# yhg926/MetaKSSD

Hardware: AMD Instinct MI355X
Metric: Gbases/s sketched (150 bp synthetic reads, L3K11 -A) (higher is better)
Workload: dtype u64 k-mers over u8 bases (integer)

## Files before the change

### include/metakssd_hip.h

```cpp
#ifndef METAKSSD_HIP_H
#define METAKSSD_HIP_H
#include <stddef.h>
#include <stdint.h>

#ifdef __cplusplus
extern "C" {
#endif

#define MK_ABI_VERSION 1

enum {
  MK_OK = 0,
  MK_ERR_ARG = -1,
  MK_ERR_NO_DEVICE = -2,
  MK_ERR_HIP = -3,
  MK_ERR_CROWDED = -4,
  MK_ERR_STATE = -5,
  MK_ERR_IO = -6,
  MK_ERR_FORMAT = -7,
  MK_ERR_NOMEM = -8
};

enum {
  MK_MODE_KOC = 0,
  MK_MODE_SET = 1,
  MK_MODE_UNIQ_SET = 2,
  MK_MODE_OCC_SET = 3
};

typedef struct mk_shuf {
  int32_t id, k, subk, drlevel;
  int32_t *table;
  uint64_t len;
} mk_shuf;

int mk_shuf_read(const char *path, mk_shuf *out);
int mk_shuf_generate(int32_t k, int32_t subk, int32_t drlevel, uint64_t seed, mk_shuf *out);
int mk_shuf_write(const mk_shuf *s, const char *path);
void mk_shuf_free(mk_shuf *s);

typedef struct mk_params {
  int32_t shuf_id, k, subk, drlevel;
  int32_t half_outctx_len;
  int32_t TL;
  int32_t crvsaddmove;
  int32_t component_num;
  int32_t comp_code_bits;
  int32_t dim_start, dim_end;
  uint32_t hashsize;
  uint32_t hashlimit;
  uint64_t tupmask, domask, undomask;
  const int32_t *shuf_table;
  uint64_t shuf_len;
  int32_t component_sz;
  int32_t reserved;
} mk_params;

int mk_params_init(const mk_shuf *shuf, mk_params *out);
int mk_params_init_csz(const mk_shuf *shuf, int32_t component_sz, mk_params *out);

typedef struct mk_engine mk_engine;

typedef struct mk_component {
  uint32_t *ids;
  uint16_t *counts;
  uint64_t n;
} mk_component;

typedef struct mk_result {
  int32_t component_num;
  uint64_t total;
  mk_component *components;
} mk_result;

typedef struct mk_profile {
  double scan_ms;
  uint64_t scan_launches;
  double resolve_ms;
  double clear_ms;
  double finish_ms;
  uint64_t bases_scanned;
  uint64_t rows_scanned;
  double finish_side_ms;
} mk_profile;

int mk_device_count(int *n);
int mk_engine_create(const mk_params *p, int device, mk_engine **out);
enum { MK_ENGINE_LAZY_TABLES = 1u };
int mk_engine_create_ex(const mk_params *p, int device, unsigned flags, mk_engine **out);
int mk_engine_destroy(mk_engine *e);
enum { MK_OPT_SPARSE = 1, MK_OPT_CAND_CAP = 2, MK_OPT_RESULT_CAP = 3, MK_OPT_DIRECT_HOST = 4, MK_OPT_FRONT_BITS = 5, MK_OPT_KEYLIST_CAP = 6,
       MK_OPT_BATCH_TAB_BITS = 7, MK_OPT_SPLIT_CUS = 10 };
int mk_engine_set_option(mk_engine *e, int option, int64_t value);
int mk_engine_set_stream(mk_engine *e, void *hip_stream);
int mk_engine_use_own_stream(mk_engine *e);
int mk_engine_share_scan_queue(mk_engine *e, mk_engine *with);
const char *mk_last_error(const mk_engine *e);

enum { MK_BEGIN_NOTHING_FOLLOWS = 0x100 };
int mk_sketch_begin(mk_engine *e, int mode);
int mk_sketch_begin_occ(mk_engine *e, int min_occurrence);
#define MK_ROW_PITCH(need) ((((need) + 15u) & ~15u) + (((((need) + 15u) & ~15u) & 127u) == 0u && (((need) + 15u) & ~15u) < 4096u ? 16u : 0u))
int mk_sketch_push_reads(mk_engine *e, const uint8_t *rows, uint32_t stride, uint64_t nreads, uint64_t first_read_ordinal);
#define MK_ROWS_PACKED 0x80000000u
#define MK_PACKED_PITCH 64u
#define MK_PACKED_MAX_BASES 152u
int mk_params_packed_ok(const mk_params *p);
int mk_pack_rows_host(const uint8_t *rows, uint32_t stride, uint64_t nrows, uint8_t *packed );
#define MK_ROWS_WIDE 0x40000000u
#define MK_WIDE_MAX_BASES 240u
uint64_t mk_fasta_pack_bound(size_t n, int32_t TL, uint32_t format);
int mk_fasta_pack_rows(const uint8_t *text, size_t n, int32_t TL, uint32_t format, uint8_t *rows, uint64_t max_rows, uint64_t *nrows);
int mk_sketch_push_reads_device(mk_engine *e, const uint8_t *rows_dev, uint32_t stride, uint64_t nreads,
                                uint64_t first_read_ordinal);
int mk_sketch_push_reads_async(mk_engine *e, const uint8_t *rows, uint32_t stride, uint64_t nreads, uint64_t first_read_ordinal,
                               uint64_t *ticket);
int mk_sketch_push_wait(mk_engine *e, uint64_t ticket);
int mk_sketch_push_stream(mk_engine *e, const uint8_t *text, uint64_t n, int final);
int mk_sketch_finish(mk_engine *e, mk_result *out);
int mk_sketch_finish_begin(mk_engine *e);
int mk_sketch_finish_end(mk_engine *e, mk_result *out);
int mk_result_release(mk_engine *e, mk_result *r);
int mk_engine_sync(mk_engine *e);

#define MK_BATCH_MAX_FILES 1024u
#define MK_BATCH_FILE_MAX ((uint64_t)64 << 20)
#define MK_BATCH_TEXT_MAX ((uint64_t)1 << 30)
typedef struct mk_batch_file {
  const uint8_t *text;
  uint64_t n;
} mk_batch_file;
typedef struct mk_batch_result {
  int32_t status;
  int32_t alone;
  mk_result r;
} mk_batch_result;
int mk_sketch_batch_begin(mk_engine *e, int mode, const mk_batch_file *files, uint32_t nfiles);
int mk_sketch_batch_begin_rows(mk_engine *e, int mode, uint32_t format, const mk_batch_file *files, uint32_t nfiles);
int mk_sketch_batch_end(mk_engine *e, mk_batch_result *out );

int mk_host_alloc(void **p, size_t bytes);
int mk_host_free(void *p);
int mk_host_register(void *p, size_t bytes);
int mk_host_unregister(void *p);
int mk_host_register_on(int device, void *p, size_t bytes);
int mk_host_arena_alloc(void **p, size_t bytes);
int mk_host_arena_free(void *p, size_t bytes);

int mk_partial_count(mk_engine *e, uint64_t *n);
int mk_partial_export(mk_engine *e, uint64_t *keys_dev, uint32_t *counts_dev, uint64_t *ords_dev, uint64_t capacity,
                      uint64_t *n_out);
int mk_partial_count_begin(mk_engine *e);
int mk_partial_export_async(mk_engine *e, uint64_t *keys_dev, uint32_t *counts_dev, uint64_t *ords_dev, uint64_t capacity,
                            uint64_t *n_out);
int mk_partial_import(mk_engine *e, const uint64_t *keys_dev, const uint32_t *counts_dev, const uint64_t *ords_dev,
                      uint64_t n);

int mk_partial_export_split_async(mk_engine *e, uint32_t nparts, uint64_t *keys_dev, uint32_t *counts_dev, uint64_t *ords_dev,
                                  uint64_t capacity, uint64_t *part_counts, uint64_t *n_out);
int mk_partial_export_split(mk_engine *e, uint32_t nparts, uint64_t *keys_dev, uint32_t *counts_dev, uint64_t *ords_dev,
                            uint64_t capacity, uint64_t *part_counts, uint64_t *n_out);
int mk_partial_restart(mk_engine *e);
int mk_partial_list_reserve(mk_engine *e, uint64_t n, uint64_t **keys_dev, uint32_t **counts_dev, uint64_t **ords_dev);
int mk_partial_list_commit(mk_engine *e, uint64_t n);
int mk_partial_list_adopt(mk_engine *e, const uint64_t *keys_dev, const uint32_t *counts_dev, const uint64_t *ords_dev, uint64_t n,
                          uint64_t offset);

int mk_profile_enable(mk_engine *e, int on);
int mk_profile_reset(mk_engine *e);
int mk_profile_get(mk_engine *e, mk_profile *out);

int mk_synth_rows_host(uint64_t seed, uint64_t first_read, uint64_t nreads, uint32_t len, uint32_t stride, uint8_t *rows);
int mk_synth_rows_device(int device, void *hip_stream, uint64_t seed, uint64_t first_read, uint64_t nreads, uint32_t len,
                         uint32_t stride, uint8_t *rows_dev);
int mk_synth_fastq_write(const char *path, uint64_t seed, uint64_t first_read, uint64_t nreads, uint32_t len);
int mk_synth_fastq_write_mt(const char *path, uint64_t seed, uint64_t first_read, uint64_t nreads, uint32_t len, int nthreads);

int mk_fastq_frame(const uint8_t *buf, size_t n, int final, uint8_t *rows, uint32_t stride, uint64_t max_rows,
                   uint64_t *nrows, size_t *consumed);
int mk_fastq_frame_q(const uint8_t *buf, size_t n, int final, int32_t qmin, int32_t TL, uint64_t records_before,
                     uint8_t *rows, uint32_t stride, uint64_t max_rows, uint64_t *nrows, uint64_t *nrecords,
                     size_t *consumed);
int mk_fastq_frame_mt(const uint8_t *buf, size_t n, int final, int occ, int32_t qmin, int32_t TL, uint64_t records_before,
                      uint8_t *rows, uint32_t stride, uint64_t max_rows, int nthreads, uint64_t *nrows, uint64_t *nrecords,
                      size_t *consumed);
typedef struct mk_fastq_opts {
  int32_t occ;
  int32_t qmin, TL;
  int32_t nthreads;
  int32_t inflight;
  uint64_t chunk_bytes;
  int32_t drop_pages;
  int32_t ahead;
  int32_t packed;
  int32_t fd;
  int32_t early_chunks;
  int32_t reserved2;
  uint64_t pool_bytes;
} mk_fastq_opts;
typedef struct mk_fastq_stats {
  uint64_t rows, records, chunks, chunks_discarded, serial_rows;
  uint32_t threads;
  double t_setup_s, t_wait_frame_s, t_push_s, t_total_s;
  double t_push_call_s, t_wait_call_s, t_push_call_max_s, t_first_push_call_s;
} mk_fastq_stats;
typedef struct mk_rows_sink {
  void *ctx;
  int (*push)(void *ctx, const uint8_t *rows, uint32_t stride, uint64_t nrows, uint64_t first_row_ordinal, uint64_t *token);
  int (*wait)(void *ctx, uint64_t token);
  uint8_t *(*alloc)(void *ctx, size_t bytes);
  void (*release)(void *ctx, uint8_t *p, size_t bytes);
  void (*ready)(void *ctx, const uint8_t *rows, size_t bytes);
} mk_rows_sink;
int mk_fastq_stream(const uint8_t *text, size_t n, const mk_fastq_opts *o, const mk_rows_sink *sink, uint64_t first_ordinal,
                    mk_fastq_stats *st);
int mk_sketch_push_fastq(mk_engine *e, const uint8_t *text, size_t n, const mk_fastq_opts *o, uint64_t first_ordinal,
                         mk_fastq_stats *st);

typedef struct mk_fasta_state {
  uint32_t TL;
  uint32_t in_header;
  uint32_t fill;
  uint32_t fresh;
  uint8_t pending[4096];
} mk_fasta_state;
int mk_fasta_window_init(mk_fasta_state *st, int32_t TL);
int mk_fasta_window(mk_fasta_state *st, const uint8_t *buf, size_t n, int final, uint8_t *rows, uint32_t stride,
                    uint64_t max_rows, uint64_t *nrows, size_t *consumed);

typedef struct mk_sketchdir mk_sketchdir;
int mk_sketchdir_open(const char *outdir, const mk_params *p, int koc, int nfiles, mk_sketchdir **out);
int mk_sketchdir_add(mk_sketchdir *d, const char *input_path, const mk_result *r);
int mk_sketchdir_close(mk_sketchdir *d);

enum { MK_SET_UNION = 0, MK_SET_UNIQ_UNION = 1 };
typedef struct mk_setop mk_setop;
int mk_setop_create(int device, mk_setop **out);
int mk_setop_destroy(mk_setop *s);
const char *mk_setop_last_error(const mk_setop *s);
int mk_setop_begin(mk_setop *s, int mode);
int mk_setop_add(mk_setop *s, const uint32_t *ids, uint64_t n);
int mk_setop_add_device(mk_setop *s, const uint32_t *ids_dev, uint64_t n);
int mk_setop_finish(mk_setop *s, const uint32_t **ids_out, uint64_t *n_out);
int mk_setop_result_device(mk_setop *s, const uint32_t **ids_dev, uint64_t *n);
int mk_setop_filter(mk_setop *s, int keep_members, const uint32_t *ids, uint64_t n, const uint64_t *bounds, uint32_t nb,
                    const uint32_t **ids_out, uint64_t *n_out, uint64_t *bounds_out);
// ... 174 lines not shown
```

### metakssd_amd/capi.py

```python
import ctypes as C
import os

import numpy as np

_HERE = os.path.dirname(os.path.abspath(__file__))
LIB_PATH = os.environ.get("MK_LIBRARY") or os.path.join(_HERE, "lib", "libmetakssd_hip.so")

MK_OK = 0
MK_ERR_ARG, MK_ERR_NO_DEVICE, MK_ERR_HIP, MK_ERR_CROWDED = -1, -2, -3, -4
MK_ERR_STATE, MK_ERR_IO, MK_ERR_FORMAT, MK_ERR_NOMEM = -5, -6, -7, -8
MK_MODE_KOC, MK_MODE_SET, MK_MODE_UNIQ_SET, MK_MODE_OCC_SET = 0, 1, 2, 3
MK_ROWS_PACKED, MK_PACKED_PITCH, MK_PACKED_MAX_BASES = 0x80000000, 64, 152
MK_ROWS_WIDE, MK_WIDE_MAX_BASES = 0x40000000, 240
MK_OPT_SPARSE, MK_OPT_CAND_CAP, MK_OPT_RESULT_CAP, MK_OPT_DIRECT_HOST, MK_OPT_FRONT_BITS, MK_OPT_KEYLIST_CAP, MK_OPT_BATCH_TAB_BITS = 1, 2, 3, 4, 5, 6, 7
MK_BEGIN_NOTHING_FOLLOWS = 0x100
MK_OPT_SPLIT_CUS = 10


class MkError(RuntimeError):
    def __init__(self, code, msg=""):
        super().__init__("metakssd_hip error %d: %s" % (code, msg))
        self.code = code


class CrowdedError(MkError):
    """more than hashlimit distinct keys: the reference aborts with 'the context space is too crowd' (iseq2comem.c:708-709)"""


class ShufC(C.Structure):
    _fields_ = [("id", C.c_int32), ("k", C.c_int32), ("subk", C.c_int32), ("drlevel", C.c_int32),
                ("table", C.POINTER(C.c_int32)), ("len", C.c_uint64)]


class ParamsC(C.Structure):
    _fields_ = [("shuf_id", C.c_int32), ("k", C.c_int32), ("subk", C.c_int32), ("drlevel", C.c_int32),
                ("half_outctx_len", C.c_int32), ("TL", C.c_int32), ("crvsaddmove", C.c_int32),
                ("component_num", C.c_int32), ("comp_code_bits", C.c_int32),
                ("dim_start", C.c_int32), ("dim_end", C.c_int32),
                ("hashsize", C.c_uint32), ("hashlimit", C.c_uint32),
                ("tupmask", C.c_uint64), ("domask", C.c_uint64), ("undomask", C.c_uint64),
                ("shuf_table", C.POINTER(C.c_int32)), ("shuf_len", C.c_uint64), ("component_sz", C.c_int32), ("reserved", C.c_int32)]


class ComponentC(C.Structure):
    _fields_ = [("ids", C.POINTER(C.c_uint32)), ("counts", C.POINTER(C.c_uint16)), ("n", C.c_uint64)]


class ResultC(C.Structure):
    _fields_ = [("component_num", C.c_int32), ("total", C.c_uint64), ("components", C.POINTER(ComponentC))]


class ProfileC(C.Structure):
    _fields_ = [("scan_ms", C.c_double), ("scan_launches", C.c_uint64), ("resolve_ms", C.c_double), ("clear_ms", C.c_double),
                ("finish_ms", C.c_double), ("bases_scanned", C.c_uint64), ("rows_scanned", C.c_uint64), ("finish_side_ms", C.c_double)]


class FastaStateC(C.Structure):
    _fields_ = [("TL", C.c_uint32), ("in_header", C.c_uint32), ("fill", C.c_uint32), ("fresh", C.c_uint32),
                ("pending", C.c_uint8 * 4096)]


class FastqOptsC(C.Structure):
    _fields_ = [("occ", C.c_int32), ("qmin", C.c_int32), ("TL", C.c_int32), ("nthreads", C.c_int32), ("inflight", C.c_int32),
                ("chunk_bytes", C.c_uint64), ("drop_pages", C.c_int32), ("ahead", C.c_int32), ("packed", C.c_int32), ("fd", C.c_int32),
                ("early_chunks", C.c_int32), ("reserved2", C.c_int32), ("pool_bytes", C.c_uint64)]


class FastqStatsC(C.Structure):
    _fields_ = [("rows", C.c_uint64), ("records", C.c_uint64), ("chunks", C.c_uint64), ("chunks_discarded", C.c_uint64),
                ("serial_rows", C.c_uint64), ("threads", C.c_uint32), ("t_setup_s", C.c_double), ("t_wait_frame_s", C.c_double),
                ("t_push_s", C.c_double), ("t_total_s", C.c_double), ("t_push_call_s", C.c_double), ("t_wait_call_s", C.c_double),
                ("t_push_call_max_s", C.c_double), ("t_first_push_call_s", C.c_double)]


_PUSH_FN = C.CFUNCTYPE(C.c_int, C.c_void_p, C.c_void_p, C.c_uint32, C.c_uint64, C.c_uint64, C.POINTER(C.c_uint64))
_WAIT_FN = C.CFUNCTYPE(C.c_int, C.c_void_p, C.c_uint64)
_ALLOC_FN = C.CFUNCTYPE(C.c_void_p, C.c_void_p, C.c_size_t)
_RELEASE_FN = C.CFUNCTYPE(None, C.c_void_p, C.c_void_p, C.c_size_t)
_READY_FN = C.CFUNCTYPE(None, C.c_void_p, C.c_void_p, C.c_size_t)


class RowsSinkC(C.Structure):
    _fields_ = [("ctx", C.c_void_p), ("push", _PUSH_FN), ("wait", _WAIT_FN), ("alloc", _ALLOC_FN), ("release", _RELEASE_FN),
                ("ready", C.c_void_p)]


class BatchFileC(C.Structure):
    _fields_ = [("text", C.c_void_p), ("n", C.c_uint64)]


class DistOptsC(C.Structure):
    _fields_ = [("metric", C.c_int32), ("outfields", C.c_int32), ("correction", C.c_int32), ("num_neigb", C.c_int32),
                ("dthreshold", C.c_double)]


class BgzfBlockC(C.Structure):
    _fields_ = [("in_off", C.c_uint64), ("out_off", C.c_uint64), ("in_len", C.c_uint32), ("pay_off", C.c_uint32), ("pay_len", C.c_uint32),
                ("crc32", C.c_uint32), ("isize", C.c_uint32), ("reserved", C.c_uint32)]


class GzipInfoC(C.Structure):
    _fields_ = [("pay_off", C.c_uint64), ("pay_len", C.c_uint64), ("crc32", C.c_uint32), ("isize", C.c_uint32), ("is_single", C.c_int32),
                ("reserved", C.c_int32)]


class GzMemberC(C.Structure):
    _fields_ = [("pay_off", C.c_uint64), ("out_off", C.c_uint64), ("pay_len", C.c_uint32), ("isize", C.c_uint32), ("crc32", C.c_uint32),
                ("reserved", C.c_uint32)]


class GzMemberResultC(C.Structure):
    _fields_ = [("status", C.c_uint32), ("consumed", C.c_uint32), ("pos", C.c_uint32), ("crc32", C.c_uint32)]


class GzFileC(C.Structure):
    _fields_ = [("comp", C.c_void_p), ("n", C.c_uint64), ("info", GzipInfoC)]


class BgzfOptsC(C.Structure):
    _fields_ = [("chunk_bytes", C.c_uint64), ("reserved", C.c_uint64)]


class BgzfStatsC(C.Structure):
    _fields_ = [("blocks", C.c_uint64), ("chunks", C.c_uint64), ("comp_bytes", C.c_uint64), ("text_bytes", C.c_uint64), ("rows", C.c_uint64),
                ("inflate_ms", C.c_double), ("frame_ms", C.c_double), ("t_scan_s", C.c_double), ("t_read_s", C.c_double), ("t_total_s", C.c_double),
                ("bad_block", C.c_int64), ("bad_status", C.c_int32), ("reserved", C.c_int32)]


def _load():
    if not os.path.exists(LIB_PATH):
        raise ImportError("%s not built: run `python -c 'import __graft_entry__ as g; g.build()'` "
                          "(make -C metakssd_amd/csrc)" % LIB_PATH)
    lib = C.CDLL(LIB_PATH)
    vp, u8p, u64, u32, i32 = C.c_void_p, C.POINTER(C.c_uint8), C.c_uint64, C.c_uint32, C.c_int32
    sig = {
        "mk_shuf_read": [C.c_char_p, C.POINTER(ShufC)],
        "mk_shuf_generate": [i32, i32, i32, u64, C.POINTER(ShufC)],
        "mk_shuf_write": [C.POINTER(ShufC), C.c_char_p],
        "mk_params_init": [C.POINTER(ShufC), C.POINTER(ParamsC)],
        "mk_params_init_csz": [C.POINTER(ShufC), i32, C.POINTER(ParamsC)],
        "mk_device_count": [C.POINTER(C.c_int)],
        "mk_engine_create": [C.POINTER(ParamsC), C.c_int, C.POINTER(vp)],
        "mk_engine_destroy": [vp],
        "mk_engine_set_option": [vp, C.c_int, C.c_int64],
        "mk_engine_set_stream": [vp, vp],
        "mk_engine_use_own_stream": [vp],
        "mk_engine_share_scan_queue": [vp, vp],
        "mk_sketch_begin": [vp, C.c_int],
        "mk_sketch_begin_occ": [vp, C.c_int],
        "mk_sketch_push_reads": [vp, vp, u32, u64, u64],
        "mk_sketch_push_reads_device": [vp, vp, u32, u64, u64],
        "mk_sketch_push_reads_async": [vp, vp, u32, u64, u64, C.POINTER(u64)],
        "mk_sketch_push_wait": [vp, u64],
        "mk_sketch_push_stream": [vp, vp, u64, C.c_int],
        "mk_partial_count_begin": [vp],
        "mk_partial_export_async": [vp, vp, vp, vp, u64, C.POINTER(u64)],
        "mk_pack_rows_host": [vp, u32, u64, vp],
        "mk_params_packed_ok": [C.POINTER(ParamsC)],
        "mk_sketch_batch_begin": [vp, C.c_int, vp, u32],
        "mk_sketch_batch_begin_rows": [vp, C.c_int, u32, vp, u32],
        "mk_fasta_pack_rows": [vp, C.c_size_t, C.c_int32, u32, vp, u64, C.POINTER(u64)],
        "mk_sketch_batch_end": [vp, vp],
        "mk_sketch_batch_begin_gz": [vp, C.c_int, C.POINTER(GzFileC), u32],
        "mk_sketch_batch_gz_status": [vp, vp, u32],
        "mk_gzip_scan": [C.c_int, vp, C.c_size_t, C.POINTER(GzipInfoC)],
        "mk_inflate_members": [vp, vp, C.c_size_t, C.POINTER(GzMemberC), u32, vp, C.c_size_t, C.POINTER(GzMemberResultC)],
        "mk_sketch_finish": [vp, C.POINTER(ResultC)],
        "mk_sketch_finish_begin": [vp],
        "mk_sketch_finish_end": [vp, C.POINTER(ResultC)],
        "mk_result_release": [vp, C.POINTER(ResultC)],
        "mk_engine_sync": [vp],
        "mk_host_alloc": [C.POINTER(vp), C.c_size_t],
        "mk_host_free": [vp],
        "mk_host_arena_alloc": [C.POINTER(vp), C.c_size_t],
        "mk_host_arena_free": [vp, C.c_size_t],
        "mk_host_register": [vp, C.c_size_t],
        "mk_host_unregister": [vp],
        "mk_partial_count": [vp, C.POINTER(u64)],
        "mk_partial_export": [vp, vp, vp, vp, u64, C.POINTER(u64)],
        "mk_partial_import": [vp, vp, vp, vp, u64],
        "mk_partial_export_split": [vp, u32, vp, vp, vp, u64, C.POINTER(u64), C.POINTER(u64)],
        "mk_partial_export_split_async": [vp, u32, vp, vp, vp, u64, C.POINTER(u64), C.POINTER(u64)],
        "mk_partial_restart": [vp],
        "mk_partial_list_reserve": [vp, u64, C.POINTER(vp), C.POINTER(vp), C.POINTER(vp)],
        "mk_partial_list_commit": [vp, u64],
        "mk_partial_list_adopt": [vp, vp, vp, vp, u64, u64],
        "mk_profile_enable": [vp, C.c_int],
        "mk_profile_reset": [vp],
        "mk_profile_get": [vp, C.POINTER(ProfileC)],
        "mk_synth_rows_host": [u64, u64, u64, u32, u32, vp],
        "mk_synth_rows_device": [C.c_int, vp, u64, u64, u64, u32, u32, vp],
        "mk_synth_fastq_write": [C.c_char_p, u64, u64, u64, u32],
        "mk_synth_fastq_write_mt": [C.c_char_p, u64, u64, u64, u32, C.c_int],
        "mk_fastq_stream": [vp, C.c_size_t, C.POINTER(FastqOptsC), C.POINTER(RowsSinkC), u64, C.POINTER(FastqStatsC)],
        "mk_sketch_push_fastq": [vp, vp, C.c_size_t, C.POINTER(FastqOptsC), u64, C.POINTER(FastqStatsC)],
        "mk_fastq_frame": [vp, C.c_size_t, C.c_int, vp, u32, u64, C.POINTER(u64), C.POINTER(C.c_size_t)],
        "mk_fastq_frame_q": [vp, C.c_size_t, C.c_int, i32, i32, u64, vp, u32, u64, C.POINTER(u64), C.POINTER(u64),
                             C.POINTER(C.c_size_t)],
        "mk_fastq_frame_mt": [vp, C.c_size_t, C.c_int, C.c_int, i32, i32, u64, vp, u32, u64, C.c_int, C.POINTER(u64), C.POINTER(u64),
                              C.POINTER(C.c_size_t)],
        "mk_fasta_window_init": [C.POINTER(FastaStateC), i32],
        "mk_fasta_window": [C.POINTER(FastaStateC), vp, C.c_size_t, C.c_int, vp, u32, u64, C.POINTER(u64),
                            C.POINTER(C.c_size_t)],
        "mk_setop_create": [C.c_int, C.POINTER(vp)],
        "mk_setop_destroy": [vp],
        "mk_setop_begin": [vp, C.c_int],
        "mk_setop_add": [vp, vp, u64],
        "mk_setop_add_device": [vp, vp, u64],
        "mk_setop_finish": [vp, C.POINTER(vp), C.POINTER(u64)],
        "mk_setop_result_device": [vp, C.POINTER(vp), C.POINTER(u64)],
        "mk_setop_join": [vp, vp, vp, u64, vp, u64, vp, u32, C.POINTER(vp), C.POINTER(u64), vp],
        "mk_setop_last_join_ms": [vp, C.POINTER(C.c_double)],
        "mk_mco_create": [C.c_int, C.POINTER(vp)],
        "mk_mco_destroy": [vp],
        "mk_mco_build": [vp, vp, vp, u32, C.POINTER(vp), C.POINTER(u64), C.POINTER(vp), C.POINTER(vp), C.POINTER(u64)],
        "mk_mco_index_rows": [vp, u64, u64, vp],
        "mk_mco_sort_pairs": [vp, vp, vp, u64],
        "mk_mco_set_option": [vp, C.c_int, C.c_int64],
        "mk_mco_count_begin": [vp, u32, u32],
        "mk_mco_count_add": [vp, vp, u64, vp, vp, vp, vp, vp],
        "mk_mco_count_finish": [vp, vp],
        "mk_mco_last_kernel_ms": [vp, C.POINTER(C.c_double), C.POINTER(C.c_double)],
        "mk_abv_create": [C.c_int, C.POINTER(vp)],
        "mk_abv_destroy": [vp],
        "mk_abv_index": [vp, vp, u64, vp, u32, u32, C.POINTER(vp), C.POINTER(vp), C.POINTER(vp), C.POINTER(C.c_int64)],
        "mk_abv_load": [vp, vp, u64, vp, u32, vp, u32],
        "mk_abv_search": [vp, C.c_int, u32, vp, vp, vp, C.POINTER(vp), C.POINTER(vp), C.POINTER(C.c_int64)],
        "mk_abv_last_kernel_ms": [vp, C.POINTER(C.c_double), C.POINTER(C.c_double)],
        "mk_composite_create": [C.c_int, C.POINTER(vp)],
        "mk_composite_destroy": [vp],
        "mk_composite_load_begin": [vp, u32, u32],
        "mk_composite_load_component": [vp, u32, vp, vp],
        "mk_composite_query_begin": [vp, u32],
        "mk_composite_query_component": [vp, u32, vp, vp, vp],
        "mk_composite_query_finish": [vp, C.POINTER(vp), vp],
        "mk_composite_set_option": [vp, C.c_int, C.c_int64],
        "mk_composite_last_kernel_ms": [vp, C.POINTER(C.c_double), C.POINTER(C.c_double)],
        "mk_composite_last_counts": [vp, C.POINTER(u64), C.POINTER(u64)],
        "mk_byread_create": [C.c_int, C.POINTER(vp)],
        "mk_byread_destroy": [vp],
        "mk_byread_begin": [vp, C.POINTER(ParamsC)],
        "mk_byread_push_text": [vp, vp, u64, C.c_int],
        "mk_byread_take": [vp, u32, C.POINTER(vp), C.POINTER(u64), C.POINTER(vp), C.POINTER(u64)],
        "mk_byread_finish": [vp, C.POINTER(u64), C.POINTER(u64), C.POINTER(C.c_double)],
        "mk_reverse_ids": [vp, vp, u64, u32, vp],
        "mk_byread_last_kernel_ms": [vp, C.POINTER(C.c_double), C.POINTER(C.c_double)],
        "mk_byread_write_stat": [C.c_char_p, C.POINTER(ParamsC), C.c_char_p],
        "mk_reverse_outname": [C.c_char_p, C.c_char_p, C.c_size_t],
        "mk_dist_print": [vp, C.POINTER(DistOptsC), i32, i32, u32, u32, vp, vp, vp, vp, vp],
        "mk_sketchdir_open": [C.c_char_p, C.POINTER(ParamsC), C.c_int, C.c_int, C.POINTER(vp)],
        "mk_sketchdir_add": [vp, C.c_char_p, C.POINTER(ResultC)],
        "mk_sketchdir_close": [vp],
        "mk_bgzf_scan": [C.c_int, vp, C.c_size_t, C.POINTER(C.POINTER(BgzfBlockC)), C.POINTER(u64), C.POINTER(u64), C.POINTER(C.c_int)],
        "mk_inflate_create": [C.c_int, C.POINTER(vp)],
        "mk_inflate_destroy": [vp],
        "mk_inflate_blocks": [vp, vp, C.c_size_t, C.POINTER(BgzfBlockC), u64, vp, C.c_size_t, vp],
        "mk_fastq_frame_device": [vp, vp, C.c_size_t, C.c_int, vp, C.c_size_t, C.POINTER(u32), C.POINTER(u64), C.POINTER(C.c_size_t), C.POINTER(u32)],
        "mk_fastq_frame_q_device": [vp, vp, C.c_size_t, C.c_int, i32, u64, vp, C.c_size_t, C.POINTER(u32), C.POINTER(u64), C.POINTER(u64),
                                    C.POINTER(C.c_size_t), C.POINTER(u32)],
        "mk_inflate_last_kernel_ms": [vp, C.POINTER(C.c_double), C.POINTER(C.c_double)],
        "mk_sketch_push_bgzf": [vp, C.c_int, C.c_size_t, C.POINTER(BgzfOptsC), u64, C.POINTER(BgzfStatsC)],
        "mk_sketch_push_bgzf_q": [vp, C.c_int, C.c_size_t, C.POINTER(BgzfOptsC), i32, u64, C.POINTER(BgzfStatsC)],
    }
    for name, args in sig.items():
        fn = getattr(lib, name)
        fn.argtypes = args
        fn.restype = C.c_int
    lib.mk_shuf_free.argtypes = [C.POINTER(ShufC)]
    lib.mk_shuf_free.restype = None
    lib.mk_setop_last_error.argtypes = [vp]
    lib.mk_setop_last_error.restype = C.c_char_p
    lib.mk_mco_last_error.argtypes = [vp]
    lib.mk_mco_last_error.restype = C.c_char_p
    lib.mk_abv_last_error.argtypes = [vp]
    lib.mk_abv_last_error.restype = C.c_char_p
    lib.mk_composite_last_error.argtypes = [vp]
    lib.mk_composite_last_error.restype = C.c_char_p
    lib.mk_byread_last_error.argtypes = [vp]
    lib.mk_byread_last_error.restype = C.c_char_p
    lib.mk_inflate_last_error.argtypes = [vp]
    lib.mk_inflate_last_error.restype = C.c_char_p
    lib.mk_inflate_status_text.argtypes = [C.c_int]
    lib.mk_inflate_status_text.restype = C.c_char_p
    lib.mk_bgzf_last_error.argtypes = []
    lib.mk_bgzf_last_error.restype = C.c_char_p
    lib.mk_bgzf_free.argtypes = [C.POINTER(BgzfBlockC)]
    lib.mk_bgzf_free.restype = None
    lib.mk_setop_stream.argtypes = [vp]
    lib.mk_setop_stream.restype = vp
    lib.mk_last_error.argtypes = [vp]
    lib.mk_last_error.restype = C.c_char_p
    lib.mk_fasta_pack_bound.argtypes = [C.c_size_t, C.c_int32, u32]
    lib.mk_fasta_pack_bound.restype = u64
    return lib


lib = _load()
# ... 51 lines not shown
def synth_rows_host(seed, first_read, nreads, length, stride):
    rows = np.empty(nreads * stride, dtype=np.uint8)
    _check(lib.mk_synth_rows_host(seed, first_read, nreads, length, stride, rows.ctypes.data))
    return rows


def pack_rows_host(rows, stride):
    rows = np.ascontiguousarray(rows, dtype=np.uint8)
    n = rows.size // stride
    raw = np.zeros(n * MK_PACKED_PITCH + 64, dtype=np.uint8)
    off = (-raw.ctypes.data) % 64
    out = raw[off:off + n * MK_PACKED_PITCH]
    _check(lib.mk_pack_rows_host(rows.ctypes.data if n else None, stride, n, out.ctypes.data if n else None))
    return out


def fasta_pack_rows(text, TL, fmt=None):
    fmt = MK_ROWS_PACKED if fmt is None else fmt
    b = np.frombuffer(bytes(text), dtype=np.uint8)
    bound = int(lib.mk_fasta_pack_bound(len(b), TL, fmt))
    raw = np.zeros(bound * MK_PACKED_PITCH + 64, dtype=np.uint8)
    off = (-raw.ctypes.data) % 64
    n = C.c_uint64(0)
    rc = lib.mk_fasta_pack_rows(b.ctypes.data if len(b) else None, len(b), TL, fmt, raw.ctypes.data + off, bound, C.byref(n))
    return raw[off:off + n.value * MK_PACKED_PITCH], rc


def fastq_frame(buf, stride, final=True, max_rows=None):
    b = np.frombuffer(buf, dtype=np.uint8)
    max_rows = max_rows if max_rows is not None else len(b) // 4 + 1
    rows = np.zeros(max(1, max_rows) * stride, dtype=np.uint8)
    n, used = C.c_uint64(0), C.c_size_t(0)
    rc = lib.mk_fastq_frame(b.ctypes.data if len(b) else None, len(b), 1 if final else 0, rows.ctypes.data, stride,
                            max_rows, C.byref(n), C.byref(used))
    return rows[: n.value * stride], n.value, used.value, rc


def fastq_frame_q(buf, stride, TL, qmin=0, final=True, records_before=0, max_rows=None):
    b = np.frombuffer(buf, dtype=np.uint8)
    max_rows = max_rows if max_rows is not None else len(b) // 4 + len(b) // max(1, stride - TL) + 2
    rows = np.zeros(max(1, max_rows) * stride, dtype=np.uint8)
    n, nrec, used = C.c_uint64(0), C.c_uint64(0), C.c_size_t(0)
    rc = lib.mk_fastq_frame_q(b.ctypes.data if len(b) else None, len(b), 1 if final else 0, qmin, TL, records_before,
                              rows.ctypes.data, stride, max_rows, C.byref(n), C.byref(nrec), C.byref(used))
    return rows[: n.value * stride], n.value, nrec.value, used.value, rc


def fastq_frame_mt(buf, stride, nthreads, occ=False, TL=22, qmin=0, final=True, records_before=0, max_rows=None):
    b = np.frombuffer(buf, dtype=np.uint8)
    max_rows = max_rows if max_rows is not None else len(b) // 4 + len(b) // max(1, stride - TL) + 2
    rows = np.zeros(max(1, max_rows) * stride, dtype=np.uint8)
    n, nrec, used = C.c_uint64(0), C.c_uint64(0), C.c_size_t(0)
    rc = lib.mk_fastq_frame_mt(b.ctypes.data if len(b) else None, len(b), 1 if final else 0, 1 if occ else 0, qmin, TL, records_before,
                               rows.ctypes.data, stride, max_rows, nthreads, C.byref(n), C.byref(nrec), C.byref(used))
    return rows[: n.value * stride], n.value, nrec.value, used.value, rc


def fastq_stream(buf, nthreads=4, chunk_bytes=0, occ=False, TL=22, qmin=0, first_ordinal=0, inflight=2, drop_pages=False, packed=False, pool_bytes=0,
                 ready_log=None, via_fd=False, early_chunks=0):
    b = np.frombuffer(buf, dtype=np.uint8)
    pushes, keep = [], {}
    libc = C.CDLL(None)
    libc.malloc.restype = C.c_void_p
    libc.malloc.argtypes = [C.c_size_t]
    libc.free.argtypes = [C.c_void_p]

    def push(ctx, rows, stride, nrows, ord0, token):
        a = np.ctypeslib.as_array(C.cast(rows, C.POINTER(C.c_uint8)), shape=(nrows * (stride & ~MK_ROWS_PACKED),)).copy()
        pushes.append((a, stride, nrows, ord0))
        token[0] = len(pushes)
        return 0

    def wait(ctx, token):
        return 0

    blocks = []

    def alloc(ctx, n):
        p = libc.malloc(n)
        blocks.append((p, n))
        return p

    def ready(ctx, rows, n):
        if ready_log is not None:
            ready_log.append((rows - blocks[-1][0], n))
    ready_fn = _READY_FN(ready)
    sink = RowsSinkC(None, _PUSH_FN(push), _WAIT_FN(wait), _ALLOC_FN(alloc), _RELEASE_FN(lambda ctx, p, n: libc.free(p)),
                     C.cast(ready_fn, C.c_void_p) if ready_log is not None else None)
    keep["sink"] = (sink, ready_fn)
    fd = -1
    if via_fd:
        import tempfile
        tf = tempfile.TemporaryFile()
        tf.write(bytes(buf))
        tf.flush()
        fd = tf.fileno()
        keep["file"] = tf
    o = FastqOptsC(1 if occ else 0, qmin, TL, nthreads, inflight, chunk_bytes, 1 if drop_pages else 0, 0, 1 if packed else 0, fd if via_fd else 0, early_chunks, 0, pool_bytes)
    if ready_log is not None:
        ready_log.append(blocks)
    st = FastqStatsC()
    rc = lib.mk_fastq_stream(None if via_fd or not len(b) else b.ctypes.data, len(b), C.byref(o), C.byref(sink), first_ordinal, C.byref(st))
    return pushes, st, rc


def fasta_windows(buf, TL, stride, chunk=None):
    b = np.frombuffer(buf, dtype=np.uint8)
    st = FastaStateC()
    _check(lib.mk_fasta_window_init(C.byref(st), TL))
    out = []
    max_rows = 4096
    rows = np.zeros(max_rows * stride, dtype=np.uint8)
    pos, step = 0, (chunk or max(1, len(b)))
    while True:
        end = min(len(b), pos + step)
        final = end >= len(b)
        off = pos
        while True:
            n, used = C.c_uint64(0), C.c_size_t(0)
            ptr = b[off:end].ctypes.data if end > off else None
            _check(lib.mk_fasta_window(C.byref(st), ptr, end - off, 1 if final else 0, rows.ctypes.data, stride, max_rows,
                                       C.byref(n), C.byref(used)))
            if n.value:
                out.append(rows[: n.value * stride].copy())
            off += used.value
            if off >= end and n.value < max_rows:
                break
        pos = end
        if final:
            break
    return np.concatenate(out) if out else np.zeros(0, dtype=np.uint8)


class Engine:

    def __init__(self, shuf, device=0, sparse=None, cand_cap=None, component_sz=8, front_bits=None):
        self.shuf = shuf
        self.params = shuf.params(component_sz)
        self.h = C.c_void_p()
        rc = lib.mk_engine_create(C.byref(self.params), device, C.byref(self.h))
        if rc != MK_OK:
            raise MkError(rc, lib.mk_last_error(None).decode(errors="replace"))
        self.device = device
        if sparse is not None:
            self.set_option(MK_OPT_SPARSE, int(sparse))
        if cand_cap is not None:
            self.set_option(MK_OPT_CAND_CAP, int(cand_cap))
        if front_bits is not None:
            self.set_option(MK_OPT_FRONT_BITS, int(front_bits))

    def set_option(self, option, value):
        _check(lib.mk_engine_set_option(self.h, option, value), self.h)

    def close(self):
        if self.h:
            lib.mk_engine_destroy(self.h)
            self.h = C.c_void_p()

    def __del__(self):
        try:
            self.close()
        except Exception:
            pass

    def set_stream(self, stream_handle):
        _check(lib.mk_engine_set_stream(self.h, C.c_void_p(stream_handle or None)), self.h)

    def use_own_stream(self):
        _check(lib.mk_engine_use_own_stream(self.h), self.h)

    def share_scan_queue(self, owner):
        _check(lib.mk_engine_share_scan_queue(self.h, owner.h), self.h)

    def begin(self, mode=MK_MODE_KOC):
        _check(lib.mk_sketch_begin(self.h, mode), self.h)

    def begin_occ(self, min_occurrence=1):
        _check(lib.mk_sketch_begin_occ(self.h, min_occurrence), self.h)

    def push_bgzf(self, path, chunk_bytes=0, first_ordinal=0, qmin=None):
        o, st = BgzfOptsC(chunk_bytes, 0), BgzfStatsC()
        fd = os.open(path, os.O_RDONLY)
        try:
            if qmin is None:
                rc = lib.mk_sketch_push_bgzf(self.h, fd, os.fstat(fd).st_size, C.byref(o), first_ordinal, C.byref(st))
            else:
                rc = lib.mk_sketch_push_bgzf_q(self.h, fd, os.fstat(fd).st_size, C.byref(o), qmin, first_ordinal, C.byref(st))
        finally:
            os.close(fd)
        if rc:
            err = MkError(rc, (lib.mk_bgzf_last_error() or b"").decode())
            err.stats = st
            raise err
        return st

    def push_bgzf_q(self, path, qmin=0, chunk_bytes=0, first_ordinal=0):
        return self.push_bgzf(path, chunk_bytes, first_ordinal, qmin=qmin)

    def push_reads(self, rows, stride, first_read_ordinal=0):
        rows = np.ascontiguousarray(rows, dtype=np.uint8)
        pitch = stride & ~MK_ROWS_PACKED
        assert rows.size % pitch == 0
        n = rows.size // pitch
        if n:
            _check(lib.mk_sketch_push_reads(self.h, rows.ctypes.data, stride, n, first_read_ordinal), self.h)
        return n

    def push_fastq(self, buf, nthreads=8, chunk_bytes=0, occ=False, TL=22, qmin=0, first_ordinal=0, inflight=2, packed=False):
        b = np.frombuffer(buf, dtype=np.uint8)
        o = FastqOptsC(1 if occ else 0, qmin, TL, nthreads, inflight, chunk_bytes, 0, 0, 1 if packed else 0)
        st = FastqStatsC()
        _check(lib.mk_sketch_push_fastq(self.h, b.ctypes.data if len(b) else None, len(b), C.byref(o), first_ordinal, C.byref(st)), self.h)
        return st

    def push_stream(self, text, final=True, piece=None):
        b = np.frombuffer(bytes(text), dtype=np.uint8)
        if not piece:
            _check(lib.mk_sketch_push_stream(self.h, b.ctypes.data if len(b) else None, len(b), 1 if final else 0), self.h)
            return
        at = 0
        while True:
            n = min(piece, len(b) - at)
            last = at + n >= len(b)
            part = np.ascontiguousarray(b[at:at + n])
            _check(lib.mk_sketch_push_stream(self.h, part.ctypes.data if n else None, n, 1 if (last and final) else 0), self.h)
            at += n
            if last:
                break

    def push_reads_async(self, rows, stride, first_read_ordinal=0):
        assert rows.dtype == np.uint8 and rows.flags["C_CONTIGUOUS"] and rows.size % stride == 0
        t = C.c_uint64(0)
        _check(lib.mk_sketch_push_reads_async(self.h, rows.ctypes.data, stride, rows.size // stride, first_read_ordinal, C.byref(t)), self.h)
        return t.value

    def push_wait(self, ticket):
        _check(lib.mk_sketch_push_wait(self.h, ticket), self.h)

    def push_reads_device(self, dev_ptr, stride, nreads, first_read_ordinal=0):
        _check(lib.mk_sketch_push_reads_device(self.h, C.c_void_p(dev_ptr), stride, nreads, first_read_ordinal), self.h)

    def finish(self):
        r = ResultC()
        _check(lib.mk_sketch_finish(self.h, C.byref(r)), self.h)
        out = []
        for c in range(r.component_num):
            comp = r.components[c]
            n = comp.n
            ids = np.ctypeslib.as_array(comp.ids, shape=(n,)).copy() if n else np.zeros(0, np.uint32)
            cnt = None
            if comp.counts:
                cnt = np.ctypeslib.as_array(comp.counts, shape=(n,)).copy() if n else np.zeros(0, np.uint16)
            out.append((ids, cnt))
        self.last_total = r.total
        lib.mk_result_release(self.h, C.byref(r))
        return out

    def batch_begin(self, texts, mode=MK_MODE_SET, one_buffer=False):
        arrs = []
        if one_buffer:
            offs, at = [], 0
            for t in texts:
                offs.append(at)
                at += (len(t) + 1023) // 1024 * 1024
            buf = np.zeros(max(at, 1024), dtype=np.uint8)
            for t, o in zip(texts, offs):
                buf[o:o + len(t)] = np.frombuffer(bytes(t), dtype=np.uint8)
            arrs = [buf[o:o + len(t)] for t, o in zip(texts, offs)]
            keep = [buf]
        else:
            arrs = [np.frombuffer(bytes(t), dtype=np.uint8).copy() for t in texts]
            keep = arrs
        files = (BatchFileC * len(texts))()
        for i, a in enumerate(arrs):
            files[i].text = (keep[0].ctypes.data + offs[i]) if one_buffer else (a.ctypes.data if a.size else None)
            files[i].n = a.size
        _check(lib.mk_sketch_batch_begin(self.h, mode, C.cast(files, C.c_void_p), len(texts)), self.h)
        self._batches = getattr(self, "_batches", [])
        self._batches.append((keep, len(texts)))

    def batch_begin_rows(self, row_arrays, mode=MK_MODE_SET, pinned=False, fmt=MK_ROWS_PACKED, gap=MK_PACKED_PITCH):
        n = len(row_arrays)
        files = (BatchFileC * n)()
        if pinned:
            total = sum(a.size + gap for a in row_arrays) + 4096
            p = C.c_void_p()
            _check(lib.mk_host_alloc(C.byref(p), total))
            buf = np.ctypeslib.as_array((C.c_uint8 * total).from_address(p.value))
            buf[:] = 0xA5
            at = 0
            for i, a in enumerate(row_arrays):
                buf[at:at + a.size] = a
                files[i].text = p.value + at
                files[i].n = a.size
                at += a.size + gap
            del buf
            keep = ("pinned", None, p.value)
        else:
            arrs = []
            for i, a in enumerate(row_arrays):
                raw = np.zeros(a.size + 64, dtype=np.uint8)
                off = (-raw.ctypes.data) % 64
                raw[off:off + a.size] = a
                arrs.append(raw)
                files[i].text = (raw.ctypes.data + off) if a.size else None
                files[i].n = a.size
# ... 768 lines not shown
```

### metakssd_amd/csrc/mk_engine.hip

```cpp
#include "metakssd_hip.h"
#include "mk_poison.hip.h"
#include "mk_kernels.hip.h"
#include "mk_stream.hip.h"
#include "mk_batch.hip.h"
#include "mk_gz.hip.h"
#include "mk_packed.hip.h"

#include <math.h>
#include <stdarg.h>
#include <stdio.h>
#include <stdlib.h>
#include <string.h>

#include <vector>

static thread_local char g_create_error[512] = "";

struct mk_evpair { hipEvent_t a, b; };
#define MK_TICKETS 16
#define MK_REGIONS 3
#define MK_REGION_BYTES ((size_t)256 << 20)

struct mk_engine {
  int device = 0;
  int num_cu = 0;
  mk_params P{};
  mk_keyparams kp{};
  char err[512] = "";
  hipStream_t own_stream = nullptr, stream = nullptr, copy_stream = nullptr;
  hipStream_t scan_stream = nullptr, split_stream = nullptr;
  hipEvent_t ev_scan_pre = nullptr, ev_scan_post = nullptr;
  int split_cus = 0, scan_cus = 0;
  bool tail = false, tail_active = false;
  bool scan_shared = false;
  mk_engine *scan_owner = nullptr;
  int scan_lent = 0;

  int32_t *d_shuf = nullptr;
  uint32_t *d_accept = nullptr;
  uint32_t *d_accept_bits = nullptr;
  uint32_t n_accept = 0;
  uint32_t bm_bits = 0;
  uint4 *d_cand = nullptr;
  uint32_t *d_cand_count = nullptr;
  uint32_t cand_slots = 0, cand_cap = 0;

  void *d_tab = nullptr;
  size_t tab_bytes = 0;
  bool sparse = false, tables_tracked = false;
  uint32_t *d_dirty_acc = nullptr, *d_dirty_slot = nullptr, *d_list_acc = nullptr, *d_list_slot = nullptr, *d_nlist = nullptr;
  uint32_t acc_words = 0, slot_words = 0, acc_blocks = 0;
  mk_table tab{};
  uint32_t *d_slot = nullptr;
  mk_dist dist{};
  uint32_t *d_chunk = nullptr;
  uint32_t nchunks = 0;
  unsigned long long *d_comp_totals = nullptr, *h_comp_totals = nullptr;
  unsigned long long *d_counters = nullptr;
  void *d_front = nullptr;
  mk_front *d_front_desc = nullptr;
  mk_front front{};
  uint64_t front_slots = 0;
  int front_bits_opt = -1;
  bool big_maybe_dirty = true;
  unsigned long long *h_counters = nullptr;
  bool tables_ready = false;
  bool init_queued = true;
  mk_accept_pair *d_pairs = nullptr;
  uint32_t *h_ids = nullptr;
  uint16_t *h_cnt = nullptr;
  uint64_t h_cap = 0;
  std::vector<mk_component> comps;

  uint8_t *d_stage[MK_REGIONS] = {};
  size_t stage_bytes = 0;
  hipEvent_t ev_copied[MK_REGIONS] = {}, ev_scanned[MK_REGIONS] = {};
  bool stage_two_streams[MK_REGIONS] = {};
  int stage_cur = 0;
  bool direct_host = false;
  bool region_open = false;
  size_t region_fill = 0;
  uint32_t region_stride = 0;
  uint64_t region_first_ord = 0, region_rows = 0;
  hipEvent_t ev_ticket[MK_TICKETS] = {};
  uint64_t tickets_issued = 0;
  std::vector<std::pair<const void *, size_t>> lds_granted;

  uint32_t *d_res_ids = nullptr;
  uint16_t *d_res_cnt = nullptr;
  uint64_t res_cap = 0;
  hipStream_t res_stream = nullptr;
  hipEvent_t ev_res = nullptr;
  bool res_koc = false;
  uint64_t res_D = 0;
  bool res_pending = false, res_side = false;
  uint64_t res_total = 0;
  unsigned long long *d_snap = nullptr, *h_snap = nullptr;
  std::vector<mk_evpair> ev_finish_side;
  void *d_kl = nullptr;
  uint64_t kl_cap = 0;
  uint32_t *d_kl_buckets = nullptr;
  uint64_t kl_bucket_cap = 0;
  bool slot_clean = false;
  uint8_t *d_text = nullptr, *d_stream = nullptr, *d_stream_tmp = nullptr;
  size_t text_cap = 0, stream_cap = 0;
  mk_fa_sum *d_fa_sum = nullptr;
  size_t fa_sum_cap = 0;
  mk_fa_state *d_fa_state = nullptr, *h_fa_state = nullptr;
  unsigned long long *d_split = nullptr;
  bool counter0_used = true;
  uint64_t fa_tail = 0;
  uint64_t fa_rows_done = 0;
  bool fa_used = false, fa_final = false;
  uint32_t fa_pitch = 0;

  struct mk_bctx *bctx[3] = {nullptr, nullptr, nullptr};
  uint64_t batch_begun = 0, batch_ended = 0;
  int batch_tb_opt = 0;
  std::vector<uint32_t> gz_status;
  const mk_batch_dev *cur_batch = nullptr;

  int mode = -1;
  uint32_t min_occ = 1;
  bool begun = false, compacted = false;
  bool count_queued = false;
  uint64_t D = 0;

  int tune_threads = 1024;
  bool tune_onepass = true;
  uint32_t tune_cb = MK_MAX_CB;

  bool profiling = false;
  std::vector<mk_evpair> ev_scan, ev_resolve, ev_clear, ev_finish, ev_pool;
  uint64_t prof_rows = 0, prof_bytes = 0;
};

static int mk_fail(mk_engine *e, int code, const char *fmt, ...) {
  char buf[512];
  va_list ap;
  va_start(ap, fmt);
  vsnprintf(buf, sizeof buf, fmt, ap);
  va_end(ap);
  if (e) snprintf(e->err, sizeof e->err, "%s", buf);
  else snprintf(g_create_error, sizeof g_create_error, "%s", buf);
  return code;
}

#define MK_HIP(e, call)                                                                                   \
  do {                                                                                                    \
    hipError_t _r = (call);                                                                               \
    if (_r != hipSuccess) return mk_fail((e), _r == hipErrorOutOfMemory ? MK_ERR_NOMEM : MK_ERR_HIP,      \
                                         "%s:%d %s -> %s", __FILE__, __LINE__, #call, hipGetErrorString(_r)); \
  } while (0)

extern "C" const char *mk_last_error(const mk_engine *e) { return e ? e->err : g_create_error; }

extern "C" int mk_device_count(int *n) {
  if (!n) return MK_ERR_ARG;
  int c = 0;
  hipError_t r = hipGetDeviceCount(&c);
  if (r != hipSuccess) { *n = 0; return mk_fail(nullptr, MK_ERR_NO_DEVICE, "hipGetDeviceCount: %s", hipGetErrorString(r)); }
  *n = c;
  return MK_OK;
}

extern "C" int mk_host_alloc(void **p, size_t bytes) {
  if (!p) return MK_ERR_ARG;
  hipError_t r = mk_pin_alloc(p, bytes, hipHostMallocDefault);
  return r == hipSuccess ? MK_OK : mk_fail(nullptr, MK_ERR_NOMEM, "mk_pin_alloc(%zu): %s", bytes, hipGetErrorString(r));
}
extern "C" int mk_host_free(void *p) { return hipHostFree(p) == hipSuccess ? MK_OK : MK_ERR_HIP; }
#include <pthread.h>
#include <sys/mman.h>
struct mk_touch_job { uint8_t *p; size_t n; pthread_t th; };
static void *mk_touch_run(void *arg) {
  mk_touch_job *j = (mk_touch_job *)arg;
  const int pz = mk_poison_byte();
  if (pz >= 0) memset(j->p, pz, j->n);
  else for (size_t off = 0; off < j->n; off += 4096) j->p[off] = 0;
  return nullptr;
}
extern "C" int mk_host_arena_alloc(void **out, size_t bytes) {
  if (!out || !bytes) return MK_ERR_ARG;
  const size_t huge = (size_t)2 << 20;
  const size_t len = (bytes + huge - 1) & ~(huge - 1);
  void *m = mmap(nullptr, len, PROT_READ | PROT_WRITE, MAP_PRIVATE | MAP_ANONYMOUS, -1, 0);
  if (m == MAP_FAILED) return mk_fail(nullptr, MK_ERR_NOMEM, "mmap(%zu) failed", len);
#ifdef MADV_HUGEPAGE
  (void)madvise(m, len, MADV_HUGEPAGE);
#endif
  enum { T = 8 };
  mk_touch_job job[T];
  int started = 0;
  for (int t = 0; t < T; t++) {
    const size_t lo = len / T * (size_t)t, hi = t + 1 == T ? len : len / T * (size_t)(t + 1);
    job[t].p = (uint8_t *)m + lo; job[t].n = hi - lo;
    if (t + 1 < T && pthread_create(&job[t].th, nullptr, mk_touch_run, &job[t]) == 0) started |= 1 << t;
    else mk_touch_run(&job[t]);
  }
  for (int t = 0; t < T; t++) if (started & (1 << t)) pthread_join(job[t].th, nullptr);
  hipError_t r = hipHostRegister(m, len, hipHostRegisterDefault);
  if (r != hipSuccess) {
    (void)hipGetLastError();
    munmap(m, len);
    return mk_fail(nullptr, r == hipErrorOutOfMemory ? MK_ERR_NOMEM : MK_ERR_HIP, "hipHostRegister(%zu): %s", len, hipGetErrorString(r));
  }
  *out = m;
  return MK_OK;
}
extern "C" int mk_host_arena_free(void *p, size_t bytes) {
  if (!p) return MK_ERR_ARG;
  const size_t huge = (size_t)2 << 20;
  const size_t len = (bytes + huge - 1) & ~(huge - 1);
  const bool ok = hipHostUnregister(p) == hipSuccess;
  if (!ok) (void)hipGetLastError();
  munmap(p, len);
  return ok ? MK_OK : MK_ERR_HIP;
}

extern "C" int mk_host_register(void *p, size_t bytes) {
  if (!p || !bytes) return MK_ERR_ARG;
  hipError_t r = hipHostRegister(p, bytes, hipHostRegisterDefault);
  if (r != hipSuccess) { (void)hipGetLastError(); return mk_fail(nullptr, MK_ERR_HIP, "hipHostRegister(%zu): %s", bytes, hipGetErrorString(r)); }
  return MK_OK;
}
extern "C" int mk_host_register_on(int device, void *p, size_t bytes) {
  if (hipSetDevice(device) != hipSuccess) { (void)hipGetLastError(); return mk_fail(nullptr, MK_ERR_NO_DEVICE, "hipSetDevice(%d) failed", device); }
  return mk_host_register(p, bytes);
}
extern "C" int mk_host_unregister(void *p) {
  if (hipHostUnregister(p) == hipSuccess) return MK_OK;
  (void)hipGetLastError();
  return MK_ERR_HIP;
}

static mk_evpair mk_ev_get(mk_engine *e) {
  mk_evpair p{nullptr, nullptr};
  if (!e->ev_pool.empty()) { p = e->ev_pool.back(); e->ev_pool.pop_back(); return p; }
  hipEventCreate(&p.a);
  hipEventCreate(&p.b);
  return p;
}

struct mk_accept_job {
  const int32_t *t;
  uint64_t lo, hi;
  int32_t ds, de;
  std::vector<mk_accept_pair> out;
  pthread_t th;
  bool started;
};
static void *mk_accept_run(void *arg) {
  mk_accept_job *j = (mk_accept_job *)arg;
  const int32_t *t = j->t;
  const uint32_t ds = (uint32_t)j->ds, span = (uint32_t)(j->de - j->ds);
  for (uint64_t d = j->lo; d < j->hi; d++) {
    const int32_t v = t[d];
    if ((uint32_t)v - ds < span) j->out.push_back(mk_accept_pair{(uint32_t)d, v});
  }
  return nullptr;
}

static void mk_bctx_free(struct mk_bctx *c);

extern "C" int mk_engine_destroy(mk_engine *e) {
  if (!e) return MK_ERR_ARG;
  if (e->scan_lent > 0) return mk_fail(e, MK_ERR_STATE, "mk_engine_destroy: %d engine(s) still borrow this engine's scan queue (mk_engine_share_scan_queue): destroy them first", e->scan_lent);
  if (e->scan_owner) { e->scan_owner->scan_lent--; e->scan_owner = nullptr; }
  hipSetDevice(e->device);
  (void)hipStreamSynchronize(e->stream);
  for (hipStream_t st : {e->own_stream, e->copy_stream, e->scan_stream, e->split_stream, e->res_stream})
    if (st && st != e->stream) (void)hipStreamSynchronize(st);
  hipFree(e->d_pairs);
  hipFree(e->d_cand); hipFree(e->d_cand_count);
  hipFree(e->d_shuf); hipFree(e->d_accept); hipFree(e->d_accept_bits); hipFree(e->d_tab); hipFree(e->d_front); hipFree(e->d_front_desc); hipFree(e->d_slot);
  hipFree(e->d_dirty_acc); hipFree(e->d_dirty_slot); hipFree(e->d_list_acc); hipFree(e->d_list_slot); hipFree(e->d_nlist);
  hipFree(e->dist.key); hipFree(e->dist.ord); hipFree(e->dist.cnt);
  hipFree(e->d_chunk); hipFree(e->d_comp_totals); hipFree(e->d_counters); hipFree(e->d_split);
  hipFree(e->d_kl); hipFree(e->d_kl_buckets);
  for (mk_bctx *c : e->bctx) mk_bctx_free(c);
  hipFree(e->d_res_ids); hipFree(e->d_res_cnt); hipFree(e->d_snap);
  if (e->h_snap) hipHostFree(e->h_snap);
  if (e->res_stream) hipStreamDestroy(e->res_stream);
  if (e->scan_stream && !e->scan_shared) hipStreamDestroy(e->scan_stream);
  if (e->split_stream) hipStreamDestroy(e->split_stream);
  if (e->ev_scan_pre) hipEventDestroy(e->ev_scan_pre);
  if (e->ev_scan_post) hipEventDestroy(e->ev_scan_post);
  if (e->ev_res) hipEventDestroy(e->ev_res);
  hipFree(e->d_text); hipFree(e->d_stream); hipFree(e->d_stream_tmp); hipFree(e->d_fa_sum); hipFree(e->d_fa_state);
  if (e->h_fa_state) hipHostFree(e->h_fa_state);
  for (int i = 0; i < MK_TICKETS; i++) if (e->ev_ticket[i]) hipEventDestroy(e->ev_ticket[i]);
  if (e->h_counters) hipHostFree(e->h_counters);
  if (e->h_ids) hipHostFree(e->h_ids);
  if (e->h_cnt) hipHostFree(e->h_cnt);
  for (int i = 0; i < MK_REGIONS; i++) {
    hipFree(e->d_stage[i]);
    if (e->ev_copied[i]) hipEventDestroy(e->ev_copied[i]);
    if (e->ev_scanned[i]) hipEventDestroy(e->ev_scanned[i]);
  }
  for (auto *v : {&e->ev_scan, &e->ev_resolve, &e->ev_clear, &e->ev_finish, &e->ev_finish_side, &e->ev_pool})
    for (auto &p : *v) { hipEventDestroy(p.a); hipEventDestroy(p.b); }
  if (e->own_stream) hipStreamDestroy(e->own_stream);
  delete e;
  return MK_OK;
}

static int mk_config_sparse(mk_engine *e, bool on) {
  hipFree(e->d_dirty_acc); hipFree(e->d_dirty_slot); hipFree(e->d_list_acc); hipFree(e->d_list_slot); hipFree(e->d_nlist);
  e->d_dirty_acc = e->d_dirty_slot = e->d_list_acc = e->d_list_slot = e->d_nlist = nullptr;
  e->tab.dirty = nullptr;
  e->tab.dirty_shift = 0;
  e->sparse = on;
  e->tables_tracked = false;
  if (!on) return MK_OK;
  const uint64_t S = e->P.hashsize;
  e->acc_blocks = (uint32_t)((S + MK_SPARSE_BLOCK - 1) / MK_SPARSE_BLOCK);
  e->acc_words = (e->acc_blocks + 31u) / 32u;
  const uint32_t nch = (uint32_t)((S + MK_DUMP_CHUNK - 1) / MK_DUMP_CHUNK);
  e->slot_words = (nch + 31u) / 32u;
  MK_HIP(e, mk_dev_alloc(&e->d_dirty_acc, (size_t)e->acc_words * 4));
  MK_HIP(e, mk_dev_alloc(&e->d_dirty_slot, (size_t)e->slot_words * 4));
  MK_HIP(e, mk_dev_alloc(&e->d_list_acc, (size_t)e->acc_words * 32 * 4));
  MK_HIP(e, mk_dev_alloc(&e->d_list_slot, (size_t)e->slot_words * 32 * 4));
  MK_HIP(e, mk_dev_alloc(&e->d_nlist, 4 * sizeof(uint32_t)));
  e->tab.dirty = e->d_dirty_acc;
  e->tab.dirty_shift = MK_SPARSE_SHIFT;
  return MK_OK;
}

static int mk_config_cand(mk_engine *e, uint32_t cap) {
  hipFree(e->d_cand); hipFree(e->d_cand_count);
  e->d_cand = nullptr; e->d_cand_count = nullptr;
  e->cand_cap = cap;
  MK_HIP(e, mk_dev_alloc(&e->d_cand, (size_t)e->cand_slots * (e->cand_cap + 1) * sizeof(uint4)));
  MK_HIP(e, mk_dev_alloc(&e->d_cand_count, (size_t)e->cand_slots * sizeof(uint32_t)));
  hipLaunchKernelGGL(mk_fill16_kernel, dim3(4), dim3(256), 0, e->stream, (uint4 *)e->d_cand_count, (unsigned long long)e->cand_slots / 4ull, 0u);
  MK_HIP(e, hipGetLastError());
  return MK_OK;
}

#include <time.h>
static double mk_tick_now() { timespec t; clock_gettime(CLOCK_MONOTONIC, &t); return t.tv_sec + 1e-9 * t.tv_nsec; }
#ifdef MK_TUNING
#define MK_TICK(label) do { if (getenv("MK_DEBUG")) { double n_ = mk_tick_now(); fprintf(stderr, "[engine create] %-22s %.4f s\n", label, n_ - tick_); tick_ = n_; } } while (0)
#else
#define MK_TICK(label) do { } while (0)
#endif

static int mk_config_front(mk_engine *e, int bits) {
  hipFree(e->d_front);
  e->d_front = nullptr; e->front_slots = 0;
  e->tab.fr = nullptr;
  e->front = mk_front{};
  e->big_maybe_dirty = true;
  const uint64_t S = e->P.hashsize;
  if (bits < 0) {
    bits = 0;
    if (!e->sparse && S >= (1ull << 20)) while ((2ull << bits) <= S / 6) bits++;
    if (e->sparse) {
      uint32_t sb = 0;
      while ((1ull << sb) < S) sb++;
      bits = sb > 21u ? 18 : (sb > 6u ? (int)sb - 3 : 3);
    }
  }
  if (bits == 0) return MK_OK;
  e->front_slots = 1ull << bits;
  MK_HIP(e, mk_dev_alloc(&e->d_front, e->front_slots * 16));
  if (!e->d_front_desc) MK_HIP(e, mk_dev_alloc((void **)&e->d_front_desc, sizeof(mk_front)));
  e->front.kc1 = (unsigned long long *)e->d_front;
  e->front.ordinv1 = e->front.kc1 + e->front_slots;
  e->front.state = (uint32_t *)(e->d_counters + 4);
  { uint32_t sb = 0; while ((1ull << sb) < S) sb++; e->front.shift = sb > (uint32_t)bits ? sb - (uint32_t)bits : 0u; }
  e->front.mask = (uint32_t)(e->front_slots - 1);
  e->front.limit = (uint32_t)(e->front_slots / 4);
  hipLaunchKernelGGL(mk_front_store_kernel, dim3(1), dim3(1), 0, e->stream, e->d_front_desc, e->front);
  MK_HIP(e, hipGetLastError());
  e->tab.fr = e->d_front_desc;
  return MK_OK;
}

static int mk_dist_reserve(mk_engine *e, uint64_t cap) {
  if (cap <= e->dist.cap && e->dist.key) return MK_OK;
  hipFree(e->dist.key); hipFree(e->dist.ord); hipFree(e->dist.cnt);
  e->dist.key = nullptr; e->dist.ord = nullptr; e->dist.cnt = nullptr; e->dist.cap = 0;
  MK_HIP(e, mk_dev_alloc(&e->dist.key, cap * 8));
  MK_HIP(e, mk_dev_alloc(&e->dist.ord, cap * 8));
  MK_HIP(e, mk_dev_alloc(&e->dist.cnt, cap * 4));
  e->dist.cap = cap;
  return MK_OK;
}

static int mk_tables_alloc(mk_engine *e);
static int mk_engine_init(mk_engine *e, const mk_params *p, bool lazy_tables) {
#ifdef MK_TUNING
  double tick_ = mk_tick_now();
#endif
  const uint64_t L = p->shuf_len;
  enum { NT = 4 };
  mk_accept_job job[NT];
  const int nt = L >= (1ull << 20) ? NT : 1;
  for (int t = 0; t < nt; t++) {
    job[t].t = p->shuf_table; job[t].lo = L / nt * (uint64_t)t; job[t].hi = t + 1 == nt ? L : L / nt * (uint64_t)(t + 1);
    job[t].ds = p->dim_start; job[t].de = p->dim_end;
    job[t].started = nt > 1 && pthread_create(&job[t].th, nullptr, mk_accept_run, &job[t]) == 0;
  }
  struct warm_job { int device; pthread_t th; bool started; } warm{e->device, {}, false};
  warm.started = pthread_create(&warm.th, nullptr, [](void *arg) -> void * {
    warm_job *w = (warm_job *)arg;
    hipFuncAttributes attr;
    if (hipSetDevice(w->device) != hipSuccess || hipFuncGetAttributes(&attr, (const void *)mk_fill16_kernel) != hipSuccess) (void)hipGetLastError();
    return nullptr;
  }, &warm) == 0;
  auto join_accept = [&]() {
    for (int t = 0; t < nt; t++) {
      if (job[t].started) { pthread_join(job[t].th, nullptr); job[t].started = false; }
      else if (job[t].t) mk_accept_run(&job[t]);
      job[t].t = nullptr;
    }
  };
  auto join_all = [&]() {
    join_accept();
    if (warm.started) { pthread_join(warm.th, nullptr); warm.started = false; }
  };
  struct joiner { decltype(join_all) &f; ~joiner() { f(); } } join_guard{join_all};

  MK_HIP(e, hipSetDevice(e->device));
  MK_HIP(e, hipDeviceGetAttribute(&e->num_cu, hipDeviceAttributeMultiprocessorCount, e->device));
  MK_TICK("device");
#ifdef MK_TUNING
  if (const char *t = getenv("MK_TUNE_CUS")) {
    const int n = atoi(t), first = getenv("MK_TUNE_CU_FIRST") ? atoi(getenv("MK_TUNE_CU_FIRST")) : 0;
    if (n < 1 || first < 0 || first + n > e->num_cu) return mk_fail(e, MK_ERR_ARG, "MK_TUNE_CUS / MK_TUNE_CU_FIRST out of range");
    uint32_t mask[16] = {0};
    for (int i = first; i < first + n; i++) mask[i >> 5] |= 1u << (i & 31);
    MK_HIP(e, hipExtStreamCreateWithCUMask(&e->own_stream, (uint32_t)((e->num_cu + 31) / 32), mask));
    e->num_cu = n;
    fprintf(stderr, "[tuning] queue on CUs %d..%d of the mask\n", first, first + n - 1);
  } else
#endif
  MK_HIP(e, hipStreamCreateWithFlags(&e->own_stream, hipStreamNonBlocking));
  MK_TICK("stream 1");
  e->copy_stream = e->own_stream;
  e->stream = e->own_stream;
  for (int i = 0; i < MK_REGIONS; i++) {
    MK_HIP(e, hipEventCreateWithFlags(&e->ev_copied[i], hipEventDisableTiming));
    MK_HIP(e, hipEventCreateWithFlags(&e->ev_scanned[i], hipEventDisableTiming));
  }

  e->P = *p;
  mk_keyparams &kp = e->kp;
  kp.tupmask = p->tupmask; kp.domask = p->domask; kp.undomask = p->undomask;
  kp.lowmask = (1ull << (2 * p->half_outctx_len)) - 1ull;
  kp.TL = (uint32_t)p->TL; kp.crvsaddmove = (uint32_t)p->crvsaddmove;
  kp.out2 = 2u * (uint32_t)p->half_outctx_len;
  kp.key_lshift = 2u * (uint32_t)p->TL - 4u * (uint32_t)p->half_outctx_len;
  kp.dr4 = 4u * (uint32_t)p->drlevel;
  kp.dim_start = p->dim_start; kp.dim_end = p->dim_end;
  kp.S = p->hashsize;

  const uint32_t dbits = 4u * (uint32_t)p->subk;
  const size_t bit_bytes = ((size_t)((L + 31) / 32) * sizeof(uint32_t) + 15u) & ~(size_t)15u;
  MK_HIP(e, mk_dev_alloc(&e->d_shuf, L * sizeof(int32_t)));
  MK_HIP(e, mk_dev_alloc(&e->d_accept_bits, bit_bytes));
  MK_HIP(e, mk_dev_alloc(&e->d_counters, 8 * sizeof(unsigned long long)));
  MK_TICK("events + first allocs");
  join_accept();
  size_t npairs = 0;
  for (int t = 0; t < nt; t++) npairs += job[t].out.size();
  if (npairs > (1u << 30)) return mk_fail(e, MK_ERR_ARG, "mk_engine_create: %zu accepted inner substrings", npairs);
  e->n_accept = (uint32_t)(2u * npairs);
  const size_t fixed = (16 + MK_MAX_COMP) * sizeof(unsigned long long);
  MK_HIP(e, mk_pin_alloc((void **)&e->h_counters, fixed + (npairs + 1) * sizeof(mk_accept_pair), hipHostMallocDefault));
  e->h_comp_totals = e->h_counters + 16;
  mk_accept_pair *hp = (mk_accept_pair *)((uint8_t *)e->h_counters + fixed);
  {
    size_t at = 0;
    for (int t = 0; t < nt; t++) { if (!job[t].out.empty()) memcpy(hp + at, job[t].out.data(), job[t].out.size() * sizeof(mk_accept_pair)); at += job[t].out.size(); }
  }
  MK_TICK("accept pass joined + pinned block");
  MK_HIP(e, mk_dev_alloc(&e->d_accept, ((size_t)e->n_accept + 2) * sizeof(uint32_t)));
  if (warm.started) { pthread_join(warm.th, nullptr); warm.started = false; }
  MK_TICK("code object");
  hipLaunchKernelGGL(mk_fill16_kernel, dim3((unsigned)e->num_cu * 2u), dim3(256), 0, e->own_stream, (uint4 *)e->d_accept_bits,
                     (unsigned long long)(bit_bytes / 16u), 0u);
  hipLaunchKernelGGL(mk_fill16_kernel, dim3(1), dim3(64), 0, e->own_stream, (uint4 *)e->d_counters, 4ull, 0u);
  MK_HIP(e, hipGetLastError());
  MK_TICK("first launches");
  if (npairs) {
    uint64_t blocks = (npairs + 255) / 256;
    if (blocks > (uint64_t)e->num_cu * 8u) blocks = (uint64_t)e->num_cu * 8u;
    hipLaunchKernelGGL(mk_accept_scatter_kernel, dim3((unsigned)blocks), dim3(256), 0, e->own_stream, (const mk_accept_pair *)hp,
                       (uint32_t)npairs, dbits, e->d_shuf, e->d_accept_bits, e->d_accept);
    MK_HIP(e, hipGetLastError());
  }
  MK_TICK("accept upload + scatter");
  {
    int wb = 4 * p->subk - 10;
    e->bm_bits = (uint32_t)(wb < 0 ? 0 : wb > 14 ? 14 : wb);
  }

  e->nchunks = (uint32_t)((p->hashsize + MK_DUMP_CHUNK - 1) / MK_DUMP_CHUNK);
  if (p->component_num > (int)MK_MAX_COMP) return mk_fail(e, MK_ERR_ARG, "component_num %d > %u", p->component_num, MK_MAX_COMP);
  e->tab.err = (uint32_t *)(e->d_counters + 2);
  e->comps.resize((size_t)p->component_num);
  e->cand_slots = (uint32_t)e->num_cu * 16u;
  { int rc = mk_config_cand(e, 8192u); if (rc) return rc; }
  MK_TICK("candidate buffers");
  for (int i = 0; i < MK_TICKETS; i++) MK_HIP(e, hipEventCreateWithFlags(&e->ev_ticket[i], hipEventDisableTiming));
#ifdef MK_TUNING
  if (const char *t = getenv("MK_SCAN_THREADS")) { int v = atoi(t); if (v == 512 || v == 768 || v == 1024) e->tune_threads = v; }
  if (const char *t = getenv("MK_SCAN_ONEPASS")) e->tune_onepass = atoi(t) != 0;
  if (const char *t = getenv("MK_SCAN_CB")) { int v = atoi(t); if (v >= 16 && v <= MK_MAX_CB && v % 16 == 0) e->tune_cb = (uint32_t)v; }
#endif
  return lazy_tables ? MK_OK : mk_tables_alloc(e);
}

static int mk_tables_alloc(mk_engine *e) {
  if (e->tables_ready) return MK_OK;
#ifdef MK_TUNING
  double tick_ = mk_tick_now();
#endif
  const mk_params *p = &e->P;
  MK_HIP(e, hipSetDevice(e->device));
  const uint64_t S = p->hashsize;
  e->tab_bytes = S * (8 + 8);
  MK_HIP(e, mk_dev_alloc(&e->d_tab, e->tab_bytes));
  e->tab.kc = (unsigned long long *)e->d_tab;
  e->tab.ordinv = e->tab.kc + S;
  MK_HIP(e, mk_dev_alloc(&e->d_slot, S * sizeof(uint32_t)));
  MK_TICK("table + layout table");
  { int rc = mk_config_sparse(e, S >= (1ull << 26)); if (rc) return rc; }
  { int rc = mk_config_front(e, -1); if (rc) return rc; }
  MK_TICK("sparse + front");
  { int rc = mk_dist_reserve(e, e->sparse && S > (32ull << 20) ? (32ull << 20) : S); if (rc) return rc; }
  MK_HIP(e, mk_dev_alloc(&e->d_chunk, (size_t)e->nchunks * (size_t)p->component_num * sizeof(uint32_t)));
  MK_HIP(e, mk_dev_alloc(&e->d_comp_totals, MK_MAX_COMP * sizeof(unsigned long long)));
  MK_TICK("key list + dump tables");
  e->tables_ready = true;
  return MK_OK;
}

extern "C" int mk_engine_create(const mk_params *p, int device, mk_engine **out) { return mk_engine_create_ex(p, device, 0u, out); }

extern "C" int mk_engine_create_ex(const mk_params *p, int device, unsigned flags, mk_engine **out) {
  if (!p || !out || !p->shuf_table) return mk_fail(nullptr, MK_ERR_ARG, "mk_engine_create: null argument");
  if (p->k < 1 || p->k > 16 || p->hashsize < 251u || p->shuf_len != (1ull << (4 * p->subk)))
    return mk_fail(nullptr, MK_ERR_ARG, "mk_engine_create: inconsistent mk_params (use mk_params_init)");
  int n = 0;
  hipError_t r = hipGetDeviceCount(&n);
  if (r != hipSuccess || n <= 0)
    return mk_fail(nullptr, MK_ERR_NO_DEVICE, "no HIP device (%s); this library has no CPU path",
                   r == hipSuccess ? "device count 0" : hipGetErrorString(r));
  if (device < 0 || device >= n) return mk_fail(nullptr, MK_ERR_NO_DEVICE, "device %d out of range (0..%d)", device, n - 1);
  mk_engine *e = new mk_engine();
  e->device = device;
  int rc = mk_engine_init(e, p, (flags & MK_ENGINE_LAZY_TABLES) != 0);
  if (rc != MK_OK) {
    snprintf(g_create_error, sizeof g_create_error, "%s", e->err);
    mk_engine_destroy(e);
    return rc;
  }
  *out = e;
  return MK_OK;
}

static int mk_flush_region(mk_engine *e);
static int mk_tail_end(mk_engine *e);

static int mk_poison_scratch(mk_engine *e) {
  if (mk_poison_byte() < 0) return MK_OK;
  { static const bool off = getenv("MK_POISON_SCRATCH") && atoi(getenv("MK_POISON_SCRATCH")) == 0; if (off) return MK_OK; }
  hipStream_t s = e->stream;
  if (e->d_cand) MK_HIP(e, mk_dev_repoison(e->d_cand, (size_t)e->cand_slots * (e->cand_cap + 1) * sizeof(uint4), s));
  if (e->d_kl) MK_HIP(e, mk_dev_repoison(e->d_kl, (size_t)e->kl_cap * (8 + 8 + 4 + 4 + 2) + 64, s));
  if (e->d_kl_buckets) MK_HIP(e, mk_dev_repoison(e->d_kl_buckets, (size_t)e->kl_bucket_cap * 4, s));
  if (e->d_split) MK_HIP(e, mk_dev_repoison(e->d_split, 2 * MK_SPLIT_MAX * sizeof(unsigned long long), s));
  if (!e->res_pending) {
    if (e->dist.key) {
      MK_HIP(e, mk_dev_repoison(e->dist.key, (size_t)e->dist.cap * 8, s));
      MK_HIP(e, mk_dev_repoison(e->dist.ord, (size_t)e->dist.cap * 8, s));
      MK_HIP(e, mk_dev_repoison(e->dist.cnt, (size_t)e->dist.cap * 4, s));
    }
    if (e->d_chunk) MK_HIP(e, mk_dev_repoison(e->d_chunk, (size_t)e->nchunks * (size_t)e->P.component_num * sizeof(uint32_t), s));
    if (e->d_comp_totals) MK_HIP(e, mk_dev_repoison(e->d_comp_totals, MK_MAX_COMP * sizeof(unsigned long long), s));
    if (e->d_res_ids) {
      MK_HIP(e, mk_dev_repoison(e->d_res_ids, (size_t)e->res_cap * 4, s));
      MK_HIP(e, mk_dev_repoison(e->d_res_cnt, (size_t)e->res_cap * 2, s));
    }
  }
  if (e->d_text) MK_HIP(e, mk_dev_repoison(e->d_text, e->text_cap, s));
  if (e->d_stream) MK_HIP(e, mk_dev_repoison(e->d_stream, e->stream_cap, s));
  if (e->d_stream_tmp) MK_HIP(e, mk_dev_repoison(e->d_stream_tmp, 8192, s));
  if (e->d_fa_sum) MK_HIP(e, mk_dev_repoison(e->d_fa_sum, e->fa_sum_cap * sizeof(mk_fa_sum), s));
  if (e->d_stage[0] && e->copy_stream == e->stream)
    for (int i = 0; i < MK_REGIONS; i++) MK_HIP(e, mk_dev_repoison(e->d_stage[i], e->stage_bytes, s));
  return MK_OK;
}

static int mk_config_split(mk_engine *e, int r) {
  bool nomask = false;
#ifdef MK_TUNING
  nomask = getenv("MK_TUNE_SPLIT_NOMASK") != nullptr;
#endif
  if (r != 0 && !nomask && (r < 32 || r > e->num_cu / 2 || r % 32 != 0))
    return mk_fail(e, MK_ERR_ARG, "MK_OPT_SPLIT_CUS takes 0 (one queue) or a multiple of 32 up to half the device's %d compute units", e->num_cu);
  if (e->batch_begun != e->batch_ended) return mk_fail(e, MK_ERR_STATE, "MK_OPT_SPLIT_CUS while a batch is in flight");
  if (e->scan_lent > 0) return mk_fail(e, MK_ERR_STATE, "MK_OPT_SPLIT_CUS: %d engine(s) borrow this engine's scan queue (set them back to one queue first)", e->scan_lent);
  if (e->scan_owner) { e->scan_owner->scan_lent--; e->scan_owner = nullptr; }
  if (e->stream == e->split_stream && e->split_stream) e->stream = e->own_stream;
  e->tail = e->tail_active = false;
  if (e->scan_stream) { (void)hipStreamSynchronize(e->scan_stream); if (!e->scan_shared) (void)hipStreamDestroy(e->scan_stream); e->scan_stream = nullptr; }
  if (e->split_stream) { (void)hipStreamSynchronize(e->split_stream); (void)hipStreamDestroy(e->split_stream); e->split_stream = nullptr; }
  if (e->res_stream) { (void)hipStreamSynchronize(e->res_stream); (void)hipStreamDestroy(e->res_stream); e->res_stream = nullptr; }
  e->split_cus = 0; e->scan_cus = 0; e->scan_shared = false;
  if (e->init_queued) { MK_HIP(e, hipStreamSynchronize(e->own_stream)); e->init_queued = false; }
  if (r == 0) return MK_OK;
  const int n = e->num_cu;
  uint32_t scan_mask[16] = {0}, rest_mask[16] = {0};
  if (n > 512) return mk_fail(e, MK_ERR_ARG, "MK_OPT_SPLIT_CUS: %d compute units", n);
  for (int i = 0; i < n; i++) (i < n - r ? scan_mask : rest_mask)[i >> 5] |= 1u << (i & 31);
  if (nomask) {
    MK_HIP(e, hipStreamCreateWithFlags(&e->scan_stream, hipStreamNonBlocking));
    MK_HIP(e, hipStreamCreateWithFlags(&e->split_stream, hipStreamNonBlocking));
  } else {
    MK_HIP(e, hipExtStreamCreateWithCUMask(&e->scan_stream, (uint32_t)((n + 31) / 32), scan_mask));
    MK_HIP(e, hipExtStreamCreateWithCUMask(&e->split_stream, (uint32_t)((n + 31) / 32), rest_mask));
  }
  if (!e->ev_scan_pre) {
    MK_HIP(e, hipEventCreateWithFlags(&e->ev_scan_pre, hipEventDisableTiming));
    MK_HIP(e, hipEventCreateWithFlags(&e->ev_scan_post, hipEventDisableTiming));
  }
  e->split_cus = r; e->scan_cus = n - r;
  if (e->stream == e->own_stream) e->stream = e->split_stream;
  return MK_OK;
}

extern "C" int mk_engine_set_option(mk_engine *e, int option, int64_t value) {
  if (!e) return MK_ERR_ARG;
  if (e->begun) return mk_fail(e, MK_ERR_STATE, "mk_engine_set_option inside a sketch (between begin and finish)");
  if (e->res_pending) return mk_fail(e, MK_ERR_STATE, "mk_engine_set_option while a result is outstanding (mk_sketch_finish_end first)");
  MK_HIP(e, hipSetDevice(e->device));
  if (option == MK_OPT_SPARSE || option == MK_OPT_FRONT_BITS || option == MK_OPT_KEYLIST_CAP) { int rc = mk_tables_alloc(e); if (rc) return rc; }
  MK_HIP(e, hipStreamSynchronize(e->stream));
  if (e->res_stream) MK_HIP(e, hipStreamSynchronize(e->res_stream));
  switch (option) {
    case MK_OPT_SPARSE: {
      if (value < -1 || value > 1) return mk_fail(e, MK_ERR_ARG, "MK_OPT_SPARSE takes -1 (by table size), 0 or 1");
      int rc = mk_config_sparse(e, value < 0 ? e->P.hashsize >= (1u << 26) : value != 0);
      if (rc == MK_OK && !e->sparse) rc = mk_dist_reserve(e, e->kp.S);
      return rc ? rc : mk_config_front(e, e->front_bits_opt);
    }
    case MK_OPT_FRONT_BITS:
      if (value < -1 || (value > 0 && value < 3) || value > 28) return mk_fail(e, MK_ERR_ARG, "MK_OPT_FRONT_BITS takes -1 (by table size), 0 (none) or 3..28");
      e->front_bits_opt = (int)value;
      return mk_config_front(e, e->front_bits_opt);
    case MK_OPT_CAND_CAP:
      if (value < 0 || value > (1 << 20)) return mk_fail(e, MK_ERR_ARG, "MK_OPT_CAND_CAP takes 0 .. 2^20 records per scan wave");
      if (e->batch_begun != e->batch_ended) return mk_fail(e, MK_ERR_STATE, "MK_OPT_CAND_CAP while a batch is in flight");
      return mk_config_cand(e, (uint32_t)value);
    case MK_OPT_DIRECT_HOST:
      e->direct_host = value != 0;
      return MK_OK;
    case MK_OPT_SPLIT_CUS: return mk_config_split(e, (int)value);
    case MK_OPT_BATCH_TAB_BITS:
      if (value != 0 && (value < 9 || value > 22)) return mk_fail(e, MK_ERR_ARG, "MK_OPT_BATCH_TAB_BITS takes 0 (by file size) or 9..22");
      if (e->batch_begun != e->batch_ended) return mk_fail(e, MK_ERR_STATE, "MK_OPT_BATCH_TAB_BITS while a batch is in flight");
      e->batch_tb_opt = (int)value;
      return MK_OK;
    case MK_OPT_KEYLIST_CAP: {
      if (!e->sparse) return mk_fail(e, MK_ERR_ARG, "MK_OPT_KEYLIST_CAP needs sparse bookkeeping (the dense passes do not grow the key list)");
      if (value < 16 || (uint64_t)value > e->kp.S) return mk_fail(e, MK_ERR_ARG, "MK_OPT_KEYLIST_CAP takes 16 .. hashsize entries");
      hipFree(e->dist.key); hipFree(e->dist.ord); hipFree(e->dist.cnt);
      e->dist.key = nullptr; e->dist.ord = nullptr; e->dist.cnt = nullptr; e->dist.cap = 0;
      return mk_dist_reserve(e, (uint64_t)value);
    }
    case MK_OPT_RESULT_CAP: {
      if (value < 1 || value > (int64_t)e->P.hashsize) return mk_fail(e, MK_ERR_ARG, "MK_OPT_RESULT_CAP takes 1 .. hashsize entries");
      if (e->h_ids) hipHostFree(e->h_ids);
      if (e->h_cnt) hipHostFree(e->h_cnt);
      e->h_ids = nullptr; e->h_cnt = nullptr; e->h_cap = 0;
      MK_HIP(e, mk_pin_alloc((void **)&e->h_ids, (size_t)value * 4, hipHostMallocDefault));
      MK_HIP(e, mk_pin_alloc((void **)&e->h_cnt, (size_t)value * 2, hipHostMallocDefault));
      e->h_cap = (uint64_t)value;
      return MK_OK;
    }
    default: return mk_fail(e, MK_ERR_ARG, "unknown engine option %d", option);
  }
}

extern "C" int mk_engine_set_stream(mk_engine *e, void *hip_stream) {
  if (!e) return MK_ERR_ARG;
  if (e->region_open) {
    MK_HIP(e, hipSetDevice(e->device));
    int rc = mk_flush_region(e);
    if (rc) return rc;
  }
  if (e->init_queued) {
    MK_HIP(e, hipSetDevice(e->device));
    MK_HIP(e, hipStreamSynchronize(e->own_stream));
    e->init_queued = false;
  }
  { int rc = mk_tail_end(e); if (rc) return rc; }
  if (e->split_stream && (hipStream_t)hip_stream != e->split_stream) {
    MK_HIP(e, hipSetDevice(e->device));
    MK_HIP(e, hipEventRecord(e->ev_scan_pre, e->split_stream));
    MK_HIP(e, hipStreamWaitEvent((hipStream_t)hip_stream, e->ev_scan_pre, 0));
  }
  e->stream = (hipStream_t)hip_stream;
  return MK_OK;
}
extern "C" int mk_engine_share_scan_queue(mk_engine *e, mk_engine *with) {
  if (!e || !with || e == with) return MK_ERR_ARG;
  if (e->begun) return mk_fail(e, MK_ERR_STATE, "mk_engine_share_scan_queue inside a sketch");
  if (!e->scan_stream || !with->scan_stream || with->scan_shared || e->split_cus != with->split_cus || e->device != with->device)
    return mk_fail(e, MK_ERR_ARG, "mk_engine_share_scan_queue: both engines need the same MK_OPT_SPLIT_CUS setting on one device, and the owner a queue of its own");
  MK_HIP(e, hipSetDevice(e->device));
  MK_HIP(e, hipStreamSynchronize(e->scan_stream));
  if (e->scan_lent > 0) return mk_fail(e, MK_ERR_STATE, "mk_engine_share_scan_queue: this engine's own queue is lent to another engine");
  if (!e->scan_shared) MK_HIP(e, hipStreamDestroy(e->scan_stream));
  if (e->scan_owner) e->scan_owner->scan_lent--;
  e->scan_stream = with->scan_stream;
  e->scan_shared = true;
  e->scan_owner = with;
  with->scan_lent++;
  return MK_OK;
}
extern "C" int mk_engine_use_own_stream(mk_engine *e) {
  if (!e) return MK_ERR_ARG;
  if (e->region_open) {
    MK_HIP(e, hipSetDevice(e->device));
    int rc = mk_flush_region(e);
    if (rc) return rc;
  }
  { int rc = mk_tail_end(e); if (rc) return rc; }
  e->stream = e->split_stream ? e->split_stream : e->own_stream;
  return MK_OK;
}

extern "C" int mk_engine_sync(mk_engine *e) {
  if (!e) return MK_ERR_ARG;
  MK_HIP(e, hipSetDevice(e->device));
  { int rc = mk_flush_region(e); if (rc) return rc; }
  if (e->copy_stream != e->stream) MK_HIP(e, hipStreamSynchronize(e->copy_stream));
  MK_HIP(e, hipStreamSynchronize(e->stream));
  return MK_OK;
}

extern "C" int mk_engine_get_stream(mk_engine *e, void **hip_stream, int *device) {
  if (!e || !hip_stream) return MK_ERR_ARG;
  if (e->scan_stream) return mk_fail(e, MK_ERR_STATE, "mk_engine_get_stream: MK_OPT_SPLIT_CUS runs the scan on a queue of its own");
  MK_HIP(e, hipSetDevice(e->device));
  { int rc = mk_flush_region(e); if (rc) return rc; }
  if (e->copy_stream != e->stream) MK_HIP(e, hipStreamSynchronize(e->copy_stream));
  *hip_stream = (void *)e->stream;
  if (device) *device = e->device;
  return MK_OK;
}

extern "C" int mk_profile_enable(mk_engine *e, int on) { if (!e) return MK_ERR_ARG; e->profiling = on != 0; return MK_OK; }

extern "C" int mk_profile_reset(mk_engine *e) {
  if (!e) return MK_ERR_ARG;
  MK_HIP(e, hipSetDevice(e->device));
  MK_HIP(e, hipStreamSynchronize(e->stream));
  if (e->res_stream) MK_HIP(e, hipStreamSynchronize(e->res_stream));
  for (auto *v : {&e->ev_scan, &e->ev_resolve, &e->ev_clear, &e->ev_finish, &e->ev_finish_side}) {
    for (auto &p : *v) e->ev_pool.push_back(p);
    v->clear();
  }
  e->prof_rows = e->prof_bytes = 0;
  return MK_OK;
}

extern "C" int mk_profile_get(mk_engine *e, mk_profile *out) {
  if (!e || !out) return MK_ERR_ARG;
  MK_HIP(e, hipSetDevice(e->device));
  MK_HIP(e, hipStreamSynchronize(e->stream));
  if (e->res_stream) MK_HIP(e, hipStreamSynchronize(e->res_stream));
  memset(out, 0, sizeof *out);
  auto sum = [&](std::vector<mk_evpair> &v) {
    double s = 0;
    for (auto &p : v) { float ms = 0; if (hipEventElapsedTime(&ms, p.a, p.b) == hipSuccess) s += ms; }
    return s;
  };
  out->scan_ms = sum(e->ev_scan);
  out->scan_launches = e->ev_scan.size();
  out->resolve_ms = sum(e->ev_resolve);
  out->clear_ms = sum(e->ev_clear);
  out->finish_ms = sum(e->ev_finish);
  out->finish_side_ms = sum(e->ev_finish_side);
  out->rows_scanned = e->prof_rows;
  out->bases_scanned = e->prof_bytes;
  return MK_OK;
}

static int mk_tail_end(mk_engine *e) {
  e->tail = false;
  if (e->tail_active) {
    if (e->split_stream && e->stream == e->own_stream) {
      MK_HIP(e, hipEventRecord(e->ev_scan_pre, e->own_stream));
      MK_HIP(e, hipStreamWaitEvent(e->split_stream, e->ev_scan_pre, 0));
      e->stream = e->split_stream;
    }
    e->tail_active = false;
  }
  return MK_OK;
}

extern "C" int mk_sketch_begin_occ(mk_engine *e, int min_occurrence) {
  if (!e) return MK_ERR_ARG;
  if (min_occurrence < 1 || min_occurrence >= 15)
    return mk_fail(e, MK_ERR_ARG, "fastq2co(): Occurence num should be 1..14 (got %d)", min_occurrence);
  int rc = mk_sketch_begin(e, MK_MODE_OCC_SET);
  if (rc == MK_OK) e->min_occ = (uint32_t)min_occurrence;
  return rc;
}

extern "C" int mk_sketch_begin(mk_engine *e, int mode) {
  if (!e) return MK_ERR_ARG;
  const bool tail = (mode & MK_BEGIN_NOTHING_FOLLOWS) != 0;
  mode &= ~MK_BEGIN_NOTHING_FOLLOWS;
  if (mode < MK_MODE_KOC || mode > MK_MODE_OCC_SET) return MK_ERR_ARG;
  MK_HIP(e, hipSetDevice(e->device));
  { int rc = mk_tables_alloc(e); if (rc) return rc; }
  { int rc = mk_tail_end(e); if (rc) return rc; }
  e->tail = tail && e->scan_stream && e->stream == e->split_stream;
  { int rc = mk_poison_scratch(e); if (rc) return rc; }
  mk_evpair ev{};
  if (e->profiling) { ev = mk_ev_get(e); MK_HIP(e, hipEventRecord(ev.a, e->stream)); }
  bool clear_front = false;
  if (e->sparse && e->tables_tracked) {
    if (!e->tab.fr || e->big_maybe_dirty) {
      hipLaunchKernelGGL(mk_dirty_list_kernel, dim3(1), dim3(1024), 0, e->stream, e->d_dirty_acc, e->acc_words, e->d_list_acc, e->d_nlist, 1,
                         (const uint32_t *)nullptr);
      hipLaunchKernelGGL(mk_dirty_clear_kernel, dim3((unsigned)e->num_cu * 8u), dim3(256), 0, e->stream, e->tab.kc, e->tab.ordinv, e->kp.S,
                         (const uint32_t *)e->d_list_acc, (const uint32_t *)e->d_nlist, (uint32_t)MK_SPARSE_SHIFT, (uint32_t *)nullptr,
                         (const uint32_t *)nullptr, (const uint32_t *)nullptr, (uint32_t)MK_DUMP_SHIFT);
      MK_HIP(e, hipGetLastError());
    }
    if (e->tab.fr) { clear_front = true; e->big_maybe_dirty = false; }
    if (!e->slot_clean) {
      MK_HIP(e, hipMemsetAsync(e->d_slot, 0xFF, (size_t)e->kp.S * sizeof(uint32_t), e->stream));
      e->slot_clean = true;
    }
  } else {
    if (!e->tab.fr || e->big_maybe_dirty) MK_HIP(e, hipMemsetAsync(e->d_tab, 0, e->tab_bytes, e->stream));
    if (e->tab.fr) { clear_front = true; e->big_maybe_dirty = false; }
    if (e->sparse) {
      MK_HIP(e, hipMemsetAsync(e->d_slot, 0xFF, (size_t)e->kp.S * sizeof(uint32_t), e->stream));
      MK_HIP(e, hipMemsetAsync(e->d_dirty_acc, 0, (size_t)e->acc_words * 4, e->stream));
      MK_HIP(e, hipMemsetAsync(e->d_dirty_slot, 0, (size_t)e->slot_words * 4, e->stream));
      e->tables_tracked = true;
      e->slot_clean = true;
    }
  }
  {
    const unsigned long long n16 = clear_front ? (unsigned long long)e->front_slots : 0ull;
    unsigned long long blocks = (n16 + 1023u) / 1024u;
    if (blocks > (unsigned long long)e->num_cu * 8u) blocks = (unsigned long long)e->num_cu * 8u;
    if (blocks == 0) blocks = 1;
    const bool fa = e->fa_used && e->d_fa_state;
    hipLaunchKernelGGL(mk_begin_clear_kernel, dim3((unsigned)blocks), dim3(256), 0, e->stream, (uint4 *)e->d_front, n16, e->d_counters,
                       (uint32_t *)e->d_fa_state, fa ? (uint32_t)(sizeof(mk_fa_state) / 4u) : 0u);
    MK_HIP(e, hipGetLastError());
    e->counter0_used = false;
  }
  if (e->profiling) { MK_HIP(e, hipEventRecord(ev.b, e->stream)); e->ev_clear.push_back(ev); }
  e->region_open = false;
  e->mode = mode;
  e->min_occ = 1;
  e->begun = true;
  e->compacted = false;
  e->count_queued = false;
  e->D = 0;
  e->fa_used = false; e->fa_final = false; e->fa_tail = 0; e->fa_rows_done = 0; e->fa_pitch = 0;
  return MK_OK;
}

template <int K, int SK, bool V, int T, int NP, bool OP>
static hipError_t mk_launch_scan_t(mk_engine *e, const mk_scan_args &a, dim3 grid, size_t lds, hipStream_t s) {
  const void *fn = (const void *)mk_scan_kernel<K, SK, V, T, NP, OP>;
  size_t *granted = nullptr;
  for (auto &g : e->lds_granted) if (g.first == fn) granted = &g.second;
  if (!granted) { e->lds_granted.emplace_back(fn, 0); granted = &e->lds_granted.back().second; }
  if (lds > *granted) {
    hipError_t r = hipFuncSetAttribute(fn, hipFuncAttributeMaxDynamicSharedMemorySize, (int)lds);
    if (r != hipSuccess) return r;
    *granted = lds;
  }
  hipLaunchKernelGGL((mk_scan_kernel<K, SK, V, T, NP, OP>), grid, dim3(T), lds, s, a);
  return hipGetLastError();
}
template <int K, int SK, bool V>
static hipError_t mk_launch_scan_k(mk_engine *e, int threads, bool onepass, const mk_scan_args &a, dim3 grid, size_t lds, hipStream_t s) {
  constexpr int NPBIG = V ? MK_MAX_PIECES : MK_MAX_CB / 4;
  constexpr int NPSMALL = V ? 5 : 20;
  const bool small = a.ppr <= (uint32_t)NPSMALL;
  if constexpr (V) {
    if (onepass && small)
      return threads >= 1024 ? mk_launch_scan_t<K, SK, V, 1024, NPSMALL, true>(e, a, grid, lds, s)
             : threads >= 768 ? mk_launch_scan_t<K, SK, V, 768, NPSMALL, true>(e, a, grid, lds, s)
                              : mk_launch_scan_t<K, SK, V, 512, NPSMALL, true>(e, a, grid, lds, s);
  }
  switch (threads) {
    case 1024: return small ? mk_launch_scan_t<K, SK, V, 1024, NPSMALL, false>(e, a, grid, lds, s) : mk_launch_scan_t<K, SK, V, 1024, NPBIG, false>(e, a, grid, lds, s);
    case 768: return small ? mk_launch_scan_t<K, SK, V, 768, NPSMALL, false>(e, a, grid, lds, s) : mk_launch_scan_t<K, SK, V, 768, NPBIG, false>(e, a, grid, lds, s);
    default: return small ? mk_launch_scan_t<K, SK, V, 512, NPSMALL, false>(e, a, grid, lds, s) : mk_launch_scan_t<K, SK, V, 512, NPBIG, false>(e, a, grid, lds, s);
  }
}

static int mk_launch_scan_ex(mk_engine *e, const uint8_t *rows_dev, uint32_t stride, uint32_t pitch, uint32_t rowlen, uint64_t nreads,
                             const unsigned long long *nreads_dev, uint64_t first_ord) {
  if (nreads == 0) return MK_OK;
  if (nreads >= (1ull << 31)) return mk_fail(e, MK_ERR_ARG, "scan launch of %llu reads: the caller splits pushes below 2^31", (unsigned long long)nreads);
  const bool wide = (stride & MK_ROWS_WIDE) != 0;
  const bool packed = (stride & (MK_ROWS_PACKED | MK_ROWS_WIDE)) != 0;
  if (packed) { stride &= ~(MK_ROWS_PACKED | MK_ROWS_WIDE); pitch = stride; }
  mk_scan_args a{};
  a.rows = rows_dev; a.nreads = nreads; a.first_ord = first_ord; a.stride = stride;
  a.pitch = pitch; a.rowlen = rowlen; a.nreads_dev = nreads_dev;
  const bool vec = (stride % 16u == 0) && (pitch % 16u == 0) && (((uintptr_t)rows_dev & 15u) == 0);
  const bool tuned_sk = (e->P.subk == 6 && e->P.k >= 9 && e->P.k <= 11) || (e->P.subk == 5 && e->P.k == 11);
  const bool tuned_geom = tuned_sk && stride % 8u == 0;
  const uint32_t g = vec ? 16u : (tuned_geom ? 8u : 4u);
  const uint32_t max_cb = e->tune_cb;
  a.ncb = (stride + max_cb - 1) / max_cb;
  a.CB = ((stride + a.ncb - 1) / a.ncb + g - 1) / g * g;
  if (a.CB > max_cb) { a.ncb++; a.CB = ((stride + a.ncb - 1) / a.ncb + g - 1) / g * g; }
  a.ncb = (stride + a.CB - 1) / a.CB;
  a.ppr = a.CB / (vec ? 16u : 4u);
  a.ppr_inv = (1u << 20) / a.ppr + 1u;
  a.rowdw = (a.CB / 4u) | 1u;
  a.wave_lds_dwords = ((64u * a.rowdw + 1u) & ~1u) + 2u;
  a.bm_words = 1u << e->bm_bits;
  const int tuned_k = (tuned_sk && stride % 8u == 0 && a.CB % 8u == 0) ? e->P.k : 0;
  if (packed && !tuned_k) return mk_fail(e, MK_ERR_ARG, "packed rows need a geometry with a tuned scan kernel");
  a.mt_words = tuned_k && e->P.subk == 6 ? MK_ZMASK_WORDS : 0u;
  a.pair_subk = tuned_k ? (uint32_t)e->P.subk : 0u;
  if (tuned_k && e->P.subk == 5) a.bm_words = 16384u;
  a.dimmask = (uint32_t)((1ull << (4 * e->P.subk)) - 1ull);
  a.accept = e->d_accept; a.n_accept = e->n_accept;
  a.shuf = e->d_shuf;
  a.accept_bits = e->d_accept_bits;
  a.kp = e->kp;
  a.tab = e->tab;
  a.cand = e->d_cand; a.cand_count = e->d_cand_count; a.cand_cap = e->cand_cap;
  a.batch = e->cur_batch;
  if (a.batch) a.tab.fr = nullptr;
  const bool onepass = e->tune_onepass && vec && a.ncb == 2 && stride == 2u * a.CB && a.ppr <= 5u;
  int threads = e->tune_threads;
  size_t lds = 0;
  const size_t fwords = tuned_k && e->P.subk == 6 && !packed ? (size_t)MK_ZF_WORDS : (size_t)a.bm_words;
  for (;; threads -= 256) {
    lds = ((size_t)a.mt_words + fwords + (size_t)(threads / 64) * a.wave_lds_dwords) * 4u;
    if (vec) lds += 2u * (a.ppr <= 5u ? 5u : (uint32_t)MK_MAX_PIECES) * 64u * 4u;
    if (packed) { threads = 1024; lds = ((size_t)a.mt_words + (size_t)a.bm_words) * 4u; }
    if (lds <= 160u * 1024u || threads <= 512) break;
  }
  if (lds > 160u * 1024u) return mk_fail(e, MK_ERR_ARG, "scan: LDS budget exceeded (%zu bytes)", lds);
  const uint32_t waves = (uint32_t)threads / 64u;
  const uint64_t ntiles = (nreads + 63) / 64;
  uint64_t blocks = (ntiles + waves - 1) / waves;
  uint64_t wgs_per_cu = 1;
#ifdef MK_TUNING
  if (const char *t = getenv("MK_SCAN_WGS_PER_CU")) { const int v = atoi(t); if (v >= 1 && v * waves <= 16u) wgs_per_cu = (uint64_t)v; }
#endif
  const uint64_t scan_cus = e->scan_stream ? (uint64_t)e->scan_cus : (uint64_t)e->num_cu;
  if (blocks > scan_cus * wgs_per_cu) blocks = scan_cus * wgs_per_cu;
  dim3 grid((unsigned)blocks);
#ifdef MK_TUNING
  if (getenv("MK_DEBUG")) {
    static int once = 0;
    if (!once++) fprintf(stderr, "scan cfg: threads %d blocks %llu CB %u ncb %u rowdw %u lds %zu B onepass %d\n", threads,
                         (unsigned long long)blocks, a.CB, a.ncb, a.rowdw, lds, (int)onepass);
  }
#endif

  if (!a.batch) e->big_maybe_dirty = true;
  hipStream_t ss = e->stream;
  if (e->scan_stream) {
    MK_HIP(e, hipEventRecord(e->ev_scan_pre, e->stream));
    MK_HIP(e, hipStreamWaitEvent(e->scan_stream, e->ev_scan_pre, 0));
    ss = e->scan_stream;
  }
  mk_evpair ev{};
  if (e->profiling) { ev = mk_ev_get(e); MK_HIP(e, hipEventRecord(ev.a, ss)); }
  hipError_t r;
  if (packed) {
    auto launch_packed = [&](auto kern) -> hipError_t {
      const void *fn = (const void *)kern;
      size_t *granted = nullptr;
      for (auto &g : e->lds_granted) if (g.first == fn) granted = &g.second;
      if (!granted) { e->lds_granted.emplace_back(fn, 0); granted = &e->lds_granted.back().second; }
      if (lds > *granted) {
        const hipError_t rr = hipFuncSetAttribute(fn, hipFuncAttributeMaxDynamicSharedMemorySize, (int)lds);
        if (rr != hipSuccess) return rr;
        *granted = lds;
      }
      hipLaunchKernelGGL(kern, grid, dim3(1024), lds, ss, a);
      return hipGetLastError();
    };
    if (wide) switch (tuned_k * 10 + e->P.subk) {
      case 116: r = launch_packed(mk_scan_packed_kernel<11, 6, true>); break;
      case 106: r = launch_packed(mk_scan_packed_kernel<10, 6, true>); break;
      case 96: r = launch_packed(mk_scan_packed_kernel<9, 6, true>); break;
      default: r = launch_packed(mk_scan_packed_kernel<11, 5, true>); break;
    } else switch (tuned_k * 10 + e->P.subk) {
      case 116: r = launch_packed(mk_scan_packed_kernel<11, 6>); break;
      case 106: r = launch_packed(mk_scan_packed_kernel<10, 6>); break;
      case 96: r = launch_packed(mk_scan_packed_kernel<9, 6>); break;
      default: r = launch_packed(mk_scan_packed_kernel<11, 5>); break;
    }
  } else
  switch (tuned_k * 10 + (tuned_k ? e->P.subk : 0)) {
    case 116: r = vec ? mk_launch_scan_k<11, 6, true>(e, threads, onepass, a, grid, lds, ss) : mk_launch_scan_k<11, 6, false>(e, threads, false, a, grid, lds, ss); break;
    case 106: r = vec ? mk_launch_scan_k<10, 6, true>(e, threads, onepass, a, grid, lds, ss) : mk_launch_scan_k<10, 6, false>(e, threads, false, a, grid, lds, ss); break;
    case 96: r = vec ? mk_launch_scan_k<9, 6, true>(e, threads, onepass, a, grid, lds, ss) : mk_launch_scan_k<9, 6, false>(e, threads, false, a, grid, lds, ss); break;
    case 115: r = vec ? mk_launch_scan_k<11, 5, true>(e, threads, onepass, a, grid, lds, ss) : mk_launch_scan_k<11, 5, false>(e, threads, false, a, grid, lds, ss); break;
    default: r = vec ? mk_launch_scan_k<0, 0, true>(e, threads, onepass, a, grid, lds, ss) : mk_launch_scan_k<0, 0, false>(e, threads, false, a, grid, lds, ss); break;
  }
  if (r != hipSuccess) return mk_fail(e, MK_ERR_HIP, "scan launch: %s", hipGetErrorString(r));
  if (e->profiling) {
    MK_HIP(e, hipEventRecord(ev.b, ss));
    e->ev_scan.push_back(ev);
    e->prof_rows += nreads;
    e->prof_bytes += nreads * stride;
  }
  if (e->scan_stream) {
    MK_HIP(e, hipEventRecord(e->ev_scan_post, ss));
    if (e->tail && e->begun && !a.batch && e->stream == e->split_stream) {
      MK_HIP(e, hipEventRecord(e->ev_scan_pre, e->split_stream));
      MK_HIP(e, hipStreamWaitEvent(e->own_stream, e->ev_scan_pre, 0));
      e->stream = e->own_stream;
      e->tail_active = true;
    }
    MK_HIP(e, hipStreamWaitEvent(e->stream, e->ev_scan_post, 0));
  }
  {
    const uint32_t used_slots = (uint32_t)blocks * waves;
    mk_evpair ev2{};
    if (e->profiling) { ev2 = mk_ev_get(e); MK_HIP(e, hipEventRecord(ev2.a, e->stream)); }
    const uint32_t rwgs = (used_slots + MK_RESOLVE_THREADS / 64 - 1) / (MK_RESOLVE_THREADS / 64);
    const uint32_t rcus = e->scan_stream && e->stream == e->split_stream ? (uint32_t)e->split_cus : (uint32_t)e->num_cu;
    uint32_t rgrid = rwgs < rcus ? rwgs : rcus;
#ifdef MK_TUNING
    if (const char *t = getenv("MK_RESOLVE_GRID")) { const uint32_t g = (uint32_t)atoi(t); if (g && g <= used_slots) rgrid = g; }
#endif
    const size_t rlds = (size_t)a.bm_words * 4u + (size_t)(MK_RESOLVE_THREADS / 64) * 2u * MK_RQ_CAP * sizeof(uint4);
    {
      const void *fn = (const void *)mk_resolve_kernel;
      size_t *granted = nullptr;
      for (auto &g : e->lds_granted) if (g.first == fn) granted = &g.second;
      if (!granted) { e->lds_granted.emplace_back(fn, 0); granted = &e->lds_granted.back().second; }
      if (rlds > *granted) {
        MK_HIP(e, hipFuncSetAttribute(fn, hipFuncAttributeMaxDynamicSharedMemorySize, (int)rlds));
        *granted = rlds;
      }
    }
    hipLaunchKernelGGL(mk_resolve_kernel, dim3(rgrid), dim3(MK_RESOLVE_THREADS), rlds, e->stream, a, used_slots);
    MK_HIP(e, hipGetLastError());
#ifdef MK_TUNING
    if (getenv("MK_COUNT_RECORDS")) {
      static int shown = 0;
      if (shown++ < 3) {
        std::vector<uint32_t> h(used_slots);
        MK_HIP(e, hipStreamSynchronize(e->stream));
        MK_HIP(e, hipMemcpy(h.data(), e->d_cand_count, (size_t)used_slots * 4, hipMemcpyDeviceToHost));
        unsigned long long sum = 0;
        for (uint32_t v : h) sum += v;
        fprintf(stderr, "[scan records] %llu reads -> %llu candidate records (%.4f a read, %.3f %% of the 8-base windows of 150-base reads)\n",
                (unsigned long long)nreads, sum, (double)sum / (double)nreads, 100.0 * (double)sum / ((double)nreads * 19.0));
      }
    }
#endif
    if (e->profiling) { MK_HIP(e, hipEventRecord(ev2.b, e->stream)); e->ev_resolve.push_back(ev2); }
  }
  if (!a.batch) { e->compacted = false; e->count_queued = false; }
  return MK_OK;
}

static int mk_launch_scan(mk_engine *e, const uint8_t *rows_dev, uint32_t stride, uint64_t nreads, uint64_t first_ord) {
  return mk_launch_scan_ex(e, rows_dev, stride, stride, 0u, nreads, nullptr, first_ord);
}

static int mk_check_push(mk_engine *e, const void *rows, uint32_t stride) {
  if (!e) return MK_ERR_ARG;
  if (!e->begun) return mk_fail(e, MK_ERR_STATE, "push before mk_sketch_begin");
  if (stride & MK_ROWS_PACKED) {
    if (stride != (MK_PACKED_PITCH | MK_ROWS_PACKED)) return mk_fail(e, MK_ERR_ARG, "push: packed rows have a pitch of %u bytes", MK_PACKED_PITCH);
    if (!mk_params_packed_ok(&e->P)) return mk_fail(e, MK_ERR_ARG, "push: packed rows need a geometry with a tuned scan kernel (mk_params_packed_ok)");
    if (!rows) return mk_fail(e, MK_ERR_ARG, "push: rows == NULL");
    if ((uintptr_t)rows & 15u) return mk_fail(e, MK_ERR_ARG, "push: packed rows must be 16-byte aligned");
    return MK_OK;
  }
  if (!rows || stride < 4 || stride > 4096 || (stride & 3u)) return mk_fail(e, MK_ERR_ARG, "push: stride must be a multiple of 4 in 4..4096");
  return MK_OK;
}

extern "C" int mk_sketch_push_reads_device(mk_engine *e, const uint8_t *rows_dev, uint32_t stride, uint64_t nreads,
                                           uint64_t first_read_ordinal) {
  int rc = mk_check_push(e, rows_dev, stride);
  if (rc) return rc;
  MK_HIP(e, hipSetDevice(e->device));
  if ((first_read_ordinal + nreads) >> 51) return mk_fail(e, MK_ERR_ARG, "read ordinal too large");
  const uint64_t waves = (uint64_t)e->num_cu * (uint64_t)(e->tune_threads / 64);
  uint64_t per = (uint64_t)(e->cand_cap / 32u) * 64u * waves;
  if (per < 64u * waves) per = 64u * waves;
  if (per > (1ull << 30)) per = 1ull << 30;
  for (uint64_t done = 0; done < nreads; done += per) {
    const uint64_t n = nreads - done < per ? nreads - done : per;
    int rc2 = mk_launch_scan(e, rows_dev + done * (uint64_t)(stride & ~MK_ROWS_PACKED), stride, n, first_read_ordinal + done);
    if (rc2) return rc2;
  }
  return MK_OK;
}

static int mk_flush_region(mk_engine *e) {
  if (!e->region_open) return MK_OK;
  const int b = e->stage_cur;
  e->region_open = false;
  e->stage_cur = (b + 1) % MK_REGIONS;
  if (e->region_rows == 0) return MK_OK;
  const bool two_streams = e->stream != e->copy_stream;
  if (two_streams) {
    MK_HIP(e, hipEventRecord(e->ev_copied[b], e->copy_stream));
    MK_HIP(e, hipStreamWaitEvent(e->stream, e->ev_copied[b], 0));
  }
  int rc = mk_launch_scan(e, e->d_stage[b], e->region_stride, e->region_rows, e->region_first_ord);
  if (rc) return rc;
  if (two_streams) MK_HIP(e, hipEventRecord(e->ev_scanned[b], e->stream));
  e->stage_two_streams[b] = two_streams;
  return MK_OK;
}

extern "C" int mk_sketch_push_reads_async(mk_engine *e, const uint8_t *rows, uint32_t stride, uint64_t nreads,
                                          uint64_t first_read_ordinal, uint64_t *ticket) {
  int rc = mk_check_push(e, rows, stride);
  if (rc) return rc;
  if (!ticket) return MK_ERR_ARG;
  MK_HIP(e, hipSetDevice(e->device));
  if ((first_read_ordinal + nreads) >> 51) return mk_fail(e, MK_ERR_ARG, "read ordinal too large");
#ifdef MK_TUNING
  double tick_ = mk_tick_now();
  const bool first_push_ = !e->d_stage[0];
#endif
  if (e->direct_host) {
    hipPointerAttribute_t attr;
    if (hipPointerGetAttributes(&attr, rows) == hipSuccess && attr.type == hipMemoryTypeHost && attr.devicePointer) {
      rc = mk_flush_region(e);
      if (rc) return rc;
      rc = mk_launch_scan(e, (const uint8_t *)attr.devicePointer, stride, nreads, first_read_ordinal);
      if (rc) return rc;
      const uint64_t t = e->tickets_issued;
      hipEvent_t ev = e->ev_ticket[t % MK_TICKETS];
      if (t >= MK_TICKETS) MK_HIP(e, hipEventSynchronize(ev));
      MK_HIP(e, hipEventRecord(ev, e->stream));
      e->tickets_issued = t + 1;
      *ticket = t;
      return MK_OK;
    }
    (void)hipGetLastError();
  }
  if (!e->d_stage[0]) {
    e->stage_bytes = MK_REGION_BYTES;
    for (int i = 0; i < MK_REGIONS; i++) MK_HIP(e, mk_dev_alloc(&e->d_stage[i], e->stage_bytes));
  }
#ifdef MK_TUNING
  if (first_push_) MK_TICK("push1: staging alloc");
#endif
  const uint32_t pitch = stride & ~MK_ROWS_PACKED;
  for (uint64_t done = 0; done < nreads;) {
    const uint64_t ord = first_read_ordinal + done;
    if (e->region_open && (stride != e->region_stride || ord != e->region_first_ord + e->region_rows ||
                           e->region_fill + pitch > e->stage_bytes)) {
      rc = mk_flush_region(e);
      if (rc) return rc;
    }
    if (!e->region_open) {
      if (e->stage_two_streams[e->stage_cur]) MK_HIP(e, hipStreamWaitEvent(e->copy_stream, e->ev_scanned[e->stage_cur], 0));
      e->region_open = true;
      e->region_fill = 0; e->region_rows = 0;
      e->region_stride = stride; e->region_first_ord = ord;
    }
    const uint64_t room = (e->stage_bytes - e->region_fill) / pitch;
    const uint64_t n = nreads - done < room ? nreads - done : room;
    MK_HIP(e, hipMemcpyAsync(e->d_stage[e->stage_cur] + e->region_fill, rows + done * pitch, n * pitch, hipMemcpyHostToDevice,
                             e->copy_stream));
#ifdef MK_TUNING
    if (first_push_ && done == 0) MK_TICK("push1: first memcpyAsync");
#endif
    e->region_fill += n * pitch;
    e->region_rows += n;
    done += n;
    if (e->region_fill + pitch > e->stage_bytes) {
      rc = mk_flush_region(e);
      if (rc) return rc;
    }
  }
  const uint64_t t = e->tickets_issued;
  hipEvent_t ev = e->ev_ticket[t % MK_TICKETS];
  if (t >= MK_TICKETS) MK_HIP(e, hipEventSynchronize(ev));
  MK_HIP(e, hipEventRecord(ev, e->copy_stream));
#ifdef MK_TUNING
  if (first_push_) MK_TICK("push1: ticket record");
#endif
  e->tickets_issued = t + 1;
  *ticket = t;
  return MK_OK;
}

extern "C" int mk_sketch_push_wait(mk_engine *e, uint64_t ticket) {
  if (!e) return MK_ERR_ARG;
// ... 1200 lines not shown
```

### metakssd_amd/csrc/mk_kernels.hip.h

```cpp
#pragma once
#include <hip/hip_runtime.h>
#include <stdint.h>

#include "host/mk_host_internal.h"
#include "mk_key.hip.h"

#define MK_WAVE 64
#define MK_MAX_CB 128
#define MK_MAX_PIECES 8
#define MK_EMPTY32 0xFFFFFFFFu
#define MK_ZMASK_WORDS 256u
#define MK_CNT_BITS 24
#define MK_CNT_MASK 0xFFFFFFull
#define MK_CNT_SAT 0xF00000ull

struct mk_table {
  unsigned long long *kc;
  unsigned long long *ordinv;
  uint32_t *err;
  uint32_t *dirty;
  uint32_t dirty_shift;
  const struct mk_front *fr;
};
struct mk_front {
  unsigned long long *kc1, *ordinv1;
  uint32_t *state;
  uint32_t shift;
  uint32_t mask;
  uint32_t limit;
  uint32_t reserved;
};
#define MK_FRONT_PROBES 16u

struct mk_batch_dev;
__device__ __forceinline__ void mk_b_upsert(const mk_batch_dev &b, uint32_t row, uint64_t key, uint64_t ord);

struct mk_scan_args {
  const uint8_t *rows;
  uint64_t nreads, first_ord;
  uint32_t stride;
  uint32_t pitch;
  uint32_t rowlen;
  const unsigned long long *nreads_dev;
  uint32_t CB, ncb;
  uint32_t ppr;
  uint32_t ppr_inv;
  uint32_t rowdw;
  uint32_t wave_lds_dwords;
  uint32_t bm_words;
  uint32_t mt_words;
  uint32_t pair_subk;
  uint32_t dimmask;
  const uint32_t *accept;
  uint32_t n_accept;
  const int32_t *shuf;
  const uint32_t *accept_bits;
  mk_keyparams kp;
  mk_table tab;
  uint4 *cand;
  uint32_t *cand_count;
  uint32_t cand_cap;
  const mk_batch_dev *batch;
};

__device__ __forceinline__ void mk_probe_init(uint64_t key, uint32_t S, uint32_t &n, uint32_t &h2) {
  n = (uint32_t)(key % S);
  h2 = 1u + (uint32_t)(key % (uint64_t)(S - 1));
}
__device__ __forceinline__ uint32_t mk_probe_next(uint32_t n, uint32_t h2, uint32_t S) {
  uint64_t t = (uint64_t)n + h2;
  return (uint32_t)(t >= S ? t - S : t);
}

__device__ __forceinline__ void mk_upsert_big(const mk_table &tab, uint32_t S, uint64_t key, uint64_t ord, uint32_t add) {
  if (tab.fr) {
    uint32_t *st = tab.fr->state;
    if (__hip_atomic_load(&st[1], __ATOMIC_RELAXED, __HIP_MEMORY_SCOPE_AGENT) == 0u) atomicOr(&st[1], 1u);
  }
  uint32_t n, h2;
  mk_probe_init(key, S, n, h2);
  const unsigned long long fresh = ((unsigned long long)key << MK_CNT_BITS) | add;
  for (uint32_t i = 0; i < S; i++) {
    unsigned long long cur = __hip_atomic_load(&tab.kc[n], __ATOMIC_RELAXED, __HIP_MEMORY_SCOPE_AGENT);
    bool mine = false;
    if (cur == 0ull) {
      const unsigned long long prev = atomicCAS(&tab.kc[n], 0ull, fresh);
      if (prev == 0ull) mine = true;
      else cur = prev;
    }
    if (mine || (cur >> MK_CNT_BITS) == key) {
      if (!mine && (cur & MK_CNT_MASK) < MK_CNT_SAT) atomicAdd(&tab.kc[n], (unsigned long long)add);
      atomicMax(&tab.ordinv[n], ~(unsigned long long)ord);
      if (mine && tab.dirty) {
        const uint32_t b = n >> tab.dirty_shift;
        atomicOr(&tab.dirty[b >> 5], 1u << (b & 31u));
      }
      return;
    }
    n = mk_probe_next(n, h2, S);
  }
  atomicOr(&tab.err[0], 1u);
}
__device__ __forceinline__ bool mk_upsert(const mk_table &tab, uint32_t S, uint64_t key, uint64_t ord, uint32_t add, bool front_open) {
  if (front_open) {
    const mk_front f = *tab.fr;
    uint32_t n = (uint32_t)(key % S) >> f.shift;
    const uint32_t step = (uint32_t)(key * 0x9E3779B1u) | 1u;
    const unsigned long long fresh = ((unsigned long long)key << MK_CNT_BITS) | add;
    for (uint32_t i = 0; i < MK_FRONT_PROBES; i++) {
      unsigned long long cur = __hip_atomic_load(&f.kc1[n], __ATOMIC_RELAXED, __HIP_MEMORY_SCOPE_AGENT);
      bool mine = false;
      if (cur == 0ull) {
        const unsigned long long prev = atomicCAS(&f.kc1[n], 0ull, fresh);
        if (prev == 0ull) mine = true;
        else cur = prev;
      }
      if (mine || (cur >> MK_CNT_BITS) == key) {
        if (!mine && (cur & MK_CNT_MASK) < MK_CNT_SAT) atomicAdd(&f.kc1[n], (unsigned long long)add);
        atomicMax(&f.ordinv1[n], ~(unsigned long long)ord);
        return mine;
      }
      n = (n + step) & f.mask;
    }
  }
  mk_upsert_big(tab, S, key, ord, add);
  return false;
}
__device__ __forceinline__ void mk_front_launch_end(const mk_table &tab, uint32_t installed, uint32_t nworkgroups) {
  if (!tab.fr) return;
  uint32_t *st = tab.fr->state;
  if (installed) atomicAdd(&st[0], installed);
  __threadfence();
  if (atomicAdd(&st[3], 1u) == nworkgroups - 1u) {
    __threadfence();
    const uint32_t total = __hip_atomic_load(&st[0], __ATOMIC_RELAXED, __HIP_MEMORY_SCOPE_AGENT);
    __hip_atomic_store(&st[2], total > tab.fr->limit ? 1u : 0u, __ATOMIC_RELAXED, __HIP_MEMORY_SCOPE_AGENT);
    __hip_atomic_store(&st[3], 0u, __ATOMIC_RELAXED, __HIP_MEMORY_SCOPE_AGENT);
  }
}
__device__ __forceinline__ bool mk_front_open(const mk_table &tab) {
  return tab.fr && __hip_atomic_load(&tab.fr->state[2], __ATOMIC_RELAXED, __HIP_MEMORY_SCOPE_AGENT) == 0u;
}

__device__ __forceinline__ uint64_t mk_scan_to_ref_codes(uint64_t k) { return k ^ ((k >> 1) & 0x5555555555555555ull); }

__device__ __forceinline__ void mk_resolve_one(const mk_scan_args &a, uint64_t scan_fwd, uint64_t ord) {
  const uint64_t fwd = mk_scan_to_ref_codes(scan_fwd);
  const uint64_t rc = mk_revcomp(fwd, a.kp.TL);
  const uint64_t uni = fwd < rc ? fwd : rc;
  uint64_t key;
  if (mk_accept_key(a.kp, a.accept_bits, a.shuf, uni, key)) {
    if (a.batch) mk_b_upsert(*a.batch, (uint32_t)(ord >> 12), key, ord);
    else mk_upsert_big(a.tab, a.kp.S, key, ord, 1u);
  }
}

typedef __attribute__((address_space(3))) const uint32_t *mk_lds_cu32;
__device__ __forceinline__ uint32_t mk_filter_mask(uint32_t x);

__device__ __forceinline__ void mk_resolve_record(const mk_scan_args &a, const uint4 r, const uint32_t *filter) {
  if (r.w & 0x80000000u) {
    mk_resolve_one(a, ((uint64_t)r.y << 32) | r.x, ((uint64_t)(r.w & 0x7FFFFFFFu) << 32) | r.z);
    return;
  }
  const uint32_t SH = a.kp.out2 - 2u;
  const uint32_t hm = (uint32_t)((1ull << (2u * a.kp.TL - 32u)) - 1ull);
  const uint32_t pos0 = (r.y & 0x1FFu) << 3, jmin = (r.y >> 9) & 7u, e = (r.y >> 12) & 15u;
  const uint32_t lo = r.y & 0xFFFF0000u, h2 = r.z & 0xFFFFu, h3 = r.z >> 16;
  const uint64_t ord0 = ((a.first_ord + (uint64_t)r.w) << 12) | pos0;
  uint32_t before = r.x, hits = 0;
#pragma unroll
  for (uint32_t j = 0; j < 8; j++) {
    const uint32_t x = (before >> SH) & a.dimmask;
    if (j >= jmin && j < e && (!filter || (mk_filter_mask(x) & ~filter[(x >> 10) & (a.bm_words - 1u)]) == 0u)) hits |= 1u << j;
    before = __builtin_amdgcn_alignbit(r.x, lo, 30u - 2u * j);
  }
  while (hits) {
    const uint32_t j = (uint32_t)__builtin_ctz(hits);
    hits &= hits - 1u;
    const uint32_t dd = 2u * (j + 1u);
    const uint32_t fl = __builtin_amdgcn_alignbit(r.x, lo, 30u - 2u * j);
    const uint32_t fhi = ((h3 << dd) | (h2 >> (16u - dd))) & hm;
    mk_resolve_one(a, ((uint64_t)fhi << 32) | fl, ord0 + j);
  }
}

__device__ __noinline__ void mk_resolve_inline(const mk_scan_args *ka, bool hit, uint4 r, const uint32_t *filter) {
  if (hit) mk_resolve_record(*ka, r, filter);
}

__device__ __forceinline__ void mk_build_filter(uint32_t *bitmap, const mk_scan_args &a);
__device__ __forceinline__ void mk_build_xfilter(uint32_t *bitmap, const mk_scan_args &a);

#define MK_RESOLVE_THREADS 1024
#define MK_RQ_CAP 128u
#ifndef MK_RESOLVE_UNROLL
#define MK_RESOLVE_UNROLL 4u
#endif


struct mk_wring {
  uint4 *q;
  uint32_t head, tail;
};
__device__ __forceinline__ void mk_wring_push(mk_wring &w, bool has, const uint4 v) {
  const uint64_t b = __ballot(has);
  if (has) w.q[(w.tail + mk_mbcnt(b)) & (MK_RQ_CAP - 1u)] = v;
  w.tail += (uint32_t)__popcll(b);
}
__device__ __forceinline__ bool mk_wring_pop(mk_wring &w, uint32_t lane, uint4 &v) {
  const uint32_t have = w.tail - w.head, n = have < 64u ? have : 64u;
  v = w.q[(w.head + lane) & (MK_RQ_CAP - 1u)];
  w.head += n;
  return lane < n;
}

__device__ __noinline__ bool mk_resolve_accepted(const mk_scan_args *ka, bool on, const uint4 v, bool front_open) {
  if (!on) return false;
  const mk_scan_args &a = *ka;
  const uint64_t uni = ((uint64_t)v.y << 32) | v.x;
  const uint32_t dim = (uint32_t)((uni & a.kp.domask) >> a.kp.out2);
  const int32_t pf = a.shuf[dim];
  if (pf >= a.kp.dim_start && pf < a.kp.dim_end) {
    const uint64_t key = mk_reduce_key(a.kp, uni, (uint64_t)(pf - a.kp.dim_start)), ord = ((uint64_t)v.w << 32) | v.z;
    if (a.batch) { mk_b_upsert(*a.batch, (uint32_t)(ord >> 12), key, ord); return false; }
    return mk_upsert(a.tab, a.kp.S, key, ord, 1u, front_open);
  }
  return false;
}
__device__ __forceinline__ void mk_resolve_candidate(const mk_scan_args &a, bool on, const uint4 v, mk_wring &r2) {
  bool pass = false;
  uint4 o = v;
  if (on) {
    const uint64_t fwd = mk_scan_to_ref_codes(((uint64_t)v.y << 32) | v.x);
    const uint64_t rc = mk_revcomp(fwd, a.kp.TL);
    const uint64_t uni = fwd < rc ? fwd : rc;
    const uint32_t dim = (uint32_t)((uni & a.kp.domask) >> a.kp.out2);
    pass = (a.accept_bits[dim >> 5] >> (dim & 31u)) & 1u;
    o.x = (uint32_t)uni; o.y = (uint32_t)(uni >> 32);
  }
  mk_wring_push(r2, pass, o);
}

__global__ void __launch_bounds__(MK_RESOLVE_THREADS) mk_resolve_kernel(const mk_scan_args a, uint32_t nslots) {
  extern __shared__ __align__(16) uint32_t rlds[];
  __shared__ uint32_t wg_installed;
  const mk_scan_args *ka = (const mk_scan_args *)__builtin_amdgcn_kernarg_segment_ptr();
  if (threadIdx.x == 0) wg_installed = 0u;
  const bool front_open = mk_front_open(a.tab);
  uint32_t installed = 0;
  if (a.pair_subk == 5u) mk_build_xfilter(rlds, a);
  else mk_build_filter(rlds, a);
  const uint32_t lane = mk_lane(), wave = threadIdx.x >> 6;
  uint4 *rings = (uint4 *)(rlds + a.bm_words) + (size_t)wave * 2u * MK_RQ_CAP;
  mk_wring r1{rings, 0u, 0u}, r2{rings + MK_RQ_CAP, 0u, 0u};

  auto drain2 = [&](uint32_t least) {
    while (r2.tail - r2.head >= least) {
      uint4 v;
      const bool on = mk_wring_pop(r2, lane, v);
      mk_wave_lds_fence();
      installed += (uint32_t)__popcll(__ballot(mk_resolve_accepted(ka, on, v, front_open)));
    }
  };
  auto drain1 = [&](uint32_t least) {
    while (r1.tail - r1.head >= least) {
      uint4 v;
      const bool on = mk_wring_pop(r1, lane, v);
      mk_wave_lds_fence();
      mk_resolve_candidate(a, on, v, r2);
      mk_wave_lds_fence();
      drain2(64u);
    }
  };

  const uint32_t SH = a.pair_subk ? a.kp.out2 - 2u : 0u;
  const bool x5 = a.pair_subk == 5u;
  const uint32_t hm = a.kp.TL > 16u ? (uint32_t)((1ull << (2u * a.kp.TL - 32u)) - 1ull) : 0u;
  const uint32_t wmask = a.bm_words - 1u;

  const uint32_t nwaves = gridDim.x * (blockDim.x >> 6);
  uint32_t slot = blockIdx.x * (blockDim.x >> 6) + wave, base = 0u, n = slot < nslots ? a.cand_count[slot] : 0u;
  auto fetch = [&](uint4 (&r)[MK_RESOLVE_UNROLL]) -> bool {
    while (slot < nslots && base >= n) {
      slot += nwaves;
      base = 0u;
      n = slot < nslots ? a.cand_count[slot] : 0u;
    }
    if (slot >= nslots) return false;
    const uint4 *c = a.cand + (size_t)slot * a.cand_cap;
#pragma unroll
    for (uint32_t u = 0; u < MK_RESOLVE_UNROLL; u++) {
      const uint32_t i = base + u * 64u + lane;
      r[u] = i < n ? c[i] : make_uint4(0u, 0u, 0u, 0u);
    }
    base += 64u * MK_RESOLVE_UNROLL;
    return true;
  };

  auto process = [&](const uint4 r) {
    const bool single = (r.w & 0x80000000u) != 0u;
    if (__any(single)) {
      mk_wring_push(r1, single, make_uint4(r.x, r.y, r.z, r.w & 0x7FFFFFFFu));
      mk_wave_lds_fence();
      drain1(64u);
    }
    const uint32_t jmin = (r.y >> 9) & 7u, e = single ? 0u : (r.y >> 12) & 15u;
    const uint32_t lo = r.y & 0xFFFF0000u;
    uint32_t hits = 0;
    if (x5) {
      uint32_t before = r.x;
#pragma unroll
      for (uint32_t j = 0; j < 8; j++) {
        const uint32_t x = (before >> SH) & 0xFFFFFu;
        if ((rlds[x >> 6] >> (x & 31u)) & 1u) hits |= 1u << j;
        before = __builtin_amdgcn_alignbit(r.x, lo, 30u - 2u * j);
      }
      hits &= (0xFFu << jmin) & ~(0xFFFFFFFFu << e);
    } else {
      uint32_t oh3 = 1u << ((r.x >> (SH + 6u)) & 31u), oh2 = 1u << ((r.x >> (SH + 4u)) & 31u), oh1 = 1u << ((r.x >> (SH + 2u)) & 31u);
      uint32_t before = r.x;
#pragma unroll
      for (uint32_t j = 0; j < 8; j++) {
        const uint32_t oh0 = 1u << ((before >> SH) & 31u);
        const uint32_t word = rlds[(before >> (SH + 10u)) & wmask];
        if (((oh0 | oh1 | oh3) & ~word) == 0u) hits |= 1u << j;
        oh3 = oh2; oh2 = oh1; oh1 = oh0;
        before = __builtin_amdgcn_alignbit(r.x, lo, 30u - 2u * j);
      }
      hits &= (0xFFu << jmin) & ~(0xFFFFFFFFu << e);
    }
    if (__any(hits != 0u)) {
      const uint32_t pos0 = (r.y & 0x1FFu) << 3, h2 = r.z & 0xFFFFu, h3 = r.z >> 16;
      const uint64_t ord0 = ((a.first_ord + (uint64_t)r.w) << 12) | pos0;
      do {
        const bool has = hits != 0u;
        const uint32_t j = has ? (uint32_t)__builtin_ctz(hits) : 0u;
        hits &= hits - 1u;
        const uint32_t dd = 2u * (j + 1u);
        const uint32_t fl = __builtin_amdgcn_alignbit(r.x, lo, 30u - 2u * j);
        const uint32_t fhi = ((h3 << dd) | (h2 >> (16u - dd))) & hm;
        const uint64_t ord = ord0 + j;
        mk_wring_push(r1, has, make_uint4(fl, fhi, (uint32_t)ord, (uint32_t)(ord >> 32)));
        mk_wave_lds_fence();
        drain1(64u);
      } while (__any(hits != 0u));
    }
  };

  uint4 r[MK_RESOLVE_UNROLL], rn[MK_RESOLVE_UNROLL];
  bool more = fetch(r);
  while (more) {
    more = fetch(rn);
#pragma unroll
    for (uint32_t u = 0; u < MK_RESOLVE_UNROLL; u++) process(r[u]);
#pragma unroll
    for (uint32_t u = 0; u < MK_RESOLVE_UNROLL; u++) r[u] = rn[u];
  }
  mk_wave_lds_fence();
  drain1(1u);
  drain2(1u);
  if (a.tab.fr) {
    if (lane == 0 && installed) atomicAdd(&wg_installed, installed);
    __syncthreads();
    if (threadIdx.x == 0) mk_front_launch_end(a.tab, wg_installed, gridDim.x);
  }
}

__device__ __forceinline__ uint32_t mk_filter_mask(uint32_t x) {
  return (1u << (x & 31u)) | (1u << ((x >> 2) & 31u)) | (1u << ((x >> 6) & 31u));
}

template <int K>
struct mk_kmer {
  uint64_t f;
  __device__ __forceinline__ void reset() { f = 0; }
  __device__ __forceinline__ void roll(uint32_t code, const mk_keyparams &kp) { f = ((f << 2) | code) & kp.tupmask; }
  __device__ __forceinline__ uint64_t fwd() const { return f; }
  __device__ __forceinline__ uint32_t dimx(const mk_keyparams &kp, uint32_t dimmask) const { return (uint32_t)(f >> kp.out2) & dimmask; }
  static __device__ __forceinline__ uint32_t TL(const mk_keyparams &kp) { return kp.TL; }
};

template <int K>
struct mk_kmer_hi {
  static_assert(K > 8 && K <= 16, "two-half representation needs 32 < 4K <= 64");
  static constexpr uint32_t HMASK = (uint32_t)((1ull << (4 * K - 32)) - 1ull);
  uint32_t flo, fhi;
  __device__ __forceinline__ void reset() { flo = fhi = 0; }
  __device__ __forceinline__ void roll(uint32_t code, const mk_keyparams &) {
    const uint32_t nfhi = __builtin_amdgcn_alignbit(fhi, flo, 30) & HMASK;
    flo = (flo << 2) | code;
    fhi = nfhi;
  }
  __device__ __forceinline__ uint64_t fwd() const { return ((uint64_t)fhi << 32) | flo; }
  __device__ __forceinline__ uint32_t dimx(const mk_keyparams &kp, uint32_t dimmask) const {
    return (uint32_t)(fwd() >> kp.out2) & dimmask;
  }
  static __device__ __forceinline__ uint32_t TL(const mk_keyparams &) { return 2u * K; }
};
template <> struct mk_kmer<9> : mk_kmer_hi<9> {};
template <> struct mk_kmer<10> : mk_kmer_hi<10> {};
template <> struct mk_kmer<11> : mk_kmer_hi<11> {};
template <> struct mk_kmer<12> : mk_kmer_hi<12> {};



template <int J>
__device__ __forceinline__ uint32_t mk_code_of(uint32_t w) {
  uint32_t r;
  asm("v_bfe_u32 %0, %1, %2, 2" : "=v"(r) : "v"(w), "n"(8 * J + 1));
  return r;
}

template <uint32_t SH>
__device__ __forceinline__ uint32_t mk_onehot_at(uint32_t flo) {
  if constexpr (SH == 8u) {
    uint32_t r;
    asm("v_lshlrev_b32_sdwa %0, %1, %2 dst_sel:DWORD dst_unused:UNUSED_PAD src0_sel:BYTE_1 src1_sel:DWORD"
        : "=v"(r) : "v"(flo), "s"(1u));
    return r;
  } else {
    return 1u << ((flo >> SH) & 31u);
  }
}

__device__ __forceinline__ uint32_t mk_nonzero_bytes(uint32_t v) {
  return (((v & 0x7F7F7F7Fu) + 0x7F7F7F7Fu) | v) & 0x80808080u;
}

__device__ __forceinline__ uint32_t mk_zmask(uint32_t b) {
  uint32_t m = 0, h = b * 0x9E3779B1u + 0x7F4A7C15u;
  while (__builtin_popcount(m) < 6) {
    m |= 1u << (h >> 27);
    h = h * 0x85EBCA6Bu + 0xC2B2AE35u;
  }
  return m;
}
#define MK_ZF_WORDS 16384u
__device__ __forceinline__ void mk_build_zfilter(uint32_t *masktab, uint32_t *bitmap, const mk_scan_args &a) {
  for (uint32_t i = threadIdx.x; i < MK_ZMASK_WORDS; i += blockDim.x) masktab[i] = mk_zmask(i);
  for (uint32_t i = threadIdx.x; i < MK_ZF_WORDS; i += blockDim.x) bitmap[i] = 0u;
  __syncthreads();
  for (uint32_t i = threadIdx.x; i < a.n_accept; i += blockDim.x) {
    const uint32_t d = (uint32_t)mk_scan_to_ref_codes(a.accept[i]);
    const uint32_t z1 = d & 0x3FFFFFu, z2 = d >> 2;
    atomicOr(&bitmap[(z1 >> 8) & (MK_ZF_WORDS - 1u)], masktab[z1 & 255u]);
    atomicOr(&bitmap[(z2 >> 8) & (MK_ZF_WORDS - 1u)], masktab[z2 & 255u]);
  }
  __syncthreads();
}

__device__ __forceinline__ void mk_build_xfilter(uint32_t *bitmap, const mk_scan_args &a) {
  for (uint32_t i = threadIdx.x; i < 16384u; i += blockDim.x) bitmap[i] = 0u;
  __syncthreads();
  for (uint32_t i = threadIdx.x; i < a.n_accept; i += blockDim.x) {
    const uint32_t d = (uint32_t)mk_scan_to_ref_codes(a.accept[i]) & 0xFFFFFu;
    atomicOr(&bitmap[d >> 6], 1u << (d & 31u));
  }
  __syncthreads();
}

__device__ __forceinline__ void mk_build_filter(uint32_t *bitmap, const mk_scan_args &a) {
  for (uint32_t i = threadIdx.x; i < a.bm_words; i += blockDim.x) bitmap[i] = 0u;
  __syncthreads();
  for (uint32_t i = threadIdx.x; i < a.n_accept; i += blockDim.x) {
    const uint32_t d = (uint32_t)mk_scan_to_ref_codes(a.accept[i]);
    atomicOr(&bitmap[(d >> 10) & (a.bm_words - 1u)], mk_filter_mask(d));
  }
  __syncthreads();
}

template <int K, int SUBK, bool VEC16, int THREADS, int NPIECES, bool ONEPASS>
__global__ void __launch_bounds__(THREADS) mk_scan_kernel(const mk_scan_args a) {
  static_assert(K == 0 || SUBK == 6 || (SUBK == 5 && K == 11), "tuned instantiations: k 9..11 with subk 6, k 11 with subk 5");
  extern __shared__ __align__(16) uint32_t lds[];
  constexpr uint32_t WAVES = THREADS / 64;
  const uint32_t lane = threadIdx.x & 63u, wave = threadIdx.x >> 6;
  const uint32_t fwords = (K != 0 && SUBK == 6) ? MK_ZF_WORDS : a.bm_words;
  uint32_t *bitmap = lds + a.mt_words;
  uint32_t *tile = lds + a.mt_words + fwords + wave * a.wave_lds_dwords;

  if constexpr (VEC16) {
    if (wave == 0) {
      uint32_t *t = lds + a.mt_words + fwords + WAVES * a.wave_lds_dwords + lane;
#pragma unroll
      for (int i = 0; i < NPIECES; i++) {
        const uint32_t q = lane + 64u * i;
        const uint32_t r = (q * a.ppr_inv) >> 20, c = q - r * a.ppr;
        t[128 * i] = r * a.pitch + c * 16u;
        t[128 * i + 64] = r * a.rowdw + c * 4u;
      }
    }
  }
  if constexpr (K != 0 && SUBK == 6) mk_build_zfilter(lds, bitmap, a);
  else if constexpr (K != 0) mk_build_xfilter(bitmap, a);
  else mk_build_filter(bitmap, a);

  const uint32_t filter_base = (uint32_t)(uintptr_t)(mk_lds_cu32)bitmap;
  constexpr uint32_t MTW = (K != 0 && SUBK == 6) ? MK_ZMASK_WORDS : 0u;
  if (K != 0 && (filter_base != MTW * 4u || a.mt_words != MTW || a.bm_words != 16384u || a.dimmask != (SUBK == 6 ? 0xFFFFFFu : 0xFFFFFu))) {
    if (threadIdx.x == 0) atomicOr(&a.tab.err[0], 4u);
    if (lane == 0) a.cand_count[blockIdx.x * WAVES + wave] = 0u;
    return;
  }
  const mk_scan_args *ka = (const mk_scan_args *)__builtin_amdgcn_kernarg_segment_ptr();
  const uint32_t TL = mk_kmer<K>::TL(a.kp);
  const uint32_t dimmask = a.dimmask;
  const uint32_t wmask4 = (a.bm_words - 1u) << 2;
  uint64_t nreads = a.nreads;
  if (a.nreads_dev) { const uint64_t nd = *a.nreads_dev; if (nd < nreads) nreads = nd; }
  const uint32_t ntiles = (uint32_t)((nreads + 63u) >> 6);
  const uint32_t wave_global = blockIdx.x * WAVES + wave;
  const uint32_t nwaves = gridDim.x * WAVES;
  uint4 *const my_cand = a.cand + (size_t)__builtin_amdgcn_readfirstlane(wave_global) * a.cand_cap;
  if (wave_global >= ntiles) {
    if (lane == 0) a.cand_count[wave_global] = 0u;
    return;
  }

  using piece_t = typename std::conditional<VEC16, uint4, uint32_t>::type;
  constexpr int NP = NPIECES;
  constexpr uint32_t PW = VEC16 ? 16u : 4u;
  piece_t regs[NP];
  piece_t regs2[ONEPASS ? NP : 1];
  auto goff_calc = [&](int i) { const uint32_t q = lane + 64u * i; const uint32_t r = (q * a.ppr_inv) >> 20, c = q - r * a.ppr; return r * a.pitch + c * PW; };
  auto loff_calc = [&](int i) { const uint32_t q = lane + 64u * i; const uint32_t r = (q * a.ppr_inv) >> 20, c = q - r * a.ppr; return r * a.rowdw + c * (PW / 4u); };
  const uint32_t *offtab = lds + a.mt_words + fwords + WAVES * a.wave_lds_dwords + lane;
  auto goff_of = [&](int i) { if constexpr (VEC16) return offtab[128 * i]; else return goff_calc(i); };
  auto loff_of = [&](int i) { if constexpr (VEC16) return offtab[128 * i + 64]; else return loff_calc(i); };
  auto issue_loads = [&](uint32_t tile_id, uint32_t cb) {
    const uint32_t row0 = tile_id << 6;
    const uint8_t *base = a.rows + (uint64_t)row0 * a.pitch + (uint64_t)cb * a.CB;
    const uint32_t cols_here = min(a.CB, a.stride - cb * a.CB);
    if constexpr (ONEPASS) {
      if (row0 + 64u <= nreads) {
#pragma unroll
        for (int i = 0; i < NP; i++)
          if ((uint32_t)i < a.ppr) { regs[i] = *(const piece_t *)(base + goff_of(i)); regs2[i] = *(const piece_t *)(base + a.CB + goff_of(i)); }
      } else {
        const uint32_t rows_here = (uint32_t)(nreads - row0);
#pragma unroll
        for (int i = 0; i < NP; i++) {
          if ((uint32_t)i < a.ppr) {
            const uint32_t q = lane + 64u * i;
            const uint32_t r = (q * a.ppr_inv) >> 20;
            if (r < rows_here) { regs[i] = *(const piece_t *)(base + goff_of(i)); regs2[i] = *(const piece_t *)(base + a.CB + goff_of(i)); }
          }
        }
      }
    } else if (row0 + 64u <= nreads && cols_here == a.CB) {
#pragma unroll
      for (int i = 0; i < NP; i++)
        if ((uint32_t)i < a.ppr) regs[i] = *(const piece_t *)(base + goff_of(i));
    } else {
      const uint32_t rows_here = (uint32_t)(nreads - row0 < 64u ? nreads - row0 : 64u);
#pragma unroll
      for (int i = 0; i < NP; i++) {
        if ((uint32_t)i < a.ppr) {
          const uint32_t q = lane + 64u * i;
          const uint32_t r = (q * a.ppr_inv) >> 20, c = q - r * a.ppr;
          if (r < rows_here && c * PW < cols_here) regs[i] = *(const piece_t *)(base + goff_of(i));
        }
      }
    }
  };
  auto commit = [&](uint32_t cb) {
    (void)cb;
#pragma unroll
    for (int i = 0; i < NP; i++) {
      if ((uint32_t)i < a.ppr) {
        if constexpr (VEC16) {
          uint32_t *p = tile + loff_of(i);
          if constexpr (ONEPASS) {
            const piece_t v = cb ? regs2[i] : regs[i];
            p[0] = v.x; p[1] = v.y; p[2] = v.z; p[3] = v.w;
          } else {
            p[0] = regs[i].x; p[1] = regs[i].y; p[2] = regs[i].z; p[3] = regs[i].w;
          }
        } else {
          tile[loff_of(i)] = regs[i];
        }
      }
    }
  };

  mk_kmer<K> km;
  km.reset();
  uint32_t hh = 0;
  uint32_t run = 0;
  bool done = true;
  uint32_t qn = 0;
  const uint32_t *myrow = tile + lane * a.rowdw;
  uint64_t ord_row = 0;

  struct quad { uint64_t u0, u1, u2, u3; uint32_t m0, m1, m2, m3, w0, w1, w2, w3; };

  auto lookup = [&](uint32_t &mask, uint32_t &word) {
    const uint32_t xx = km.dimx(a.kp, dimmask);
    if constexpr (K != 0) {
      const uint32_t z = xx & 0x3FFFFFu;
      word = *(mk_lds_cu32)(uintptr_t)(((z >> 6) & (SUBK == 6 ? (MK_ZF_WORDS - 1u) << 2 : wmask4)) + filter_base);
      mask = lds[z & 255u];
    } else {
      word = *(mk_lds_cu32)(uintptr_t)(((xx >> 8) & wmask4) + filter_base);
      mask = mk_filter_mask(xx);
    }
  };
  auto push_record = [&](bool hit, const uint4 r) {
    const uint64_t m = __ballot(hit);
    if (m == 0) return;
    const uint32_t cnt = (uint32_t)__popcll(m);
    if (qn + cnt > a.cand_cap) {
      mk_resolve_inline(ka, hit, r, K != 0 ? nullptr : bitmap);
      return;
    }
    if (hit) my_cand[qn + mk_mbcnt(m)] = r;
    qn = __builtin_amdgcn_readfirstlane(qn + cnt);
  };
  auto push_pair = [&](const bool hit, const uint64_t hm, const uint4 r) {
    const uint32_t cnt = (uint32_t)__popcll(hm);
    if (qn + cnt > a.cand_cap) { mk_resolve_inline(ka, hit, r, nullptr); return; }
    if (hit) *(uint4 *)((uint8_t *)my_cand + (qn + mk_mbcnt(hm)) * 16u) = r;
    qn += cnt;
  };
  auto push = [&](bool hit, uint64_t fwd, uint32_t pos) {
    const uint64_t ord = ord_row | (uint64_t)pos;
    push_record(hit, make_uint4((uint32_t)fwd, (uint32_t)(fwd >> 32), (uint32_t)ord, (uint32_t)(ord >> 32) | 0x80000000u));
  };

  auto fast4 = [&](uint32_t codes, quad &q) {
    km.roll(codes & 3u, a.kp);         q.u0 = km.fwd(); lookup(q.m0, q.w0);
    km.roll((codes >> 8) & 3u, a.kp);  q.u1 = km.fwd(); lookup(q.m1, q.w1);
    km.roll((codes >> 16) & 3u, a.kp); q.u2 = km.fwd(); lookup(q.m2, q.w2);
    km.roll(codes >> 24, a.kp);        q.u3 = km.fwd(); lookup(q.m3, q.w3);
  };
  auto general4 = [&](uint32_t w, uint32_t codes, uint32_t x, quad &q) {
    auto one = [&](uint32_t j, uint64_t &pu, uint32_t &pm, uint32_t &pw) {
      const uint32_t ch = (w >> (8u * j)) & 0xffu;
      const bool valid = ((x >> (8u * j)) & 0xffu) == 0u;
      if (!done && ch == '\n') done = true;
      const bool ok = valid && !done;
      if (ok) { km.roll((codes >> (8u * j)) & 3u, a.kp); run++; }
      else if (!done) run = 0;
      pu = km.fwd();
      lookup(pm, pw);
      if (!(ok && run >= TL)) { pm = 1u; pw = 0u; }
    };
    one(0, q.u0, q.m0, q.w0); one(1, q.u1, q.m1, q.w1); one(2, q.u2, q.m2, q.w2); one(3, q.u3, q.m3, q.w3);
  };
  auto hits4 = [&](const quad &q, uint32_t pos0) {
    push((q.m0 & ~q.w0) == 0u, q.u0, pos0);
    push((q.m1 & ~q.w1) == 0u, q.u1, pos0 + 1u);
    push((q.m2 & ~q.w2) == 0u, q.u2, pos0 + 2u);
    push((q.m3 & ~q.w3) == 0u, q.u3, pos0 + 3u);
  };
  auto resolve4 = [&](const quad &q, uint32_t pos0) {
    const uint32_t t0 = q.m0 & ~q.w0, t1 = q.m1 & ~q.w1, t2 = q.m2 & ~q.w2, t3 = q.m3 & ~q.w3;
    const uint32_t mn = min(min(t0, t1), min(t2, t3));
    if (__any(mn == 0u)) hits4(q, pos0);
  };
  auto decode = [&](uint32_t w, uint32_t &codes, uint32_t &x) {
    codes = (w >> 1) & 0x03030303u;
    const uint32_t expect = __builtin_amdgcn_perm(0u, 0x47544341u, codes);
    x = (w & 0xDFDFDFDFu) ^ expect;
  };
  auto slow_dword = [&](uint32_t w, uint32_t codes, uint32_t x, uint32_t pos0) {
    if (__all(x == 0u && !done && run + 4u < TL)) {
      km.roll(codes & 3u, a.kp); km.roll((codes >> 8) & 3u, a.kp); km.roll((codes >> 16) & 3u, a.kp); km.roll(codes >> 24, a.kp);
      run += 4u;
      return;
    }
    const uint32_t inval = mk_nonzero_bytes(x);
    const uint32_t notnl = mk_nonzero_bytes(w ^ 0x0A0A0A0Au);
    const uint32_t pat = inval | (notnl >> 1);
    const uint32_t pat0 = __builtin_amdgcn_readfirstlane(pat), run0 = __builtin_amdgcn_readfirstlane(run);
    if (__all(pat == pat0 && run == run0 && !done)) {
      uint32_t urun = run0;
#pragma unroll 1
      for (uint32_t j = 0; j < 4; j++) {
        if (!(pat0 & (0x40u << (8u * j)))) { done = true; break; }
        if (pat0 & (0x80u << (8u * j))) { urun = 0; continue; }
        km.roll((codes >> (8u * j)) & 3u, a.kp);
        urun++;
        if (urun >= TL) {
          uint32_t m, wd;
          lookup(m, wd);
          push((m & ~wd) == 0u, km.fwd(), pos0 + j);
        }
      }
      run = urun;
      return;
    }
    quad q;
    general4(w, codes, x, q);
    resolve4(q, pos0);
  };

  uint32_t nt_tile = wave_global;
  uint32_t nt_cb = 0;
  issue_loads(nt_tile, nt_cb);
  for (uint32_t tile_id = wave_global; tile_id < ntiles; tile_id += nwaves) {
    const uint32_t row0 = tile_id << 6;
    km.reset(); run = 0; hh = 0;
    done = row0 + lane >= nreads;
    ord_row = (a.first_ord + row0 + lane) << 12;
    for (uint32_t cb = 0; cb < a.ncb; cb++) {
      mk_wave_lds_fence();
      commit(cb);
      mk_wave_lds_fence();
      if (a.rowlen) {
        const uint32_t c0b = cb * a.CB;
        if (a.rowlen >= c0b && a.rowlen < c0b + a.CB) {
          uint32_t *q = tile + lane * a.rowdw + ((a.rowlen - c0b) >> 2);
          const uint32_t sh = (a.rowlen & 3u) * 8u;
          *q = (*q & ((1u << sh) - 1u)) | (0x0A0A0A0Au << sh);
        }
        mk_wave_lds_fence();
      }
      if constexpr (ONEPASS) {
        if (cb == 1u) { nt_tile += nwaves; if (nt_tile < ntiles) issue_loads(nt_tile, 0u); }
      } else {
        if (++nt_cb == a.ncb) { nt_cb = 0; nt_tile += nwaves; }
        if (nt_tile < ntiles) issue_loads(nt_tile, nt_cb);
      }
      if (__all(done)) continue;

      const uint32_t col0 = cb * a.CB;
      const uint32_t ndw = min(a.CB, a.stride - col0) >> 2;
      const uint32_t npairs = ndw >> 1;
      if constexpr (K != 0) {
        constexpr uint32_t SH = 2u * (K - SUBK) - 2u;
        constexpr uint32_t HM = mk_kmer<K>::HMASK;
        static_assert(SH + 4u * SUBK <= 32u, "inner substring must lie inside flo(j-1)");
        constexpr uint32_t D = SUBK == 6 ? (SH - 2u) / 2u : 1u;
        static_assert(SUBK != 6 || (SH >= 4u && SH <= 8u), "pair probing: z[0..7] at bits 2..9 of a low word D bases earlier");
        static_assert(SUBK != 5 || SH == 10u, "per-base probing: word address in WORD_1 of before_{j+1}, bit index in BYTE_1 of before_{j-1}");
        uint32_t urun = 0;
        auto in_step = [&]() -> bool {
          const uint32_t rc = min(run, TL);
          urun = __builtin_amdgcn_readlane(rc, (int)__builtin_ctzll(~__ballot(done) & __builtin_amdgcn_read_exec()));
          return __all(done || rc == urun);
        };
        bool step = in_step();
        uint32_t nw0 = myrow[0], nw1 = myrow[1];
        uint32_t p = 0;
        uint32_t flo = km.flo;
        uint32_t pa[3] = {0u, 0u, 0u};
        auto oh_init = [&]() {
          if constexpr (SUBK == 6) {
#pragma unroll
            for (uint32_t k = 0; k < D; k++) pa[k] = (flo >> (2u * (D - k))) & 0x3FCu;
          } else {
            pa[0] = flo >> 2;
          }
        };
        oh_init();
        uint32_t w0, w1, c0, x0, c1, x1;
        auto next_pair = [&]() {
          w0 = nw0; w1 = nw1;
          nw0 = myrow[2 * p + 2];
          nw1 = myrow[2 * p + 3];
          decode(w0, c0, x0);
          decode(w1, c1, x1);
        };
        auto pair_body = [&](const bool rollonly, const uint32_t jmin, const uint32_t e, const bool live, const uint64_t livem) {
          const uint32_t fstart = flo;
          const uint32_t lo = __builtin_amdgcn_perm(__builtin_amdgcn_udot4(c0, 0x01041040u, 0u, false),
                                                    __builtin_amdgcn_udot4(c1, 0x01041040u, 0u, false), 0x04000C0Cu);
          if (rollonly) {
            flo = __builtin_amdgcn_alignbit(fstart, lo, 16);
            oh_init();
          } else {
            const uint32_t f0 = __builtin_amdgcn_alignbit(fstart, lo, 30), f1 = __builtin_amdgcn_alignbit(fstart, lo, 28);
            const uint32_t f2 = __builtin_amdgcn_alignbit(fstart, lo, 26), f3 = __builtin_amdgcn_alignbit(fstart, lo, 24);
            const uint32_t f4 = __builtin_amdgcn_alignbit(fstart, lo, 22), f5 = __builtin_amdgcn_alignbit(fstart, lo, 20);
            const uint32_t f6 = __builtin_amdgcn_alignbit(fstart, lo, 18), f7 = __builtin_amdgcn_alignbit(fstart, lo, 16);
            const uint32_t bj[9] = {fstart, f0, f1, f2, f3, f4, f5, f6, f7};
            bool fired;
            if constexpr (SUBK == 6) {
              uint32_t mm[4], dd[4];
#pragma unroll
              for (uint32_t t = 0; t < 4; t++) {
                const uint32_t wsrc = bj[2u * t + 1u];
                dd[t] = *(mk_lds_cu32)(uintptr_t)(((wsrc >> (SH + 8u)) & ((MK_ZF_WORDS - 1u) << 2)) + MK_ZMASK_WORDS * 4u);
                mm[t] = *(mk_lds_cu32)(uintptr_t)(2u * t >= D ? bj[2u * t - D] & 0x3FCu : pa[2u * t]);
              }
#pragma unroll
              for (uint32_t k = 0; k < D; k++) pa[k] = bj[8u - D + k] & 0x3FCu;
              flo = f7;
              __builtin_amdgcn_sched_barrier(0);
              __builtin_amdgcn_s_waitcnt(0xC07F);
              const uint32_t tt0 = mm[0] & ~dd[0], tt1 = mm[1] & ~dd[1], tt2 = mm[2] & ~dd[2], tt3 = mm[3] & ~dd[3];
              fired = min(min(tt0, tt1), min(tt2, tt3)) == 0u;
            } else {
              uint32_t wd[8];
#pragma unroll
              for (uint32_t j = 0; j < 8; j++) {
                uint32_t addr;
                asm("v_and_b32_sdwa %0, %1, %2 dst_sel:DWORD dst_unused:UNUSED_PAD src0_sel:WORD_1 src1_sel:DWORD"
                    : "=v"(addr) : "v"(bj[j + 1u]), "v"(0xFFFCu));
                wd[j] = *(mk_lds_cu32)(uintptr_t)addr;
              }
              const uint32_t bprev = pa[0];
              pa[0] = f6;
              flo = f7;
              __builtin_amdgcn_sched_barrier(0);
              __builtin_amdgcn_s_waitcnt(0xC07F);
              uint32_t sh[8];
#pragma unroll
              for (uint32_t j = 0; j < 8; j++) {
                const uint32_t src = j == 0 ? bprev : bj[j - 1u];
                asm("v_lshrrev_b32_sdwa %0, %1, %2 dst_sel:DWORD dst_unused:UNUSED_PAD src0_sel:BYTE_1 src1_sel:DWORD"
                    : "=v"(sh[j]) : "v"(src), "v"(wd[j]));
              }
              fired = (((sh[0] | sh[1] | sh[2]) | (sh[3] | sh[4] | sh[5]) | (sh[6] | sh[7])) & 1u) != 0u;
            }
            const bool hit = fired && live;
            const uint64_t hm = __builtin_amdgcn_ballot_w64(fired) & livem;
            if (hm) {
              const uint32_t meta = ((col0 + 8u * p) >> 3) | (jmin << 9) | (e << 12);
              push_pair(hit, hm, make_uint4(fstart, (lo & 0xFFFF0000u) | meta, hh, (uint32_t)(row0 + lane)));
            }
          }
          hh = __builtin_amdgcn_perm(hh, fstart, 0x05040100u);
          ++p;
        };
        uint64_t donem = __ballot(done);
        for (;;) {
          if (step) {
            bool left = false, more = true;
            auto pair_is_bases = [&]() -> bool {
              const uint64_t bad = ((uint64_t)x1 << 32) | x0;
              uint64_t lanes_ok;
              asm("v_cmp_eq_u64_e64 %0, 0, %1" : "=s"(lanes_ok) : "v"(bad));
              return (lanes_ok | donem) == __builtin_amdgcn_read_exec();
            };
            while (urun + 1u < TL) {
              next_pair();
              if (!pair_is_bases()) { left = true; break; }
              pair_body(urun + 8u < TL, TL - 1u - urun, 8u, !done, ~donem);
              urun += 8u;
              if (p == npairs) { more = false; break; }
            }
            if (!left && more) {
              const uint32_t p0 = p;
              for (;;) {
                next_pair();
                if (!pair_is_bases()) { left = true; break; }
                pair_body(false, 0u, 8u, !done, ~donem);
                if (p == npairs) break;
              }
              urun += 8u * (p - p0);
            }
            run = urun;
            if (!left) break;
          } else {
            next_pair();
          }
          {
            const uint64_t inval = ((uint64_t)mk_nonzero_bytes(x1) << 32) | mk_nonzero_bytes(x0);
            const uint64_t nl = ((uint64_t)(mk_nonzero_bytes(w1 ^ 0x0A0A0A0Au) ^ 0x80808080u) << 32) |
                                (mk_nonzero_bytes(w0 ^ 0x0A0A0A0Au) ^ 0x80808080u);
            const uint32_t e = inval ? (uint32_t)__builtin_ctzll(inval) >> 3 : 8u;
            const uint32_t jm = run + 1u >= TL ? 0u : TL - 1u - run;
            const bool say = !done && jm < e;
            pair_body(false, jm & 7u, e, say, __builtin_amdgcn_ballot_w64(say));
            run = inval ? (uint32_t)__builtin_clzll(inval) >> 3 : min(run + 8u, 0xFFFFu);
            done = done || nl != 0ull;
            donem = __ballot(done);
            if (donem == __builtin_amdgcn_read_exec() || p == npairs) break;
            step = in_step();
          }
        }
        km.flo = flo;
        km.fhi = (hh >> 16) & HM;
      } else {
        uint32_t nw0 = myrow[0], nw1 = ndw > 1 ? myrow[1] : 0x0a0a0a0au;
        for (uint32_t p = 0; p < npairs; p++) {
          const uint32_t w0 = nw0, w1 = nw1;
          if (p + 1 < npairs) { nw0 = myrow[2 * p + 2]; nw1 = myrow[2 * p + 3]; }
          else if (ndw & 1u) nw0 = myrow[ndw - 1];
          uint32_t c0, x0, c1, x1;
          decode(w0, c0, x0);
          decode(w1, c1, x1);
          const uint32_t pos0 = col0 + 8u * p;
          if (__all((x0 | x1) == 0u && !done && run + 1u >= TL)) {
            quad qa, qb;
            fast4(c0, qa);
            fast4(c1, qb);
            run += 8u;
            resolve4(qa, pos0);
            resolve4(qb, pos0 + 4u);
          } else {
            slow_dword(w0, c0, x0, pos0);
            slow_dword(w1, c1, x1, pos0 + 4u);
            if (__all(done)) break;
          }
        }
        if ((ndw & 1u) && !__all(done)) {
          uint32_t c0, x0;
          decode(nw0, c0, x0);
          slow_dword(nw0, c0, x0, col0 + 4u * (ndw - 1u));
        }
      }
    }
  }
  if (lane == 0) a.cand_count[wave_global] = qn;
}

__global__ void __launch_bounds__(1024) mk_import_kernel(mk_table tab, uint32_t S, const unsigned long long *keys,
                                                         const uint32_t *counts, const unsigned long long *ords, uint64_t n) {
  __shared__ uint32_t wg_installed;
  if (threadIdx.x == 0) wg_installed = 0u;
  __syncthreads();
  const bool front_open = mk_front_open(tab);
  uint32_t installed = 0;
  for (uint64_t i = (uint64_t)blockIdx.x * blockDim.x + threadIdx.x; i < n; i += (uint64_t)gridDim.x * blockDim.x)
    installed += mk_upsert(tab, S, keys[i], ords[i], counts[i], front_open) ? 1u : 0u;
  if (tab.fr) {
    if (installed) atomicAdd(&wg_installed, installed);
    __syncthreads();
    if (threadIdx.x == 0) mk_front_launch_end(tab, wg_installed, gridDim.x);
  }
}

__global__ void __launch_bounds__(1024) mk_front_fold_kernel(mk_table tab, uint32_t S) {
  const mk_front f = *tab.fr;
  if (__hip_atomic_load(&f.state[1], __ATOMIC_RELAXED, __HIP_MEMORY_SCOPE_AGENT) == 0u) return;
  const uint64_t slots = (uint64_t)f.mask + 1u;
  for (uint64_t i = (uint64_t)blockIdx.x * blockDim.x + threadIdx.x; i < slots; i += (uint64_t)gridDim.x * blockDim.x) {
    const unsigned long long kc = f.kc1[i];
    if (kc == 0ull) continue;
    const uint32_t c = (uint32_t)(kc & MK_CNT_MASK);
    mk_upsert_big(tab, S, kc >> MK_CNT_BITS, ~f.ordinv1[i], c > 65535u ? 65535u : c);
    f.kc1[i] = 0ull;
    f.ordinv1[i] = 0ull;
  }
}

struct mk_dist {
  unsigned long long *key;
  unsigned long long *ord;
  uint32_t *cnt;
  uint64_t cap;
};

#define MK_SPLIT_MAX 16u
__global__ void __launch_bounds__(1024) mk_split_count_kernel(mk_dist d, const unsigned long long *Dp, uint32_t nparts, unsigned long long *hist) {
  __shared__ uint32_t h[MK_SPLIT_MAX];
  if (threadIdx.x < MK_SPLIT_MAX) h[threadIdx.x] = 0u;
  __syncthreads();
  const uint64_t D = *Dp;
  for (uint64_t i = (uint64_t)blockIdx.x * blockDim.x + threadIdx.x; i < D; i += (uint64_t)gridDim.x * blockDim.x)
    atomicAdd(&h[(uint32_t)(d.key[i] % nparts)], 1u);
  __syncthreads();
  if (threadIdx.x < nparts && h[threadIdx.x]) atomicAdd(&hist[threadIdx.x], (unsigned long long)h[threadIdx.x]);
}
__global__ void mk_split_offsets_kernel(const unsigned long long *hist, unsigned long long *cursor, uint32_t nparts) {
  unsigned long long at = 0;
  for (uint32_t g = 0; g < nparts; g++) { cursor[g] = at; at += hist[g]; }
}
__global__ void __launch_bounds__(1024) mk_split_scatter_kernel(mk_dist d, const unsigned long long *Dp, uint32_t nparts, unsigned long long *cursor,
                                                                unsigned long long *okey, uint32_t *ocnt, unsigned long long *oord, uint64_t ocap) {
  __shared__ uint32_t h[MK_SPLIT_MAX];
  __shared__ unsigned long long base[MK_SPLIT_MAX];
  const uint64_t D = *Dp;
  const uint64_t tiles = (D + blockDim.x - 1) / blockDim.x;
  for (uint64_t t = blockIdx.x; t < tiles; t += gridDim.x) {
    if (threadIdx.x < MK_SPLIT_MAX) h[threadIdx.x] = 0u;
    __syncthreads();
    const uint64_t i = t * blockDim.x + threadIdx.x;
    unsigned long long k = 0;
    uint32_t g = 0, r = 0;
    if (i < D) { k = d.key[i]; g = (uint32_t)(k % nparts); r = atomicAdd(&h[g], 1u); }
    __syncthreads();
    if (threadIdx.x < nparts) base[threadIdx.x] = h[threadIdx.x] ? atomicAdd(&cursor[threadIdx.x], (unsigned long long)h[threadIdx.x]) : 0ull;
    __syncthreads();
    if (i < D) {
      const unsigned long long o = base[g] + r;
      if (o < ocap) { okey[o] = k; ocnt[o] = d.cnt[i]; oord[o] = d.ord[i]; }
    }
    __syncthreads();
  }
}
__global__ void mk_set_counter_kernel(unsigned long long *counter, unsigned long long v) { counter[0] = v; }


__global__ void __launch_bounds__(1024) mk_dirty_list_kernel(uint32_t *bitmap, uint32_t nwords, uint32_t *list, uint32_t *count,
                                                            int clear_bitmap, const uint32_t *big_used) {
  if (big_used && __hip_atomic_load(big_used, __ATOMIC_RELAXED, __HIP_MEMORY_SCOPE_AGENT) == 0u) {
    if (threadIdx.x == 0) *count = 0u;
    return;
  }
  __shared__ uint32_t base_s;
  if (threadIdx.x == 0) base_s = 0;
  __syncthreads();
  for (uint32_t w0 = 0; w0 < nwords; w0 += 1024u) {
    const uint32_t w = w0 + threadIdx.x;
    uint32_t bits = w < nwords ? bitmap[w] : 0u;
    if (bits && clear_bitmap) bitmap[w] = 0u;
    uint32_t off = bits ? atomicAdd(&base_s, (uint32_t)__popc(bits)) : 0u;
    while (bits) {
      list[off++] = (w << 5) + (uint32_t)__builtin_ctz(bits);
      bits &= bits - 1u;
    }
  }
  __syncthreads();
  if (threadIdx.x == 0) *count = base_s;
}

__global__ void __launch_bounds__(256) mk_dirty_clear_kernel(unsigned long long *kc, unsigned long long *ordinv, uint32_t S,
                                                             const uint32_t *list, const uint32_t *nlist, uint32_t shift,
                                                             uint32_t *slot, const uint32_t *slist, const uint32_t *nslist,
                                                             uint32_t sshift) {
  const uint32_t lane = threadIdx.x & 63u;
  const uint64_t wave = ((uint64_t)blockIdx.x * blockDim.x + threadIdx.x) >> 6, nwaves = ((uint64_t)gridDim.x * blockDim.x) >> 6;
  const uint32_t n = *nlist, ns = slot ? *nslist : 0u;
  for (uint64_t i = wave; i < n; i += nwaves) {
    const uint64_t b0 = (uint64_t)list[i] << shift;
    for (uint32_t k = lane; k < (1u << shift); k += 64u)
      if (b0 + k < S) { kc[b0 + k] = 0ull; ordinv[b0 + k] = 0ull; }
  }
  for (uint64_t i = wave; i < ns; i += nwaves) {
    const uint64_t b0 = (uint64_t)slist[i] << sshift;
    for (uint32_t k = lane; k < (1u << sshift); k += 64u)
      if (b0 + k < S) slot[b0 + k] = MK_EMPTY32;
// ... 481 lines not shown
```

Before: 2730.

## Add lazy scan path that defers base validity checks to resolve

```diff
diff --git a/include/metakssd_hip.h b/include/metakssd_hip.h
--- a/include/metakssd_hip.h
+++ b/include/metakssd_hip.h
@@ -90,8 +90,9 @@
 int mk_engine_create_ex(const mk_params *p, int device, unsigned flags, mk_engine **out);
 int mk_engine_destroy(mk_engine *e);
 enum { MK_OPT_SPARSE = 1, MK_OPT_CAND_CAP = 2, MK_OPT_RESULT_CAP = 3, MK_OPT_DIRECT_HOST = 4, MK_OPT_FRONT_BITS = 5, MK_OPT_KEYLIST_CAP = 6,
-       MK_OPT_BATCH_TAB_BITS = 7, MK_OPT_SPLIT_CUS = 10 };
+       MK_OPT_BATCH_TAB_BITS = 7, MK_OPT_SPLIT_CUS = 10, MK_OPT_LAZY_SCAN = 11 };
 int mk_engine_set_option(mk_engine *e, int option, int64_t value);
+int mk_engine_get_option(mk_engine *e, int option, int64_t *value);
 int mk_engine_set_stream(mk_engine *e, void *hip_stream);
 int mk_engine_use_own_stream(mk_engine *e);
 int mk_engine_share_scan_queue(mk_engine *e, mk_engine *with);
diff --git a/metakssd_amd/capi.py b/metakssd_amd/capi.py
--- a/metakssd_amd/capi.py
+++ b/metakssd_amd/capi.py
@@ -14,6 +14,7 @@
 MK_ROWS_WIDE, MK_WIDE_MAX_BASES = 0x40000000, 240
 MK_OPT_SPARSE, MK_OPT_CAND_CAP, MK_OPT_RESULT_CAP, MK_OPT_DIRECT_HOST, MK_OPT_FRONT_BITS, MK_OPT_KEYLIST_CAP, MK_OPT_BATCH_TAB_BITS = 1, 2, 3, 4, 5, 6, 7
 MK_BEGIN_NOTHING_FOLLOWS = 0x100
+MK_OPT_LAZY_SCAN = 11
 MK_OPT_SPLIT_CUS = 10
 
 
@@ -143,6 +144,7 @@
         "mk_engine_create": [C.POINTER(ParamsC), C.c_int, C.POINTER(vp)],
         "mk_engine_destroy": [vp],
         "mk_engine_set_option": [vp, C.c_int, C.c_int64],
+        "mk_engine_get_option": [vp, C.c_int, C.POINTER(C.c_int64)],
         "mk_engine_set_stream": [vp, vp],
         "mk_engine_use_own_stream": [vp],
         "mk_engine_share_scan_queue": [vp, vp],
@@ -500,6 +502,11 @@
     def set_option(self, option, value):
         _check(lib.mk_engine_set_option(self.h, option, value), self.h)
 
+    def get_option(self, option):
+        v = C.c_int64()
+        _check(lib.mk_engine_get_option(self.h, option, C.byref(v)), self.h)
+        return int(v.value)
+
     def close(self):
         if self.h:
             lib.mk_engine_destroy(self.h)
diff --git a/metakssd_amd/csrc/mk_engine.hip b/metakssd_amd/csrc/mk_engine.hip
--- a/metakssd_amd/csrc/mk_engine.hip
+++ b/metakssd_amd/csrc/mk_engine.hip
@@ -129,6 +129,8 @@
   int tune_threads = 1024;
   bool tune_onepass = true;
   uint32_t tune_cb = MK_MAX_CB;
+  int lazy_opt = 0;
+  bool lazy_safe = false;
 
   bool profiling = false;
   std::vector<mk_evpair> ev_scan, ev_resolve, ev_clear, ev_finish, ev_pool;
@@ -250,6 +252,48 @@
   pthread_t th;
   bool started;
 };
+static uint32_t mk_zmask_host(uint32_t b) {
+  uint32_t m = 0, h = b * 0x9E3779B1u + 0x7F4A7C15u;
+  while (__builtin_popcount(m) < 6) {
+    m |= 1u << (h >> 27);
+    h = h * 0x85EBCA6Bu + 0xC2B2AE35u;
+  }
+  return m;
+}
+static bool mk_lazy_guard(int subk, const std::vector<uint32_t> &accepted ) {
+  if (subk != 5 && subk != 6) return false;
+  const uint32_t dbits = 4u * (uint32_t)subk;
+  std::vector<uint32_t> bitmap(16384u, 0u);
+  auto put = [&](uint32_t dref) {
+    const uint32_t d = dref ^ ((dref >> 1) & 0x55555555u);
+    if (subk == 6) {
+      const uint32_t z1 = d & 0x3FFFFFu, z2 = d >> 2;
+      bitmap[(z1 >> 8) & 16383u] |= mk_zmask_host(z1 & 255u);
+      bitmap[(z2 >> 8) & 16383u] |= mk_zmask_host(z2 & 255u);
+    } else {
+      const uint32_t x = d & 0xFFFFFu;
+      bitmap[x >> 6] |= 1u << (x & 31u);
+    }
+  };
+  for (uint32_t d : accepted) {
+    uint32_t c = ~d, r = 0;
+    for (uint32_t k = 0; k < dbits; k += 2) r |= ((c >> k) & 3u) << (dbits - 2u - k);
+    put(d);
+    put(r);
+  }
+  for (uint32_t code = 0; code < 4; code++) {
+    const uint32_t homo = code * 0x55555555u;
+    if (subk == 6) {
+      const uint32_t z = homo & 0x3FFFFFu;
+      if ((mk_zmask_host(z & 255u) & ~bitmap[(z >> 8) & 16383u]) == 0u) return false;
+    } else {
+      const uint32_t x = homo & 0xFFFFFu;
+      if ((bitmap[x >> 6] >> (x & 31u)) & 1u) return false;
+    }
+  }
+  return true;
+}
+
 static void *mk_accept_run(void *arg) {
   mk_accept_job *j = (mk_accept_job *)arg;
   const int32_t *t = j->t;
@@ -477,6 +521,11 @@
     size_t at = 0;
     for (int t = 0; t < nt; t++) { if (!job[t].out.empty()) memcpy(hp + at, job[t].out.data(), job[t].out.size() * sizeof(mk_accept_pair)); at += job[t].out.size(); }
   }
+  if ((p->subk == 6 && p->k >= 9 && p->k <= 11) || (p->subk == 5 && p->k == 11)) {
+    std::vector<uint32_t> acc(npairs);
+    for (size_t i = 0; i < npairs; i++) acc[i] = hp[i].d;
+    e->lazy_safe = mk_lazy_guard(p->subk, acc);
+  }
   MK_TICK("accept pass joined + pinned block");
   MK_HIP(e, mk_dev_alloc(&e->d_accept, ((size_t)e->n_accept + 2) * sizeof(uint32_t)));
   if (warm.started) { pthread_join(warm.th, nullptr); warm.started = false; }
@@ -511,6 +560,7 @@
   if (const char *t = getenv("MK_SCAN_THREADS")) { int v = atoi(t); if (v == 512 || v == 768 || v == 1024) e->tune_threads = v; }
   if (const char *t = getenv("MK_SCAN_ONEPASS")) e->tune_onepass = atoi(t) != 0;
   if (const char *t = getenv("MK_SCAN_CB")) { int v = atoi(t); if (v >= 16 && v <= MK_MAX_CB && v % 16 == 0) e->tune_cb = (uint32_t)v; }
+  if (const char *t = getenv("MK_SCAN_LAZY")) { int v = atoi(t); if (v >= -1 && v <= 1) e->lazy_opt = v; }
 #endif
   return lazy_tables ? MK_OK : mk_tables_alloc(e);
 }
@@ -661,6 +711,10 @@
     case MK_OPT_DIRECT_HOST:
       e->direct_host = value != 0;
       return MK_OK;
+    case MK_OPT_LAZY_SCAN:
+      if (value < -1 || value > 1) return mk_fail(e, MK_ERR_ARG, "MK_OPT_LAZY_SCAN takes -1 (by the .shuf's filter), 0 or 1");
+      e->lazy_opt = (int)value;
+      return MK_OK;
     case MK_OPT_SPLIT_CUS: return mk_config_split(e, (int)value);
     case MK_OPT_BATCH_TAB_BITS:
       if (value != 0 && (value < 9 || value > 22)) return mk_fail(e, MK_ERR_ARG, "MK_OPT_BATCH_TAB_BITS takes 0 (by file size) or 9..22");
@@ -685,6 +739,19 @@
       return MK_OK;
     }
     default: return mk_fail(e, MK_ERR_ARG, "unknown engine option %d", option);
+  }
+}
+
+extern "C" int mk_engine_get_option(mk_engine *e, int option, int64_t *value) {
+  if (!e || !value) return MK_ERR_ARG;
+  switch (option) {
+    case MK_OPT_LAZY_SCAN:
+      *value = e->lazy_opt > 0 || (e->lazy_opt < 0 && e->lazy_safe) ? 1 : 0;
+      return MK_OK;
+    case MK_OPT_CAND_CAP: *value = (int64_t)e->cand_cap; return MK_OK;
+    case MK_OPT_DIRECT_HOST: *value = e->direct_host ? 1 : 0; return MK_OK;
+    case MK_OPT_SPLIT_CUS: *value = (int64_t)e->split_cus; return MK_OK;
+    default: return mk_fail(e, MK_ERR_ARG, "mk_engine_get_option: option %d cannot be read", option);
   }
 }
 
@@ -877,9 +944,9 @@
   return MK_OK;
 }
 
-template <int K, int SK, bool V, int T, int NP, bool OP>
+template <int K, int SK, bool V, int T, int NP, bool OP, bool LZ = false>
 static hipError_t mk_launch_scan_t(mk_engine *e, const mk_scan_args &a, dim3 grid, size_t lds, hipStream_t s) {
-  const void *fn = (const void *)mk_scan_kernel<K, SK, V, T, NP, OP>;
+  const void *fn = (const void *)mk_scan_kernel<K, SK, V, T, NP, OP, LZ>;
   size_t *granted = nullptr;
   for (auto &g : e->lds_granted) if (g.first == fn) granted = &g.second;
   if (!granted) { e->lds_granted.emplace_back(fn, 0); granted = &e->lds_granted.back().second; }
@@ -888,7 +955,7 @@
     if (r != hipSuccess) return r;
     *granted = lds;
   }
-  hipLaunchKernelGGL((mk_scan_kernel<K, SK, V, T, NP, OP>), grid, dim3(T), lds, s, a);
+  hipLaunchKernelGGL((mk_scan_kernel<K, SK, V, T, NP, OP, LZ>), grid, dim3(T), lds, s, a);
   return hipGetLastError();
 }
 template <int K, int SK, bool V>
@@ -897,6 +964,9 @@
   constexpr int NPSMALL = V ? 5 : 20;
   const bool small = a.ppr <= (uint32_t)NPSMALL;
   if constexpr (V) {
+    if constexpr (K != 0) {
+      if (a.lazy && onepass && small && threads >= 1024) return mk_launch_scan_t<K, SK, V, 1024, NPSMALL, true, true>(e, a, grid, lds, s);
+    }
     if (onepass && small)
       return threads >= 1024 ? mk_launch_scan_t<K, SK, V, 1024, NPSMALL, true>(e, a, grid, lds, s)
              : threads >= 768 ? mk_launch_scan_t<K, SK, V, 768, NPSMALL, true>(e, a, grid, lds, s)
@@ -958,6 +1028,8 @@
     if (lds <= 160u * 1024u || threads <= 512) break;
   }
   if (lds > 160u * 1024u) return mk_fail(e, MK_ERR_ARG, "scan: LDS budget exceeded (%zu bytes)", lds);
+  a.lazy = (e->lazy_opt > 0 || (e->lazy_opt < 0 && e->lazy_safe)) && tuned_k && !packed && onepass && threads >= 1024 && rowlen == 0u &&
+           !nreads_dev && !a.batch && stride <= MK_LAZY_MAX_STRIDE ? 1u : 0u;
   const uint32_t waves = (uint32_t)threads / 64u;
   const uint64_t ntiles = (nreads + 63) / 64;
   uint64_t blocks = (ntiles + waves - 1) / waves;
@@ -1048,7 +1120,7 @@
 #endif
     const size_t rlds = (size_t)a.bm_words * 4u + (size_t)(MK_RESOLVE_THREADS / 64) * 2u * MK_RQ_CAP * sizeof(uint4);
     {
-      const void *fn = (const void *)mk_resolve_kernel;
+      const void *fn = a.lazy ? (const void *)mk_resolve_kernel<true> : (const void *)mk_resolve_kernel<false>;
       size_t *granted = nullptr;
       for (auto &g : e->lds_granted) if (g.first == fn) granted = &g.second;
       if (!granted) { e->lds_granted.emplace_back(fn, 0); granted = &e->lds_granted.back().second; }
@@ -1057,7 +1129,8 @@
         *granted = rlds;
       }
     }
-    hipLaunchKernelGGL(mk_resolve_kernel, dim3(rgrid), dim3(MK_RESOLVE_THREADS), rlds, e->stream, a, used_slots);
+    if (a.lazy) hipLaunchKernelGGL(mk_resolve_kernel<true>, dim3(rgrid), dim3(MK_RESOLVE_THREADS), rlds, e->stream, a, used_slots);
+    else hipLaunchKernelGGL(mk_resolve_kernel<false>, dim3(rgrid), dim3(MK_RESOLVE_THREADS), rlds, e->stream, a, used_slots);
     MK_HIP(e, hipGetLastError());
 #ifdef MK_TUNING
     if (getenv("MK_COUNT_RECORDS")) {
diff --git a/metakssd_amd/csrc/mk_kernels.hip.h b/metakssd_amd/csrc/mk_kernels.hip.h
--- a/metakssd_amd/csrc/mk_kernels.hip.h
+++ b/metakssd_amd/csrc/mk_kernels.hip.h
@@ -41,6 +41,7 @@
   uint32_t stride;
   uint32_t pitch;
   uint32_t rowlen;
+  uint32_t lazy;
   const unsigned long long *nreads_dev;
   uint32_t CB, ncb;
   uint32_t ppr;
@@ -144,23 +145,73 @@
 
 __device__ __forceinline__ uint64_t mk_scan_to_ref_codes(uint64_t k) { return k ^ ((k >> 1) & 0x5555555555555555ull); }
 
+template <int GROUP> __device__ __forceinline__ bool mk_text_ok(const mk_scan_args &a, uint64_t ord);
+
+template <bool TEXT = false>
 __device__ __forceinline__ void mk_resolve_one(const mk_scan_args &a, uint64_t scan_fwd, uint64_t ord) {
   const uint64_t fwd = mk_scan_to_ref_codes(scan_fwd);
   const uint64_t rc = mk_revcomp(fwd, a.kp.TL);
   const uint64_t uni = fwd < rc ? fwd : rc;
   uint64_t key;
-  if (mk_accept_key(a.kp, a.accept_bits, a.shuf, uni, key)) {
+  if (mk_accept_key(a.kp, a.accept_bits, a.shuf, uni, key) && (!TEXT || mk_text_ok<1>(a, ord))) {
     if (a.batch) mk_b_upsert(*a.batch, (uint32_t)(ord >> 12), key, ord);
     else mk_upsert_big(a.tab, a.kp.S, key, ord, 1u);
   }
 }
 
+__device__ __forceinline__ uint32_t mk_nonzero_bytes(uint32_t v) {
+  return (((v & 0x7F7F7F7Fu) + 0x7F7F7F7Fu) | v) & 0x80808080u;
+}
+
+#define MK_LAZY_MAX_STRIDE 160u
+#ifndef MK_TEXT_GROUP
+#define MK_TEXT_GROUP 5
+#endif
+__device__ __forceinline__ uint32_t mk_low_bytes(int32_t n) {
+  return n <= 0 ? 0u : n >= 4 ? 0xFFFFFFFFu : (1u << (8 * n)) - 1u;
+}
+__device__ __forceinline__ uint32_t mk_text_bad4(uint32_t w, int32_t npre, int32_t nupto) {
+  const uint32_t codes = (w >> 1) & 0x03030303u;
+  const uint32_t x = (w & 0xDFDFDFDFu) ^ __builtin_amdgcn_perm(0u, 0x47544341u, codes);
+  const uint32_t inval = mk_nonzero_bytes(x), nl = mk_nonzero_bytes(w ^ 0x0A0A0A0Au) ^ 0x80808080u;
+  const uint32_t pre = mk_low_bytes(npre), upto = mk_low_bytes(nupto);
+  return (nl & pre) | (inval & upto & ~pre);
+}
+template <int GROUP>
+__device__ __forceinline__ bool mk_text_ok(const mk_scan_args &a, uint64_t ord) {
+  uint64_t nreads = a.nreads;
+  if (a.nreads_dev) { const uint64_t nd = *a.nreads_dev; if (nd < nreads) nreads = nd; }
+  const uint64_t r = (ord >> 12) - a.first_ord;
+  const uint32_t j = (uint32_t)ord & 0xFFFu, TL = a.kp.TL;
+  if (r >= nreads || j + 1u < TL || j >= a.stride || a.stride > MK_LAZY_MAX_STRIDE) return false;
+  const uint4 *row = (const uint4 *)(a.rows + r * (uint64_t)a.pitch);
+  const int32_t first = (int32_t)(j + 1u - TL), past = (int32_t)(j + 1u);
+  constexpr int NPC = (int)(MK_LAZY_MAX_STRIDE / 16u);
+  static_assert(NPC % GROUP == 0, "pieces of a row in whole groups");
+  uint32_t bad = 0;
+#pragma unroll 1
+  for (int g = 0; g < NPC; g += GROUP) {
+    if (16 * g >= past) break;
+    uint4 v[GROUP];
+#pragma unroll
+    for (int i = 0; i < GROUP; i++) v[i] = 16 * (g + i) < past ? row[g + i] : make_uint4(0u, 0u, 0u, 0u);
+#pragma unroll
+    for (int i = 0; i < GROUP; i++) {
+      const int32_t c = 16 * (g + i);
+      bad |= mk_text_bad4(v[i].x, first - c, past - c) | mk_text_bad4(v[i].y, first - c - 4, past - c - 4) |
+             mk_text_bad4(v[i].z, first - c - 8, past - c - 8) | mk_text_bad4(v[i].w, first - c - 12, past - c - 12);
+    }
+  }
+  return bad == 0u;
+}
+
 typedef __attribute__((address_space(3))) const uint32_t *mk_lds_cu32;
 __device__ __forceinline__ uint32_t mk_filter_mask(uint32_t x);
 
+template <bool TEXT = false>
 __device__ __forceinline__ void mk_resolve_record(const mk_scan_args &a, const uint4 r, const uint32_t *filter) {
   if (r.w & 0x80000000u) {
-    mk_resolve_one(a, ((uint64_t)r.y << 32) | r.x, ((uint64_t)(r.w & 0x7FFFFFFFu) << 32) | r.z);
+    mk_resolve_one<TEXT>(a, ((uint64_t)r.y << 32) | r.x, ((uint64_t)(r.w & 0x7FFFFFFFu) << 32) | r.z);
     return;
   }
   const uint32_t SH = a.kp.out2 - 2u;
@@ -181,12 +232,15 @@
     const uint32_t dd = 2u * (j + 1u);
     const uint32_t fl = __builtin_amdgcn_alignbit(r.x, lo, 30u - 2u * j);
     const uint32_t fhi = ((h3 << dd) | (h2 >> (16u - dd))) & hm;
-    mk_resolve_one(a, ((uint64_t)fhi << 32) | fl, ord0 + j);
+    mk_resolve_one<TEXT>(a, ((uint64_t)fhi << 32) | fl, ord0 + j);
   }
 }
 
 __device__ __noinline__ void mk_resolve_inline(const mk_scan_args *ka, bool hit, uint4 r, const uint32_t *filter) {
   if (hit) mk_resolve_record(*ka, r, filter);
+}
+__device__ __noinline__ void mk_resolve_inline_lazy(const mk_scan_args *ka, bool hit, uint4 r) {
+  if (hit) mk_resolve_record<true>(*ka, r, nullptr);
 }
 
 __device__ __forceinline__ void mk_build_filter(uint32_t *bitmap, const mk_scan_args &a);
@@ -215,12 +269,16 @@
   return lane < n;
 }
 
+template <bool TEXT>
 __device__ __noinline__ bool mk_resolve_accepted(const mk_scan_args *ka, bool on, const uint4 v, bool front_open) {
   if (!on) return false;
   const mk_scan_args &a = *ka;
   const uint64_t uni = ((uint64_t)v.y << 32) | v.x;
   const uint32_t dim = (uint32_t)((uni & a.kp.domask) >> a.kp.out2);
   const int32_t pf = a.shuf[dim];
+  if constexpr (TEXT) {
+    if (!mk_text_ok<MK_TEXT_GROUP>(a, ((uint64_t)v.w << 32) | v.z)) return false;
+  }
   if (pf >= a.kp.dim_start && pf < a.kp.dim_end) {
     const uint64_t key = mk_reduce_key(a.kp, uni, (uint64_t)(pf - a.kp.dim_start)), ord = ((uint64_t)v.w << 32) | v.z;
     if (a.batch) { mk_b_upsert(*a.batch, (uint32_t)(ord >> 12), key, ord); return false; }
@@ -242,6 +300,7 @@
   mk_wring_push(r2, pass, o);
 }
 
+template <bool TEXT>
 __global__ void __launch_bounds__(MK_RESOLVE_THREADS) mk_resolve_kernel(const mk_scan_args a, uint32_t nslots) {
   extern __shared__ __align__(16) uint32_t rlds[];
   __shared__ uint32_t wg_installed;
@@ -260,7 +319,7 @@
       uint4 v;
       const bool on = mk_wring_pop(r2, lane, v);
       mk_wave_lds_fence();
-      installed += (uint32_t)__popcll(__ballot(mk_resolve_accepted(ka, on, v, front_open)));
+      installed += (uint32_t)__popcll(__ballot(mk_resolve_accepted<TEXT>(ka, on, v, front_open)));
     }
   };
   auto drain1 = [&](uint32_t least) {
@@ -424,10 +483,6 @@
   }
 }
 
-__device__ __forceinline__ uint32_t mk_nonzero_bytes(uint32_t v) {
-  return (((v & 0x7F7F7F7Fu) + 0x7F7F7F7Fu) | v) & 0x80808080u;
-}
-
 __device__ __forceinline__ uint32_t mk_zmask(uint32_t b) {
   uint32_t m = 0, h = b * 0x9E3779B1u + 0x7F4A7C15u;
   while (__builtin_popcount(m) < 6) {
@@ -470,9 +525,10 @@
   __syncthreads();
 }
 
-template <int K, int SUBK, bool VEC16, int THREADS, int NPIECES, bool ONEPASS>
+template <int K, int SUBK, bool VEC16, int THREADS, int NPIECES, bool ONEPASS, bool LAZY = false>
 __global__ void __launch_bounds__(THREADS) mk_scan_kernel(const mk_scan_args a) {
   static_assert(K == 0 || SUBK == 6 || (SUBK == 5 && K == 11), "tuned instantiations: k 9..11 with subk 6, k 11 with subk 5");
+  static_assert(!LAZY || (K != 0 && VEC16 && ONEPASS), "the lazy loop: tuned geometries, one-pass staging");
   extern __shared__ __align__(16) uint32_t lds[];
   constexpr uint32_t WAVES = THREADS / 64;
   const uint32_t lane = threadIdx.x & 63u, wave = threadIdx.x >> 6;
@@ -619,7 +675,11 @@
   };
   auto push_pair = [&](const bool hit, const uint64_t hm, const uint4 r) {
     const uint32_t cnt = (uint32_t)__popcll(hm);
-    if (qn + cnt > a.cand_cap) { mk_resolve_inline(ka, hit, r, nullptr); return; }
+    if (qn + cnt > a.cand_cap) {
+      if constexpr (LAZY) mk_resolve_inline_lazy(ka, hit, r);
+      else mk_resolve_inline(ka, hit, r, nullptr);
+      return;
+    }
     if (hit) *(uint4 *)((uint8_t *)my_cand + (qn + mk_mbcnt(hm)) * 16u) = r;
     qn += cnt;
   };
@@ -708,7 +768,7 @@
       mk_wave_lds_fence();
       commit(cb);
       mk_wave_lds_fence();
-      if (a.rowlen) {
+      if (!LAZY && a.rowlen) {
         const uint32_t c0b = cb * a.CB;
         if (a.rowlen >= c0b && a.rowlen < c0b + a.CB) {
           uint32_t *q = tile + lane * a.rowdw + ((a.rowlen - c0b) >> 2);
@@ -735,13 +795,6 @@
         constexpr uint32_t D = SUBK == 6 ? (SH - 2u) / 2u : 1u;
         static_assert(SUBK != 6 || (SH >= 4u && SH <= 8u), "pair probing: z[0..7] at bits 2..9 of a low word D bases earlier");
         static_assert(SUBK != 5 || SH == 10u, "per-base probing: word address in WORD_1 of before_{j+1}, bit index in BYTE_1 of before_{j-1}");
-        uint32_t urun = 0;
-        auto in_step = [&]() -> bool {
-          const uint32_t rc = min(run, TL);
-          urun = __builtin_amdgcn_readlane(rc, (int)__builtin_ctzll(~__ballot(done) & __builtin_amdgcn_read_exec()));
-          return __all(done || rc == urun);
-        };
-        bool step = in_step();
         uint32_t nw0 = myrow[0], nw1 = myrow[1];
         uint32_t p = 0;
         uint32_t flo = km.flo;
@@ -765,8 +818,14 @@
         };
         auto pair_body = [&](const bool rollonly, const uint32_t jmin, const uint32_t e, const bool live, const uint64_t livem) {
           const uint32_t fstart = flo;
-          const uint32_t lo = __builtin_amdgcn_perm(__builtin_amdgcn_udot4(c0, 0x01041040u, 0u, false),
-                                                    __builtin_amdgcn_udot4(c1, 0x01041040u, 0u, false), 0x04000C0Cu);
+          uint32_t lo;
+          if constexpr (LAZY) {
+            lo = (__builtin_amdgcn_udot4(w0 & 0x06060606u, 0x01041040u, 0u, false) << 23) |
+                 (__builtin_amdgcn_udot4(w1 & 0x06060606u, 0x01041040u, 0u, false) << 15);
+          } else {
+            lo = __builtin_amdgcn_perm(__builtin_amdgcn_udot4(c0, 0x01041040u, 0u, false),
+                                       __builtin_amdgcn_udot4(c1, 0x01041040u, 0u, false), 0x04000C0Cu);
+          }
           if (rollonly) {
             flo = __builtin_amdgcn_alignbit(fstart, lo, 16);
             oh_init();
@@ -818,13 +877,38 @@
             const bool hit = fired && live;
             const uint64_t hm = __builtin_amdgcn_ballot_w64(fired) & livem;
             if (hm) {
-              const uint32_t meta = ((col0 + 8u * p) >> 3) | (jmin << 9) | (e << 12);
-              push_pair(hit, hm, make_uint4(fstart, (lo & 0xFFFF0000u) | meta, hh, (uint32_t)(row0 + lane)));
+              uint32_t meta = ((col0 + 8u * p) >> 3) | (jmin << 9) | (e << 12);
+              if constexpr (LAZY) {
+                asm("" : "+s"(meta));
+                push_pair(hit, hm, make_uint4(fstart, lo | meta, hh, (uint32_t)(row0 + lane)));
+              } else {
+                push_pair(hit, hm, make_uint4(fstart, (lo & 0xFFFF0000u) | meta, hh, (uint32_t)(row0 + lane)));
+              }
             }
           }
           hh = __builtin_amdgcn_perm(hh, fstart, 0x05040100u);
           ++p;
         };
+        if constexpr (LAZY) {
+          const bool live = !done;
+          const uint64_t livem = ~__ballot(done);
+          auto lazy_pair = [&](const bool rollonly, const uint32_t jmin) {
+            w0 = nw0; w1 = nw1;
+            nw0 = myrow[2 * p + 2];
+            nw1 = myrow[2 * p + 3];
+            pair_body(rollonly, jmin, 8u, live, livem);
+          };
+          while (p < npairs && col0 + 8u * p + 8u < TL) lazy_pair(true, 0u);
+          if (p < npairs && col0 + 8u * p + 1u < TL) lazy_pair(false, TL - 1u - (col0 + 8u * p));
+          while (p < npairs) lazy_pair(false, 0u);
+        } else {
+        uint32_t urun = 0;
+        auto in_step = [&]() -> bool {
+          const uint32_t rc = min(run, TL);
+          urun = __builtin_amdgcn_readlane(rc, (int)__builtin_ctzll(~__ballot(done) & __builtin_amdgcn_read_exec()));
+          return __all(done || rc == urun);
+        };
+        bool step = in_step();
         uint64_t donem = __ballot(done);
         for (;;) {
           if (step) {
@@ -872,6 +956,7 @@
             step = in_step();
           }
         }
+        }
         km.flo = flo;
         km.fhi = (hh >> 16) & HM;
       } else {
```

Result: slower. 2650 (-2.9%).
